# Fancomi2017/InstanceFusion

Hardware: AMD Instinct MI355X
Metric: frames/s + ms/frame (ICP|fuse|instance) at 640x480, 5M surfels, 1/2/4/8 GPU (higher is better)
Workload: dtype f32; 1 GPU; 5000000-surfel map, 640x480 synthetic RGBD stream, 3-level ICP+RGB + surfel fuse + canned-mask instance votes with superpixel refinement; surfels_live=4734799, surfel_slots=4734799, map_order=random, parallelism=replicas x1, loop_frames=90

## Files before the change

include/ifx_c_api.h:

```cpp
#ifndef IFX_C_API_H_
#define IFX_C_API_H_

#include <stdint.h>

#ifdef __cplusplus
extern "C" {
#endif

#define IFX_NUM_INSTANCES 96
#define IFX_VOTE_FLOATS 48

enum {
    IFX_OK = 0,
    IFX_E_INVALID = -1,
    IFX_E_HIP = -2,
    IFX_E_CAPACITY = -3,
    IFX_E_STATE = -4
};

typedef struct ifx_config {
    int32_t width, height;
    float fx, fy, cx, cy;
    int32_t time_delta;
    float confidence;
    float depth_cut;
    float max_depth_processed;
    float icp_weight;
    int32_t pyramid;
    int32_t fast_odom;
    int32_t so3;
    int32_t max_surfels;
    int32_t device;
    int32_t n_ranks, rank;
} ifx_config;

typedef struct ifx ifx_t;

int ifx_create(const ifx_config* cfg, ifx_t** out);
void ifx_destroy(ifx_t* h);
const char* ifx_last_error(ifx_t* h);
const char* ifx_global_error(void);

int ifx_process_frame(ifx_t* h, const uint8_t* rgb, const uint16_t* depth, int64_t timestamp,
                      const float* in_pose16, float weight_mult, float* out_pose16);
int ifx_process_frame_ex(ifx_t* h, const uint8_t* rgb, const uint16_t* depth, int64_t timestamp, const int32_t* inst_table,
                         const float* in_pose16, float weight_mult, int bootstrap, float* out_pose16);
int ifx_enqueue_frame_device(ifx_t* h, const uint8_t* d_rgb, const uint16_t* d_depth,
                             int64_t timestamp, const float* in_pose16, float weight_mult);
int ifx_prefetch_frame_device(ifx_t* h, const uint8_t* d_rgb_next, const uint16_t* d_depth_next);
int ifx_hint_next_frame_device(ifx_t* h, const uint8_t* d_rgb_next, const uint16_t* d_depth_next);
int ifx_hint_next_frame(ifx_t* h, const uint8_t* rgb_next, const uint16_t* depth_next);
int ifx_set_shard(ifx_t* h, int rank, int nranks);
int ifx_sharded_frame_phase(ifx_t* h, int phase, const uint8_t* d_rgb, const uint16_t* d_depth);
int ifx_key_images(ifx_t* h, void** key_index, void** key_splat, void** key_ids, void** key_both, int64_t* n_pixels);
int ifx_stream_handles(ifx_t* h, void** main_stream, void** side_stream);
int ifx_owner_frame_phase(ifx_t* h, int phase, const uint8_t* d_rgb, const uint16_t* d_depth);
int ifx_camera_count(ifx_t* h, int n_cameras);
int ifx_camera_select(ifx_t* h, int cam);
int ifx_owner_set_frame_pose(ifx_t* h, const float* pose16);
int ifx_owner_set_tracking_rank(ifx_t* h, int rank);
int ifx_owner_track_ahead(ifx_t* h, int cam, int tracking_rank, const uint8_t* d_rgb, const uint16_t* d_depth);
int ifx_comm_unique_id(uint8_t* out128);
int ifx_owner_init_comm(ifx_t* h, const uint8_t* unique_id128);
int ifx_owner_set_comm(ifx_t* h, void* nccl_comm);
int ifx_owner_process_frame_device(ifx_t* h, const uint8_t* d_rgb, const uint16_t* d_depth, int64_t timestamp);
int ifx_owner_process_frame(ifx_t* h, const uint8_t* rgb, const uint16_t* depth, int64_t timestamp, float* out_pose16);
int ifx_owner_predict(ifx_t* h);
int ifx_owner_process_segmentation(ifx_t* h, const uint8_t* rgb, const uint16_t* depth, const uint8_t* masks, const int32_t* class_ids, int nm, int frame, int flags);
int ifx_owner_knn_vote_colour(ifx_t* h);
int ifx_owner_exchange_stats(ifx_t* h, int64_t* out2, int reset);
int ifx_owner_comm_ranks(ifx_t* h);
int ifx_owner_exchange(ifx_t* h, int phase, void** ptrs, int64_t* bytes, int32_t* ops, int max_n);
int ifx_owner_predict_phase(ifx_t* h, int step);
int ifx_owner_of(const float* xyz, int n, int n_ranks, int32_t* out);
int ifx_owner_segmentation_begin(ifx_t* h, const uint8_t* rgb, const uint16_t* depth, const uint8_t* masks, const int32_t* class_ids, int nm, int frame, int flags);
int ifx_owner_segmentation_resume(ifx_t* h);
int ifx_owner_ids_begin(ifx_t* h);
int ifx_owner_ids_resume(ifx_t* h);
int ifx_owner_knn_export(ifx_t* h, void** d_points, void** d_labels, int* n);
int ifx_owner_knn_vote(ifx_t* h, const void* d_all_points, const void* d_all_labels, int n_all, int own_offset);
int ifx_map_seq(ifx_t* h, uint32_t* out, int max_n);
int ifx_map_bounding_boxes(ifx_t* h, int bbox_type, float ratio, float* boxes96x6, float* ground_normal3, float* gc_matrix16, float* inst_matrix96x16,
                           int32_t* ground_votes648);
int ifx_instance_point_cloud(ifx_t* h, int bbox_type, int32_t* counts96, int inst, float* out10, int max_records);
int ifx_view_list_stats(ifx_t* h, int32_t* out4);
int ifx_sync(ifx_t* h);
int ifx_get_pose(ifx_t* h, float* out_pose16);
int ifx_tick(ifx_t* h);
int ifx_trajectory(ifx_t* h, float* out_poses16, int max_frames);
int ifx_tracker_diag(ifx_t* h, float* diag8);
int ifx_tracker_fallbacks(ifx_t* h);
int ifx_tracker_range_exceeded(ifx_t* h);

int ifx_set_loop_closure(ifx_t* h, int enable, int count_thresh, float err_thresh, float cov_thresh);
int ifx_loop_closure_diag(ifx_t* h, float* out24);
typedef int (*ifx_loop_closure_cb)(ifx_t* h, const float* lc24, void* user);
int ifx_set_loop_closure_callback(ifx_t* h, ifx_loop_closure_cb cb, void* user);
int ifx_sample_graph_model(ifx_t* h, float* out_xyzt, int max_n);
int ifx_loop_closure_constraints(ifx_t* h, float* src3, float* dst3, int32_t* times, int max_n);
int ifx_set_deformation(ifx_t* h, const float* graph16, int n_nodes, int is_fern);
int ifx_adopt_estimated_pose(ifx_t* h);

typedef int (*ifx_fern_cb)(ifx_t* h, void* user);
int ifx_set_fern_callback(ifx_t* h, ifx_fern_cb cb, void* user);
int ifx_adopt_pose(ifx_t* h, const float* pose16);
int ifx_fern_frame(ifx_t* h, uint8_t* img_rgb, float* verts4, float* norms4, uint8_t* inst_rgb);
int ifx_fern_frame_async(ifx_t* h);
int ifx_fern_frame_fetch(ifx_t* h, uint8_t* img_rgb, float* verts4, float* norms4, uint8_t* inst_rgb);
int ifx_track_maps(ifx_t* h, const float* model_v4, const float* model_n4, const uint8_t* model_rgba, const float* cur_v4, const float* cur_n4,
                   const uint8_t* cur_rgba, float* pose16, float* diag8);

typedef struct ifx_soa_view {
    int32_t count;
    int32_t capacity;
    float* d_pos_conf;
    float* d_norm_rad;
    float* d_color;
    float* d_times;
    float* d_img_corr;
    float* d_votes;
} ifx_soa_view;
int ifx_map_view(ifx_t* h, ifx_soa_view* out);
int ifx_hot_records_stale(ifx_t* h);
int ifx_map_count(ifx_t* h);
int ifx_map_slots(ifx_t* h);
int ifx_map_download(ifx_t* h, int max_n, float* pc, float* nr, float* col, float* tm, float* ic,
                     float* votes);
int ifx_map_upload(ifx_t* h, int n, const float* pc, const float* nr, const float* col,
                   const float* tm, const float* ic, const float* votes);
int ifx_set_pose(ifx_t* h, const float* pose16, int tick);
int ifx_compact(ifx_t* h);
int ifx_set_option(ifx_t* h, const char* name, int value);

const int32_t* ifx_ids_after(ifx_t* h);
int ifx_image_download(ifx_t* h, const char* name, void* out, int64_t max_bytes);

int ifx_predict_indices(ifx_t* h, const float* pose16, int time);
int ifx_combined_predict(ifx_t* h, const float* pose16, int time, int max_time);
int ifx_fuse(ifx_t* h, const float* pose16, int time, float weighting);
int ifx_clean(ifx_t* h, const float* pose16, int time);
int ifx_render_ids(ifx_t* h, const float* pose16, int mode);
int ifx_set_frame(ifx_t* h, const uint8_t* rgb, const uint16_t* depth);

int ifx_icp_step(ifx_t* h, const float* Rcurr9, const float* tcurr3, const float* d_vmap_curr,
                 const float* d_nmap_curr, const float* Rprev_inv9, const float* tprev3, float fx,
                 float fy, float cx, float cy, const float* d_vmap_g_prev, const float* d_nmap_g_prev,
                 float dist_thres, float angle_thres, int w, int hgt, float* out29_host);
int ifx_rgb_residual(ifx_t* h, float min_scale, const int16_t* d_didx, const int16_t* d_didy,
                     const float* d_last_depth, const float* d_next_depth, const uint8_t* d_last_img,
                     const uint8_t* d_next_img, void* d_corres8, float max_depth_delta,
                     const float* kt3, const float* krkinv9, int w, int hgt, int* count_host,
                     int* sigma_host);
int ifx_rgb_step(ifx_t* h, const void* d_corres8, float sigma, const float* d_cloud3, float fx,
                 float fy, const int16_t* d_didx, const int16_t* d_didy, float sobel_scale, int w,
                 int hgt, float* out29_host);
int ifx_so3_step(ifx_t* h, const uint8_t* d_last_img, const uint8_t* d_next_img,
                 const float* image_basis9, const float* kinv9, const float* krlr9, int w, int hgt,
                 float* out11_host);
typedef struct ifx_pyramids {
    uint16_t* depth[3];
    float* vmap_curr[3];
    float* nmap_curr[3];
    uint8_t* next_img[3];
    int16_t* didx[3];
    int16_t* didy[3];
    float* vmap_g_prev[3];
    float* nmap_g_prev[3];
    float* last_depth[3];
// ... 41 lines not shown
```

instancefusion_amd/__init__.py:

```python
from __future__ import annotations

import ctypes as C
import os

import numpy as np

_HERE = os.path.dirname(os.path.abspath(__file__))
LIB_PATH = os.environ.get("IFX_LIB") or os.path.join(_HERE, "libifx.so")
HEADER_PATH = os.path.join(os.path.dirname(_HERE), "include", "ifx_c_api.h")

NUM_INSTANCES = 96
VOTE_FLOATS = 48


class IfxError(RuntimeError):
    pass


class IfxConfig(C.Structure):
    _fields_ = [
        ("width", C.c_int32), ("height", C.c_int32),
        ("fx", C.c_float), ("fy", C.c_float), ("cx", C.c_float), ("cy", C.c_float),
        ("time_delta", C.c_int32), ("confidence", C.c_float), ("depth_cut", C.c_float),
        ("max_depth_processed", C.c_float), ("icp_weight", C.c_float),
        ("pyramid", C.c_int32), ("fast_odom", C.c_int32), ("so3", C.c_int32),
        ("max_surfels", C.c_int32), ("device", C.c_int32), ("n_ranks", C.c_int32), ("rank", C.c_int32),
    ]


class Pyramids(C.Structure):
    _fields_ = [(n, C.c_void_p * 3) for n in ("depth", "vmap_curr", "nmap_curr", "next_img", "didx", "didy", "vmap_g_prev", "nmap_g_prev", "last_depth", "last_img", "cloud")]


class SoaView(C.Structure):
    _fields_ = [("count", C.c_int32), ("capacity", C.c_int32), ("d_pos_conf", C.c_void_p), ("d_norm_rad", C.c_void_p),
                ("d_color", C.c_void_p), ("d_times", C.c_void_p), ("d_img_corr", C.c_void_p), ("d_votes", C.c_void_p)]


def default_config(w=640, h=480, fx=528.0, fy=528.0, cx=320.0, cy=240.0, max_surfels=1 << 20, **kw):
    d = dict(width=w, height=h, fx=fx, fy=fy, cx=cx, cy=cy, time_delta=200, confidence=10.0, depth_cut=12.0,
             max_depth_processed=20.0, icp_weight=10.0, pyramid=1, fast_odom=0, so3=1, max_surfels=max_surfels,
             device=0, n_ranks=1, rank=0)
    d.update(kw)
    return d


_lib = None

_P = C.c_void_p
_SIGS = {
    "ifx_create": (C.c_int, [C.POINTER(IfxConfig), C.POINTER(_P)]),
    "ifx_destroy": (None, [_P]),
    "ifx_last_error": (C.c_char_p, [_P]),
    "ifx_global_error": (C.c_char_p, []),
    "ifx_process_frame": (C.c_int, [_P, _P, _P, C.c_int64, _P, C.c_float, _P]),
    "ifx_process_frame_ex": (C.c_int, [_P, _P, _P, C.c_int64, _P, _P, C.c_float, C.c_int, _P]),
    "ifx_enqueue_frame_device": (C.c_int, [_P, _P, _P, C.c_int64, _P, C.c_float]),
    "ifx_set_shard": (C.c_int, [_P, C.c_int, C.c_int]),
    "ifx_sharded_frame_phase": (C.c_int, [_P, C.c_int, _P, _P]),
    "ifx_key_images": (C.c_int, [_P, _P, _P, _P, _P, _P]),
    "ifx_stream_handles": (C.c_int, [_P, _P, _P]),
    "ifx_owner_frame_phase": (C.c_int, [_P, C.c_int, _P, _P]),
    "ifx_owner_exchange": (C.c_int, [_P, C.c_int, _P, _P, _P, C.c_int]),
    "ifx_owner_of": (C.c_int, [_P, C.c_int, C.c_int, _P]),
    "ifx_owner_segmentation_begin": (C.c_int, [_P, _P, _P, _P, _P, C.c_int, C.c_int, C.c_int]),
    "ifx_owner_segmentation_resume": (C.c_int, [_P]),
    "ifx_owner_ids_begin": (C.c_int, [_P]),
    "ifx_owner_ids_resume": (C.c_int, [_P]),
    "ifx_owner_knn_export": (C.c_int, [_P, _P, _P, _P]),
    "ifx_owner_knn_vote": (C.c_int, [_P, _P, _P, C.c_int, C.c_int]),
    "ifx_owner_predict_phase": (C.c_int, [_P, C.c_int]),
    "ifx_camera_count": (C.c_int, [_P, C.c_int]),
    "ifx_camera_select": (C.c_int, [_P, C.c_int]),
    "ifx_owner_set_frame_pose": (C.c_int, [_P, _P]),
    "ifx_owner_set_tracking_rank": (C.c_int, [_P, C.c_int]),
    "ifx_owner_track_ahead": (C.c_int, [_P, C.c_int, C.c_int, _P, _P]),
    "ifx_comm_unique_id": (C.c_int, [_P]),
    "ifx_owner_init_comm": (C.c_int, [_P, _P]),
    "ifx_owner_set_comm": (C.c_int, [_P, _P]),
    "ifx_owner_process_frame_device": (C.c_int, [_P, _P, _P, C.c_int64]),
    "ifx_owner_process_frame": (C.c_int, [_P, _P, _P, C.c_int64, _P]),
    "ifx_owner_predict": (C.c_int, [_P]),
    "ifx_owner_process_segmentation": (C.c_int, [_P, _P, _P, _P, _P, C.c_int, C.c_int, C.c_int]),
    "ifx_owner_knn_vote_colour": (C.c_int, [_P]),
    "ifx_owner_exchange_stats": (C.c_int, [_P, _P, C.c_int]),
    "ifx_owner_comm_ranks": (C.c_int, [_P]),
    "ifx_map_seq": (C.c_int, [_P, _P, C.c_int]),
    "ifx_prefetch_frame_device": (C.c_int, [_P, _P, _P]),
    "ifx_hint_next_frame_device": (C.c_int, [_P, _P, _P]),
    "ifx_hint_next_frame": (C.c_int, [_P, _P, _P]),
    "ifx_lookahead_stats": (C.c_int, [_P, _P, C.c_int]),
    "ifx_view_list_stats": (C.c_int, [_P, _P]),
    "ifx_map_bounding_boxes": (C.c_int, [_P, C.c_int, C.c_float, _P, _P, _P, _P, _P]),
    "ifx_instance_point_cloud": (C.c_int, [_P, C.c_int, _P, C.c_int, _P, C.c_int]),
    "ifx_sync": (C.c_int, [_P]),
    "ifx_get_pose": (C.c_int, [_P, _P]),
    "ifx_tick": (C.c_int, [_P]),
    "ifx_trajectory": (C.c_int, [_P, _P, C.c_int]),
    "ifx_tracker_diag": (C.c_int, [_P, _P]),
    "ifx_tracker_fallbacks": (C.c_int, [_P]),
    "ifx_build_pyramids": (C.c_int, [_P, _P, _P, _P, _P, _P, _P, C.POINTER(Pyramids)]),
    "ifx_tracker_range_exceeded": (C.c_int, [_P]),
    "ifx_hot_records_stale": (C.c_int, [_P]),
    "ifx_set_loop_closure": (C.c_int, [_P, C.c_int, C.c_int, C.c_float, C.c_float]),
    "ifx_loop_closure_diag": (C.c_int, [_P, _P]),
    "ifx_set_loop_closure_callback": (C.c_int, [_P, _P, _P]),
    "ifx_sample_graph_model": (C.c_int, [_P, _P, C.c_int]),
    "ifx_loop_closure_constraints": (C.c_int, [_P, _P, _P, _P, C.c_int]),
    "ifx_set_deformation": (C.c_int, [_P, _P, C.c_int, C.c_int]),
    "ifx_adopt_estimated_pose": (C.c_int, [_P]),
    "ifx_set_fern_callback": (C.c_int, [_P, _P, _P]),
    "ifx_adopt_pose": (C.c_int, [_P, _P]),
    "ifx_fern_frame": (C.c_int, [_P, _P, _P, _P, _P]),
    "ifx_fern_frame_async": (C.c_int, [_P]),
    "ifx_fern_frame_fetch": (C.c_int, [_P, _P, _P, _P, _P]),
    "ifx_track_maps": (C.c_int, [_P, _P, _P, _P, _P, _P, _P, _P, _P]),
    "ifx_map_view": (C.c_int, [_P, C.POINTER(SoaView)]),
    "ifx_map_count": (C.c_int, [_P]),
    "ifx_map_slots": (C.c_int, [_P]),
    "ifx_map_download": (C.c_int, [_P, C.c_int] + [_P] * 6),
    "ifx_map_upload": (C.c_int, [_P, C.c_int] + [_P] * 6),
    "ifx_set_pose": (C.c_int, [_P, _P, C.c_int]),
    "ifx_compact": (C.c_int, [_P]),
    "ifx_set_option": (C.c_int, [_P, C.c_char_p, C.c_int]),
    "ifx_ids_after": (_P, [_P]),
    "ifx_image_download": (C.c_int, [_P, C.c_char_p, _P, C.c_int64]),
    "ifx_predict_indices": (C.c_int, [_P, _P, C.c_int]),
    "ifx_combined_predict": (C.c_int, [_P, _P, C.c_int, C.c_int]),
    "ifx_fuse": (C.c_int, [_P, _P, C.c_int, C.c_float]),
    "ifx_clean": (C.c_int, [_P, _P, C.c_int]),
    "ifx_render_ids": (C.c_int, [_P, _P, C.c_int]),
    "ifx_set_frame": (C.c_int, [_P, _P, _P]),
    "ifx_icp_step": (C.c_int, [_P, _P, _P, _P, _P, _P, _P, C.c_float, C.c_float, C.c_float, C.c_float, _P, _P, C.c_float, C.c_float, C.c_int, C.c_int, _P]),
    "ifx_rgb_residual": (C.c_int, [_P, C.c_float, _P, _P, _P, _P, _P, _P, _P, C.c_float, _P, _P, C.c_int, C.c_int, _P, _P]),
    "ifx_rgb_step": (C.c_int, [_P, _P, C.c_float, _P, C.c_float, C.c_float, _P, _P, C.c_float, C.c_int, C.c_int, _P]),
    "ifx_so3_step": (C.c_int, [_P, _P, _P, _P, _P, _P, C.c_int, C.c_int, _P]),
    "ifx_track_pair": (C.c_int, [_P] * 9),
    "ifx_tracker_buffer_download": (C.c_int, [_P, C.c_char_p, C.c_int, _P, C.c_int64]),
    "ifx_should_segment": (C.c_int, [_P, C.c_int]),
    "ifx_process_segmentation": (C.c_int, [_P, _P, _P, _P, _P, C.c_int, C.c_int, C.c_int]),
    "ifx_process_segmentation_device": (C.c_int, [_P, _P, C.c_int, C.c_float, _P, C.c_int, C.c_int, C.c_int, _P]),
    "ifx_labels": (C.c_int, [_P, _P, C.c_int]),
    "ifx_render_project_map": (C.c_int, [_P, _P, _P]),
    "ifx_set_instance_gt": (C.c_int, [_P, _P]),
    "ifx_precision_recall": (C.c_int, [_P, _P, _P, _P]),
    "ifx_instance_table": (C.c_int, [_P, _P]),
    "ifx_loop_closure_instance_table": (C.c_int, [_P, _P]),
    "ifx_mask_clean_overlap": (C.c_int, [_P, _P, C.c_int]),
    "ifx_mask_geometric_filter": (C.c_int, [_P, _P, _P, _P, C.c_int, _P]),
    "ifx_knn_vote_colour": (C.c_int, [_P, _P, C.c_int]),
    "ifx_slic_segment": (C.c_int, [_P, _P, _P]),
    "ifx_merge_superpixels": (C.c_int, [_P, _P, _P, _P, _P]),
    "ifx_mask_superpixel_filter": (C.c_int, [_P, _P, _P, C.c_int]),
    "ifx_stage_ms": (C.c_int, [_P, _P, C.c_int]),
    "ifx_superpixel_ahead_stats": (C.c_int, [_P, _P, _P, _P, C.c_int]),
    "ifx_kernel_ms": (C.c_int, [_P, C.c_char_p, _P, _P]),
}


def lib():
    global _lib
    if _lib is None:
        if not os.path.exists(LIB_PATH):
            raise IfxError(f"{LIB_PATH} is missing: build it with `make -C instancefusion_amd/csrc` "
                           "(there is no CPU fallback)")
        L = C.CDLL(LIB_PATH)
        for name, (res, args) in _SIGS.items():
            f = getattr(L, name)
            f.restype = res
            f.argtypes = args
        _lib = L
    return _lib


def exported_symbols():
# ... 45 lines not shown
        if r != 0:
            raise IfxError(f"ifx_create failed ({r}): {self.L.ifx_global_error().decode()}")
        self.handle = hp
        if id_rule is not None:
            self.set_option("id_rule", id_rule)

    def close(self):
        if getattr(self, "handle", None):
            self.L.ifx_destroy(self.handle)
            self.handle = None

    def __del__(self):
        try:
            self.close()
        except Exception:
            pass

    def _chk(self, r, what):
        if r < 0:
            raise IfxError(f"{what} failed ({r}): {self.L.ifx_last_error(self.handle).decode()}")
        return r

    def set_option(self, name, value):
        self._chk(self.L.ifx_set_option(self.handle, name.encode(), int(value)), "ifx_set_option")

    def set_instance_gt(self, gt):
        self._chk(self.L.ifx_set_instance_gt(self.handle, None if gt is None else _ptr(np.ascontiguousarray(gt, np.uint8))), "ifx_set_instance_gt")

    def processFrame(self, rgb, depth, timestamp=0, smallInstanceTable=None, instanceGT=None, inPose=None, weightMultiplier=1.0, bootstrap=False):
        rgb = np.ascontiguousarray(rgb, np.uint8)
        depth = np.ascontiguousarray(depth, np.uint16)
        assert rgb.size == self.w * self.h * 3 and depth.size == self.w * self.h
        if instanceGT is not None:
            self.set_instance_gt(instanceGT)
        out = np.zeros(16, np.float32)
        ip = None if inPose is None else np.ascontiguousarray(inPose, np.float32).reshape(16)
        tab = None if smallInstanceTable is None else np.ascontiguousarray(smallInstanceTable, np.int32)
        self._chk(self.L.ifx_process_frame_ex(self.handle, _ptr(rgb), _ptr(depth), int(timestamp), _ptr(tab), _ptr(ip), float(weightMultiplier), int(bool(bootstrap)), _ptr(out)),
                  "ifx_process_frame_ex")
        return out.reshape(4, 4)

    process_frame = processFrame

    def hint_next_frame(self, rgb, depth):
        rgb = np.ascontiguousarray(rgb, np.uint8)
        depth = np.ascontiguousarray(depth, np.uint16)
        assert rgb.size == self.w * self.h * 3 and depth.size == self.w * self.h
        self._chk(self.L.ifx_hint_next_frame(self.handle, _ptr(rgb), _ptr(depth)), "ifx_hint_next_frame")

    def enqueue_frame_device(self, d_rgb_ptr: int, d_depth_ptr: int, timestamp=0):
        self._chk(self.L.ifx_enqueue_frame_device(self.handle, C.c_void_p(d_rgb_ptr), C.c_void_p(d_depth_ptr), int(timestamp), None, 1.0),
                  "ifx_enqueue_frame_device")

    def prefetch_frame_device(self, d_rgb_ptr: int, d_depth_ptr: int):
        self._chk(self.L.ifx_prefetch_frame_device(self.handle, C.c_void_p(d_rgb_ptr), C.c_void_p(d_depth_ptr)), "ifx_prefetch_frame_device")

    def hint_next_frame_device(self, d_rgb_ptr: int, d_depth_ptr: int):
        self._chk(self.L.ifx_hint_next_frame_device(self.handle, C.c_void_p(d_rgb_ptr), C.c_void_p(d_depth_ptr)), "ifx_hint_next_frame_device")

    def camera_count(self, k):
        self._chk(self.L.ifx_camera_count(self.handle, int(k)), "ifx_camera_count")

    def camera_select(self, c):
        self._chk(self.L.ifx_camera_select(self.handle, int(c)), "ifx_camera_select")

    def owner_set_frame_pose(self, pose):
        p = None if pose is None else np.ascontiguousarray(pose, np.float32).reshape(16)
        self._chk(self.L.ifx_owner_set_frame_pose(self.handle, _ptr(p)), "ifx_owner_set_frame_pose")

    def owner_track_ahead(self, cam, tracking_rank, d_rgb_ptr=0, d_depth_ptr=0):
        return self._chk(self.L.ifx_owner_track_ahead(self.handle, int(cam), int(tracking_rank), C.c_void_p(d_rgb_ptr), C.c_void_p(d_depth_ptr)), "ifx_owner_track_ahead")

    def owner_frame_phase(self, phase, d_rgb_ptr=0, d_depth_ptr=0):
        return self._chk(self.L.ifx_owner_frame_phase(self.handle, int(phase), C.c_void_p(d_rgb_ptr), C.c_void_p(d_depth_ptr)), "ifx_owner_frame_phase")

    def owner_set_tracking_rank(self, r):
        self._chk(self.L.ifx_owner_set_tracking_rank(self.handle, int(r)), "ifx_owner_set_tracking_rank")

    def view_list_stats(self):
        out = np.zeros(4, np.int32)
        self._chk(self.L.ifx_view_list_stats(self.handle, _ptr(out)), "ifx_view_list_stats")
        return dict(window=int(out[0]), outside=int(out[1]), scans=int(out[2]), age=int(out[3]))

    def sync(self):
        self._chk(self.L.ifx_sync(self.handle), "ifx_sync")

    def getCurrPose(self):
        out = np.zeros(16, np.float32)
        self._chk(self.L.ifx_get_pose(self.handle, _ptr(out)), "ifx_get_pose")
        return out.reshape(4, 4)

    @property
    def tick(self):
        return self.L.ifx_tick(self.handle)

    def trajectory(self, max_frames=1 << 16):
        out = np.zeros((max_frames, 16), np.float32)
        n = self._chk(self.L.ifx_trajectory(self.handle, _ptr(out), max_frames), "ifx_trajectory")
        return out[:n].reshape(n, 4, 4).copy()

    def tracker_diag(self):
        out = np.zeros(8, np.float32)
        self._chk(self.L.ifx_tracker_diag(self.handle, _ptr(out)), "ifx_tracker_diag")
        return out

    def tracker_fallbacks(self):
        return self._chk(self.L.ifx_tracker_fallbacks(self.handle), "ifx_tracker_fallbacks")

    def tracker_range_exceeded(self):
        return self._chk(self.L.ifx_tracker_range_exceeded(self.handle), "ifx_tracker_range_exceeded")

    def set_loop_closure(self, enable=True, count_thresh=35000, err_thresh=5e-5, cov_thresh=1e-5):
        self._chk(self.L.ifx_set_loop_closure(self.handle, int(enable), int(count_thresh), err_thresh, cov_thresh), "ifx_set_loop_closure")

    def loop_closure_diag(self):
        out = np.zeros(24, np.float32)
        self._chk(self.L.ifx_loop_closure_diag(self.handle, _ptr(out)), "ifx_loop_closure_diag")
        return dict(ran=bool(out[0]), inactive_pixels=int(out[1]), icp_error=float(out[2]), icp_count=float(out[3]), cov_ok=bool(out[4]),
                    accepted=bool(out[5]), est_pose=out[6:22].reshape(4, 4).copy(), cov_max=float(out[22]), candidates=int(out[23]))

    def set_loop_closure_callback(self, fn):
        if fn is None:
            self._lc_cb = None
            self._chk(self.L.ifx_set_loop_closure_callback(self.handle, None, None), "ifx_set_loop_closure_callback")
            return

        def tramp(_h, lc, _user):
            try:
                fn(self, np.ctypeslib.as_array(lc, shape=(24,)).copy())
                return 0
            except Exception:
                import traceback

                traceback.print_exc()
                return -1

        self._lc_cb = C.CFUNCTYPE(C.c_int, C.c_void_p, C.POINTER(C.c_float), C.c_void_p)(tramp)
        self._chk(self.L.ifx_set_loop_closure_callback(self.handle, C.cast(self._lc_cb, C.c_void_p), None), "ifx_set_loop_closure_callback")

    def sample_graph_model(self, max_n=4096):
        out = np.zeros((max_n, 4), np.float32)
        n = self._chk(self.L.ifx_sample_graph_model(self.handle, _ptr(out), max_n), "ifx_sample_graph_model")
        return out[:n].copy()

    def loop_closure_constraints(self, max_n=4096):
        src, dst, tm = np.zeros((max_n, 3), np.float32), np.zeros((max_n, 3), np.float32), np.zeros(max_n, np.int32)
        n = self._chk(self.L.ifx_loop_closure_constraints(self.handle, _ptr(src), _ptr(dst), _ptr(tm), max_n), "ifx_loop_closure_constraints")
        return src[:n].copy(), dst[:n].copy(), tm[:n].copy()

    def set_deformation(self, graph16, is_fern=False):
        g = np.ascontiguousarray(graph16, np.float32).reshape(-1, 16)
        self._chk(self.L.ifx_set_deformation(self.handle, _ptr(g), g.shape[0], int(is_fern)), "ifx_set_deformation")

    def adopt_estimated_pose(self):
        self._chk(self.L.ifx_adopt_estimated_pose(self.handle), "ifx_adopt_estimated_pose")

    def set_fern_callback(self, fn):
        if fn is None:
            self._fern_cb = None
            self._chk(self.L.ifx_set_fern_callback(self.handle, None, None), "ifx_set_fern_callback")
            return

        def tramp(_h, _user):
            try:
                return 1 if fn(self) else 0
            except Exception:
# ... 308 lines not shown
```

instancefusion_amd/csrc/ifx_api.hip:

```cpp
#include <climits>
#include "ifx_ctx.h"
#include <string.h>
#include <stdio.h>
#include <algorithm>

int ifx_tracker_external_pose(ifx* h, const float* d_pose16, float weight_mult);
int ifx_tracker_set_weight(ifx* h, float weight_mult);
int ifx_compact_enqueue(ifx* h, int refresh_ids);

void hs_invalidate_view(ifx* h);
static std::string g_err;
extern "C" const char* ifx_global_error(void) { return g_err.c_str(); }
extern "C" const char* ifx_last_error(ifx_t* h) { return h ? h->err.c_str() : g_err.c_str(); }

hipEvent_t ifx_event_get(ifx* h)
{
    if (!h->event_pool.empty()) { hipEvent_t e = h->event_pool.back(); h->event_pool.pop_back(); return e; }
    hipEvent_t e;
    hipEventCreate(&e);
    return e;
}
void ifx_ktime_begin(ifx* h, const char* name, hipEvent_t* a)
{
    (void)name;
// ... 207 lines not shown
    if (h->ev_cam_side) hipEventDestroy(h->ev_cam_side);
    if (h->ev_slic_ahead) hipEventDestroy(h->ev_slic_ahead);
    if (h->ev_cam_parked) hipEventDestroy(h->ev_cam_parked);
    if (h->ev_lc_ready) hipEventDestroy(h->ev_lc_ready);
    if (h->ev_lc_done) hipEventDestroy(h->ev_lc_done);
    void* ptrs[] = {h->d_state, h->d_traj, h->d_scratch, h->pc, h->nr, h->col, h->tm, h->ic, h->votes, h->pc2, h->nr2, h->col2, h->tm2, h->ic2, h->votes2, h->upd_owner, h->assoc_vis, h->list_a, h->list_b, h->list_c, h->list_v, h->list_vi, h->d_list_ctr, h->tile_n, h->tile_box, h->tile_pairs, h->tile_recs, h->labels, h->seq, h->seq2,
                    h->labels2, h->scan_flags, h->scan_out, h->scan_block, h->slot[0].rgb, h->slot[0].depth_raw, h->slot[0].depth_filt, h->slot[0].dm, h->slot[0].dmf, h->slot[1].rgb, h->slot[1].depth_raw,
                    h->slot[1].depth_filt, h->slot[1].dm, h->slot[1].dmf, h->key_index, h->key_both,
                    h->index_id, h->index_vc, h->index_ct, h->index_tap, h->pred_vertex, h->fill_vertex,
                    h->fill_normal, h->fill_image, h->ids_after, h->ids_tmp, h->assoc_key, h->assoc_target, h->meas_pc, h->meas_nr, h->meas_col};
    for (void* p : ptrs) if (p) hipFree(p);
    for (size_t q = 2; q < h->slot.size(); q++) { FrameSlot& f2 = h->slot[q]; void* p2[] = {f2.rgb, f2.depth_raw, f2.depth_filt, f2.dm, f2.dmf}; for (void* p : p2) if (p) hipFree(p); }
    if (h->h_result) hipHostFree(h->h_result);
    if (h->h_pose_early) hipHostFree(h->h_pose_early);
    if (h->ev_pose_early) hipEventDestroy(h->ev_pose_early);
    for (int q_ = 0; q_ < 2; q_++) { if (h->hint_stage_rgb[q_]) hipHostFree(h->hint_stage_rgb[q_]); if (h->hint_stage_depth[q_]) hipHostFree(h->hint_stage_depth[q_]); }
    if (h->rgb_stage) hipHostFree(h->rgb_stage);
    if (h->depth_stage) hipHostFree(h->depth_stage);
    ifx_free_tracker(h);
    ifx_free_instance(h);
    ifx_slic_free(h);
    ifx_knn_free_all(h);
    for (int q = 0; q < 2; q++) { if (h->slot[q].ready) hipEventDestroy(h->slot[q].ready); if (h->slot[q].released) hipEventDestroy(h->slot[q].released); }
    if (h->stream_c) hipStreamDestroy(h->stream_c);
    if (h->stream_b) hipStreamDestroy(h->stream_b);
    if (h->stream) hipStreamDestroy(h->stream);
    delete h;
}

extern "C" int ifx_set_loop_closure(ifx_t* h, int enable, int count_thresh, float err_thresh, float cov_thresh)
{
    if (!h) return IFX_E_INVALID;
    if (h->hint_rgb || h->slot[h->tick & 1].for_tick == h->tick) { h->err = "loop-closure detection cannot change while a frame is announced ahead"; return IFX_E_STATE; }
    ifx_drop_tracked(h);
    if (h->stream_c) { HIPCHK(h, hipStreamSynchronize(h->stream_c)); h->lc_pending = 0; }
    if (enable) {
        int r = ifx_tracker_alloc_m2m(h);
        if (r) return r;
        if (!h->stream_c && hipStreamCreate(&h->stream_c) != hipSuccess) { h->err = "stream creation failed"; return IFX_E_HIP; }
        if (!h->ev_lc_ready) {
            if (hipEventCreateWithFlags(&h->ev_lc_ready, hipEventDisableTiming) != hipSuccess ||
                hipEventCreateWithFlags(&h->ev_lc_done, hipEventDisableTiming) != hipSuccess) { h->err = "event creation failed"; return IFX_E_HIP; }
        }
    }
    h->lc_enable = enable ? 1 : 0; h->lc_count_thresh = count_thresh; h->lc_err_thresh = err_thresh; h->lc_cov_thresh = cov_thresh;
    return IFX_OK;
}
extern "C" int ifx_set_loop_closure_callback(ifx_t* h, ifx_loop_closure_cb cb, void* user)
{
    if (!h) return IFX_E_INVALID;
    h->lc_cb = cb; h->lc_user = user;
    return IFX_OK;
}
extern "C" int ifx_set_fern_callback(ifx_t* h, ifx_fern_cb cb, void* user)
{
    if (!h) return IFX_E_INVALID;
    if (cb && !h->lc_enable) { h->err = "the fern callback runs inside the loop-closure block: enable it first (ifx_set_loop_closure)"; return IFX_E_STATE; }
    h->fern_cb = cb; h->fern_user = user;
    return IFX_OK;
}
extern "C" int ifx_loop_closure_diag(ifx_t* h, float* out24)
{
    if (!h || !out24) return IFX_E_INVALID;
    if (!h->h_lc) { memset(out24, 0, 24 * 4); return IFX_OK; }
    if (h->ev_result) HIPCHK(h, hipEventSynchronize(h->ev_result));
    if (h->lc_event_valid) HIPCHK(h, hipEventSynchronize(h->ev_lc_done));
    memcpy(out24, h->h_lc, 24 * 4);
    return IFX_OK;
}

extern "C" int ifx_set_option(ifx_t* h, const char* name, int value)
{
    if (!h || !name) return IFX_E_INVALID;
    std::string s(name);
    if (s == "compact_every_frame") h->opt_compact_every_frame = value;
    else if (s == "kernel_timing") { hipStreamSynchronize(h->stream); ktime_flush(h); h->opt_kernel_timing = value; }
    else if (s == "reference_passes") { h->opt_reference_passes = value; ifx_vlist_reap(h); hs_invalidate_view(h); }
    else if (s == "two_streams") h->opt_two_streams = value;
    else if (s == "stage_timing") h->opt_stage_timing = value;
    else if (s == "track_ahead") h->opt_track_ahead = value;
    else if (s == "slic_ahead") h->opt_slic_ahead = value;
    else if (s == "fold_result") h->opt_fold_result = value;
    else if (s == "clean_raster") h->opt_clean_raster = value;
    else if (s == "hot_records") { h->opt_hot = value; h->hot_valid = 0; }
    else if (s == "hot_verify") h->opt_hot_verify = value;
    else if (s == "own_first_live") h->opt_own_first_live = value;
    else if (s == "own_track_rows") {
        if (!h->own) { h->err = "own_track_rows: the handle was not created for a sharded map"; return IFX_E_STATE; }
        h->opt_own_track_rows = value;
    }
    else if (s == "own_track_rows_emulate") h->opt_own_track_rows_emulate = value;
    else if (s == "own_key_rs") {
        if (!h->own) { h->err = "own_key_rs: the handle was not created for a sharded map"; return IFX_E_STATE; }
        if (h->own_g * 8 > IFX_KEY_SLACK) { h->err = "own_key_rs: more ranks than the key image's slack allows"; return IFX_E_INVALID; }
        h->opt_own_key_rs = value;
    }
    else if (s == "own_lazy_ids") {
        if (!h->own) { h->err = "own_lazy_ids: the handle was not created for a sharded map"; return IFX_E_STATE; }
        if (value && ifx_own_lattice(h) + 1 > 16 * 1024) { h->err = "own_lazy_ids: the image's id lattice is larger than the pack kernel's one workgroup holds (16 383 entries)"; return IFX_E_INVALID; }
        h->opt_own_lazy_ids = value;
    }
    else if (s == "id_rule") {
        if (value != 0 && value != 1) { h->err = "id_rule must be 0 (ray-disc) or 1 (the reference's screen-space quads)"; return IFX_E_INVALID; }
        if (h->own || h->shard_n > 1) { h->err = "id_rule: the id renders of a sharded map keep the ray-disc rule"; return IFX_E_STATE; }
        if (h->hint_rgb || h->slot[h->tick & 1].for_tick == h->tick || h->ids_pending || h->clean_raster_pending) { h->err = "id_rule cannot change while a frame is in flight or announced ahead"; return IFX_E_STATE; }
        if (value != h->opt_id_rule) {
            h->opt_id_rule = value;
            h->ids_full_valid = 0; h->ids_sparse_frame = 1; h->ids_view_ok = 0;
            h->seg_counts_valid = 0;
            const int r = ifx_ids_ensure(h);
            if (r) return r;
        }
    }
    else if (s == "cam_swap") h->opt_cam_swap = value;
    else if (s == "cam_side") h->opt_cam_side = value;
    else if (s == "host_entry_async") h->opt_host_entry_async = value;
    else if (s == "gn_prologue_blocks") h->opt_gn_prologue_blocks = value;
    else if (s == "compact_divisor") h->opt_compact_divisor = value;
    else if (s == "icp_blocks") h->opt_icp_blocks = std::max(0, std::min(2048, value));
    else if (s == "view_blocks") h->opt_view_blocks = std::max(0, std::min(65536, value));
    else if (s == "clean_blocks") h->opt_clean_blocks = std::max(0, std::min(65536, value));
    else if (s == "index_blocks") h->opt_index_blocks = std::max(0, std::min(8192, value));
    else if (s == "res_blocks") h->opt_res_blocks = std::max(0, std::min(4096, value));
    else if (s == "rgb_blocks") h->opt_rgb_blocks = std::max(0, std::min(1024, value));
    else if (s == "raster_tiles") h->opt_raster_tiles = value;
    else if (s == "view_list") { h->opt_vlist = value; ifx_vlist_reap(h); hs_invalidate_view(h); }
    else if (s == "seg_aside") h->opt_seg_aside = value;
    else if (s == "pace") h->opt_pace = value;
    else if (s == "lazy_ids") { ifx_ids_ensure(h); h->opt_lazy_ids = value; }
    else if (s == "seg_device") h->opt_seg_device = value;
    else if (s == "ff_rounds") h->opt_ff_rounds = value;
    else if (s == "gn_persist_blocks") { if (value < 1) return IFX_E_INVALID; ifx_drop_tracked(h); h->opt_gn_persist_blocks = value; }
    else if (s == "gn_persist") {
        if (value < 0 || value > 7) { h->err = "gn_persist is a mask of pyramid levels (0..7)"; return IFX_E_INVALID; }
        ifx_drop_tracked(h);
        h->opt_gn_persist = value;
    }
    else if (s == "gn_spin_limit" || s == "gn_fault") {
        if (value < 0) return IFX_E_INVALID;
        ifx_drop_tracked(h);
        HIPCHK(h, hipStreamSynchronize(h->stream));
        HIPCHK(h, hipMemcpy((char*)h->d_state + (s == "gn_fault" ? offsetof(DevState, gn_fault) : offsetof(DevState, gn_spin_limit)), &value, sizeof(int), hipMemcpyHostToDevice));
    }
    else if (s == "gn_prologue") { ifx_drop_tracked(h); h->opt_gn_prologue = value ? 1 : 0; }
    else if (s == "raster_lds") h->opt_raster_lds = value;
    else if (s == "raster_earlyz") h->opt_raster_earlyz = value;
    else if (s == "pyramid" || s == "fast_odom" || s == "so3" || s == "icp_weight_x1000") {
        if (h->hint_rgb || h->slot[h->tick & 1].for_tick == h->tick) { h->err = "tracker options cannot change while a frame is announced ahead"; return IFX_E_STATE; }
        ifx_drop_tracked(h);
        if (s == "pyramid") h->cfg.pyramid = value ? 1 : 0;
        else if (s == "fast_odom") h->cfg.fast_odom = value ? 1 : 0;
        else if (s == "so3") h->cfg.so3 = value ? 1 : 0;
        else { if (value < 0 || value > 100000) { h->err = "icp_weight_x1000 must be in [0, 100000]"; return IFX_E_INVALID; } h->cfg.icp_weight = value / 1000.f; }
    }
    else { h->err = "unknown option " + s; return IFX_E_INVALID; }
    return IFX_OK;
}

__global__ void k_frame_result(DevState* __restrict__ st, FrameResult* __restrict__ out, float* __restrict__ traj_slot)
{
    if (threadIdx.x < 64) frame_result_wave(st, out, traj_slot, 0, (int)threadIdx.x);
}

static int enqueue_frame_side(ifx* h, int s, int tick, const uint8_t* rgb, const uint16_t* depth, int src_kind)
{
    FrameSlot& f = h->slot[s];
// ... 652 lines not shown
        }
        break;
    default: break;
    }
    return n;
}
extern "C" int ifx_owner_ids_begin(ifx_t* h)
{
    if (!h) return IFX_E_INVALID;
    if (!h->own) { h->err = "ifx_owner_ids_begin: the handle was not created for a sharded map"; return IFX_E_STATE; }
    if (h->oseg_state) { h->err = "ifx_owner_ids_begin: a segmentation call is in flight"; return IFX_E_STATE; }
    return ifx_owner_ids_begin_impl(h);
}
extern "C" int ifx_owner_ids_resume(ifx_t* h)
{
    if (!h) return IFX_E_INVALID;
    return ifx_owner_ids_resume_impl(h);
}
extern "C" int ifx_owner_of(const float* xyz, int n, int n_ranks, int32_t* out)
{
    if (!xyz || !out || n < 0) return IFX_E_INVALID;
    for (int i = 0; i < n; i++) out[i] = ifx_owner_of_point(xyz[i * 3], xyz[i * 3 + 1], xyz[i * 3 + 2], n_ranks);
    return IFX_OK;
}
extern "C" int ifx_map_seq(ifx_t* h, uint32_t* out, int max_n)
{
    if (!h || !out) return IFX_E_INVALID;
    int r = ifx_compact(h);
    if (r) return r;
    DevState hs;
    HIPCHK(h, hipMemcpy(&hs, h->d_state, sizeof(hs), hipMemcpyDeviceToHost));
    const int n = std::min(hs.count, max_n);
    HIPCHK(h, hipMemcpy(out, h->seq, (size_t)n * 4, hipMemcpyDeviceToHost));
    return n;
}

extern "C" int ifx_enqueue_frame_device(ifx_t* h, const uint8_t* d_rgb, const uint16_t* d_depth, int64_t timestamp, const float* in_pose16, float weight_mult)
{
    (void)timestamp;
    if (!h || !d_rgb || !d_depth) return IFX_E_INVALID;
    ifx_housekeeping(h);
    return enqueue_frame(h, d_rgb, d_depth, 0, in_pose16, weight_mult);
}

extern "C" int ifx_prefetch_frame_device(ifx_t* h, const uint8_t* d_rgb_next, const uint16_t* d_depth_next)
{
    if (!h || !d_rgb_next || !d_depth_next) return IFX_E_INVALID;
    if (h->tick == 1 || !h->opt_two_streams) return IFX_OK;
    return enqueue_frame_side(h, h->tick & 1, h->tick, d_rgb_next, d_depth_next, 0);
}

extern "C" int ifx_hint_next_frame_device(ifx_t* h, const uint8_t* d_rgb_next, const uint16_t* d_depth_next)
{
    if (!h || !d_rgb_next || !d_depth_next) return IFX_E_INVALID;
    h->hint_rgb = d_rgb_next; h->hint_depth = d_depth_next; h->hint_kind = 0;
    return IFX_OK;
}

extern "C" int ifx_hint_next_frame(ifx_t* h, const uint8_t* rgb_next, const uint16_t* depth_next)
{
    if (!h || !rgb_next || !depth_next) return IFX_E_INVALID;
    if (h->own || !h->cams.empty()) { h->err = "ifx_hint_next_frame: single-stream, unsharded handles (use ifx_hint_next_frame_device)"; return IFX_E_STATE; }
    if (!h->opt_two_streams || !h->stream_b) return IFX_OK;
    const int p = (h->tick + 1) & 1;
    if (!h->hint_stage_rgb[p] || !h->hint_stage_depth[p]) {
        if (h->hint_stage_rgb[p]) { (void)hipHostFree(h->hint_stage_rgb[p]); h->hint_stage_rgb[p] = nullptr; }
        if (h->hint_stage_depth[p]) { (void)hipHostFree(h->hint_stage_depth[p]); h->hint_stage_depth[p] = nullptr; }
        uint8_t* sr = nullptr; uint16_t* sd = nullptr;
        if (hipHostMalloc((void**)&sr, (size_t)h->P * 3, hipHostMallocDefault) != hipSuccess || hipHostMalloc((void**)&sd, (size_t)h->P * 2, hipHostMallocDefault) != hipSuccess) {
            (void)hipGetLastError();
            if (sr) (void)hipHostFree(sr);
            h->err = "ifx_hint_next_frame: no pinned memory for the staging pair";
            return IFX_E_HIP;
        }
        h->hint_stage_rgb[p] = sr; h->hint_stage_depth[p] = sd;
    }
    memcpy(h->hint_stage_depth[p], depth_next, (size_t)h->P * 2);
    memcpy(h->hint_stage_rgb[p], rgb_next, (size_t)h->P * 3);
    h->hinted_src_rgb[p] = rgb_next; h->hinted_src_depth[p] = depth_next; h->hinted_tick[p] = h->tick + 1;
    h->hint_rgb = h->hint_stage_rgb[p]; h->hint_depth = h->hint_stage_depth[p]; h->hint_kind = 1;
    return IFX_OK;
}

extern "C" int ifx_view_list_stats(ifx_t* h, int32_t* out4)
{
    if (!h || !out4) return IFX_E_INVALID;
    DevState hs;
    HIPCHK(h, hipStreamSynchronize(h->stream));
    HIPCHK(h, hipMemcpy(&hs, h->d_state, sizeof(hs), hipMemcpyDeviceToHost));
    out4[0] = (int32_t)hs.vl_n[0]; out4[1] = (int32_t)hs.vl_n[1]; out4[2] = hs.vl_scans; out4[3] = hs.vl_age;
    return IFX_OK;
}

extern "C" int ifx_sync(ifx_t* h)
{
    if (!h) return IFX_E_INVALID;
    HIPCHK(h, hipStreamSynchronize(h->stream));
    HIPCHK(h, hipStreamSynchronize(h->stream_b));
    if (h->stream_c) HIPCHK(h, hipStreamSynchronize(h->stream_c));
    ktime_flush(h);
    stage_flush(h);
    if (h->h_result->overflow) { h->err = "surfel store capacity exceeded"; return IFX_E_CAPACITY; }
    return IFX_OK;
}
extern "C" int ifx_tracker_fallbacks(ifx_t* h)
{
    if (!h) return IFX_E_INVALID;
    int r = ifx_sync(h);
    return r ? r : h->h_result->gn_timeout;
}

extern "C" int ifx_hot_records_stale(ifx_t* h)
{
    if (!h) return IFX_E_INVALID;
    HIPCHK(h, hipStreamSynchronize(h->stream));
    int v = 0;
    HIPCHK(h, hipMemcpy(&v, &h->d_state->hot_stale, sizeof(int), hipMemcpyDeviceToHost));
    return v;
}
extern "C" int ifx_tracker_range_exceeded(ifx_t* h)
{
    if (!h) return IFX_E_INVALID;
    int r = ifx_sync(h);
    if (r) return r;
    if (h->stream_c) HIPCHK(h, hipStreamSynchronize(h->stream_c));
    if (h->stream_b) HIPCHK(h, hipStreamSynchronize(h->stream_b));
    std::vector<const DevState*> sts;
    sts.push_back(h->d_state);
    if (h->d_m2m) sts.push_back(h->d_m2m);
    if (h->d_cam_trk) sts.push_back(h->d_cam_trk);
    for (const FrameSlot& f : h->slot) if (f.so3) sts.push_back(f.so3);
    long long total = 0;
    for (const DevState* d : sts) {
        int v = 0;
        HIPCHK(h, hipMemcpy(&v, (const char*)d + offsetof(DevState, range_exceeded), sizeof(int), hipMemcpyDeviceToHost));
        total += v;
    }
    return (int)std::min<long long>(total, 0x7FFFFFFF);
}

static int frame_sync(ifx* h)
{
    if (h->tracked_ahead == h->tick && h->ev_result && !h->lc_enable && !h->opt_kernel_timing && !h->opt_stage_timing) {
        HIPCHK(h, hipEventSynchronize(h->ev_result));
        if (h->h_result->overflow) { h->err = "surfel store capacity exceeded"; return IFX_E_CAPACITY; }
        return IFX_OK;
    }
    return ifx_sync(h);
}

extern "C" int ifx_process_frame(ifx_t* h, const uint8_t* rgb, const uint16_t* depth, int64_t timestamp, const float* in_pose16, float weight_mult, float* out_pose16)
{
    return ifx_process_frame_ex(h, rgb, depth, timestamp, nullptr, in_pose16, weight_mult, 0, out_pose16);
}

extern "C" int ifx_process_frame_ex(ifx_t* h, const uint8_t* rgb, const uint16_t* depth, int64_t timestamp, const int32_t* inst_table, const float* in_pose16,
                                    float weight_mult, int bootstrap, float* out_pose16)
{
    (void)timestamp; (void)inst_table;
    if (!h || !rgb || !depth) return IFX_E_INVALID;
    const int par = h->tick & 1;
    const bool pre = h->hinted_tick[par] == h->tick && h->hinted_src_rgb[par] == (const void*)rgb && h->hinted_src_depth[par] == (const void*)depth && h->prestaged_tick == h->tick &&
                     h->slot[par].for_tick == h->tick && h->slot[par].src_rgb == (const void*)h->hint_stage_rgb[par] && !h->own;
    h->hinted_tick[par] = -1;
    if (pre) {
        h->want_early_pose = 0;
// ... 196 lines not shown
{
    if (!h) return IFX_E_INVALID;
    ifx_drop_tracked(h);
    h->seg_counts_valid = 0;
    ifx_compact_enqueue(h, 1);
    return ifx_sync(h);
}

extern "C" int ifx_map_download(ifx_t* h, int max_n, float* pc, float* nr, float* col, float* tm, float* ic, float* votes)
{
    if (!h) return IFX_E_INVALID;
    ifx_drop_tracked(h);
    h->seg_counts_valid = 0;
    int r = ifx_compact(h);
    if (r) return r;
    DevState hs;
    r = read_state(h, &hs);
    if (r) return r;
    int n = std::min(hs.count, max_n);
    if (pc) HIPCHK(h, hipMemcpy(pc, h->pc, (size_t)n * 16, hipMemcpyDeviceToHost));
    if (nr) HIPCHK(h, hipMemcpy(nr, h->nr, (size_t)n * 16, hipMemcpyDeviceToHost));
    if (col) HIPCHK(h, hipMemcpy(col, h->col, (size_t)n * 8, hipMemcpyDeviceToHost));
    if (tm) HIPCHK(h, hipMemcpy(tm, h->tm, (size_t)n * 8, hipMemcpyDeviceToHost));
    if (ic) HIPCHK(h, hipMemcpy(ic, h->ic, (size_t)n * 16, hipMemcpyDeviceToHost));
    if (votes) HIPCHK(h, hipMemcpy(votes, h->votes, (size_t)n * IFX_VF * 4, hipMemcpyDeviceToHost));
    return n;
}

extern "C" int ifx_map_upload(ifx_t* h, int n, const float* pc, const float* nr, const float* col, const float* tm, const float* ic, const float* votes)
{
    if (!h || n < 0 || !pc || !nr || !col || !tm) return IFX_E_INVALID;
    ifx_drop_tracked(h);
    for (CamCtx& c_ : h->cams) {
        if (c_.ahead_valid && c_.ev_ahead) hipStreamWaitEvent(h->stream, c_.ev_ahead, 0);
        c_.ahead_valid = 0;
    }
    h->housekeeping_due = 0;
    h->seg_counts_valid = 0;
    h->map_external = 1;
    h->hot_valid = 0;
    h->age_epoch = INT_MAX;
    const int n_all = n;
    std::vector<uint32_t> keep;
    std::vector<float> f_pc, f_nr, f_col, f_tm, f_ic, f_votes;
    keep.reserve(h->own ? (size_t)n / h->own_g + 1024 : (size_t)n);
    for (int i = 0; i < n; i++)
        if (!h->own || ifx_owner_of_point(pc[(size_t)i * 4], pc[(size_t)i * 4 + 1], pc[(size_t)i * 4 + 2], h->own_g) == h->cfg.rank) keep.push_back((uint32_t)i);
    if (h->own) {
        const size_t m = keep.size();
        auto gather = [&](const float* src, int width, std::vector<float>& dst) {
            if (!src) return (const float*)nullptr;
            dst.resize(m * width);
            for (size_t k = 0; k < m; k++) memcpy(&dst[k * width], &src[(size_t)keep[k] * width], (size_t)width * 4);
            return (const float*)dst.data();
        };
        pc = gather(pc, 4, f_pc); nr = gather(nr, 4, f_nr); col = gather(col, 2, f_col); tm = gather(tm, 2, f_tm); ic = gather(ic, 4, f_ic); votes = gather(votes, 48, f_votes);
        n = (int)m;
    }
    if (n > h->cap) { h->err = "upload exceeds capacity"; return IFX_E_CAPACITY; }
    if (h->stream_c) { HIPCHK(h, hipStreamSynchronize(h->stream_c)); h->lc_pending = 0; }
    if (h->stream_b) HIPCHK(h, hipStreamSynchronize(h->stream_b));
    HIPCHK(h, hipStreamSynchronize(h->stream));
    HIPCHK(h, hipMemcpy(h->pc, pc, (size_t)n * 16, hipMemcpyHostToDevice));
    HIPCHK(h, hipMemcpy(h->nr, nr, (size_t)n * 16, hipMemcpyHostToDevice));
    HIPCHK(h, hipMemcpy(h->col, col, (size_t)n * 8, hipMemcpyHostToDevice));
    HIPCHK(h, hipMemcpy(h->tm, tm, (size_t)n * 8, hipMemcpyHostToDevice));
    if (ic) HIPCHK(h, hipMemcpy(h->ic, ic, (size_t)n * 16, hipMemcpyHostToDevice));
    else HIPCHK(h, hipMemset(h->ic, 0, (size_t)n * 16));
    if (votes) HIPCHK(h, hipMemcpy(h->votes, votes, (size_t)n * IFX_VF * 4, hipMemcpyHostToDevice));
    else HIPCHK(h, hipMemset(h->votes, 0, (size_t)n * IFX_VF * 4));
    DevState hs;
    HIPCHK(h, hipMemcpy(&hs, h->d_state, sizeof(hs), hipMemcpyDeviceToHost));
    HIPCHK(h, hipMemcpy(h->seq, keep.data(), (size_t)n * 4, hipMemcpyHostToDevice));
    hs.count = n; hs.n_dead = 0; hs.n_new = 0; hs.overflow = 0; hs.vl_valid = 0; hs.next_seq = (unsigned int)n_all; hs.first_live = 0;
    h->view_dirty = 0;
    {
        float rmax = 0.f;
        for (int i = 0; i < n; i++) { float r = nr[(size_t)i * 4 + 3]; if (r == r && r > rmax && r < 1e30f) rmax = r; }
        unsigned int bits; memcpy(&bits, &rmax, 4);
        if (bits > hs.r_max_bits) hs.r_max_bits = bits;
    }
    HIPCHK(h, hipMemcpy(h->d_state, &hs, sizeof(hs), hipMemcpyHostToDevice));
    HIPCHK(h, hipMemset(h->upd_owner, 0xFF, (size_t)h->cap * 4));
    HIPCHK(h, hipMemset(h->labels, 0xFF, (size_t)h->cap * 4));
    h->labels_stale_all = 1;
    return IFX_OK;
}

extern "C" int ifx_set_pose(ifx_t* h, const float* pose16, int tick)
{
    if (!h || !pose16) return IFX_E_INVALID;
    ifx_drop_tracked(h);
    for (CamCtx& c_ : h->cams) {
        if (c_.ahead_valid && c_.ev_ahead) hipStreamWaitEvent(h->stream, c_.ev_ahead, 0);
        c_.ahead_valid = 0;
    }
    DevState hs;
    int r = read_state(h, &hs);
    if (r) return r;
    memcpy(hs.pose, pose16, 64);
    memcpy(hs.last_pose, pose16, 64);
    pose_inverse(hs.pose, hs.pose_inv);
    HIPCHK(h, hipMemcpy(h->d_state, &hs, sizeof(hs), hipMemcpyHostToDevice));
    if (tick != h->tick) h->age_epoch = INT_MAX;
    h->tick = tick;
    return IFX_OK;
}

extern "C" const int32_t* ifx_ids_after(ifx_t* h)
{
    if (!h) return nullptr;
    if (ifx_ids_ensure(h)) return nullptr;
    return h->ids_after;
}

extern "C" int ifx_image_download(ifx_t* h, const char* name, void* out, int64_t max_bytes)
{
    if (!h || !name || !out) return IFX_E_INVALID;
    std::string s(name);
    size_t P = (size_t)h->P, bytes = 0;
    const void* src = nullptr;
    if (h->stream_c) HIPCHK(h, hipStreamSynchronize(h->stream_c));
    if (s == "ids_after") { const int r_ = ifx_ids_ensure(h); if (r_) return r_; src = h->ids_after; bytes = P * 4; }
    else if (s == "ids_tmp") { src = h->ids_tmp; bytes = P * 4; }
    else if (s == "index") { src = h->index_id; bytes = P * 4; }
    else if (s == "index_vc") { src = h->index_vc; bytes = P * 16; }
    else if (s == "index_ct") { src = h->index_ct; bytes = P * 16; }
    else if (s == "index_nr") { src = h->index_nr; bytes = P * 16; }
    else if (s == "pred_vertex") { src = h->pred_vertex; bytes = P * 16; }
    else if (s == "pred_normal") { src = h->pred_normal; bytes = P * 16; }
    else if (s == "pred_image") { src = h->pred_image; bytes = P * 4; }
    else if (s == "pred_inst") { src = h->pred_inst; bytes = P * 4; }
    else if (s == "pred_time") { src = h->pred_time; bytes = P * 2; }
    else if (s == "old_vertex" && h->d_m2m) { src = h->old_vertex; bytes = P * 16; }
    else if (s == "old_normal" && h->d_m2m) { src = h->old_normal; bytes = P * 16; }
    else if (s == "old_image" && h->d_m2m) { src = h->old_image; bytes = P * 4; }
    else if (s == "old_time" && h->d_m2m) { src = h->old_time; bytes = P * 2; }
    else if (s == "act_vertex" && h->d_m2m) { src = h->act_vertex; bytes = P * 16; }
    else if (s == "act_normal" && h->d_m2m) { src = h->act_normal; bytes = P * 16; }
    else if (s == "act_image" && h->d_m2m) { src = h->act_image; bytes = P * 4; }
    else if (s == "fill_vertex") { src = h->fill_vertex; bytes = P * 16; }
    else if (s == "fill_normal") { src = h->fill_normal; bytes = P * 16; }
    else if (s == "fill_image") { src = h->fill_image; bytes = P * 4; }
    else if (s == "depth_filtered") { src = h->depth_filt; bytes = P * 2; }
    else if (s == "depth_metric") { src = h->dm; bytes = P * 4; }
    else if (s == "depth_metric_filtered") { src = h->dmf; bytes = P * 4; }
    else { h->err = "unknown image " + s; return IFX_E_INVALID; }
    if ((int64_t)bytes > max_bytes) { h->err = "buffer too small"; return IFX_E_INVALID; }
    HIPCHK(h, hipStreamSynchronize(h->stream));
    HIPCHK(h, hipMemcpy(out, src, bytes, hipMemcpyDeviceToHost));
    return (int)bytes;
}

#ifdef IFX_STAMPS
void ifx_debug_copy2(long long* out);
extern "C" int ifx_debug_stamps(ifx_t* h, long long* out8, int reset)
{
    DevState hs;
    int r = read_state(h, &hs);
    if (r) return r;
    memcpy(out8, hs.dbg, sizeof(hs.dbg));
    ifx_debug_copy2(out8 + 8);
    if (reset) { memset(hs.dbg, 0, sizeof(hs.dbg)); hipMemcpy((char*)h->d_state + offsetof(DevState, dbg), hs.dbg, sizeof(hs.dbg), hipMemcpyHostToDevice); }
    return IFX_OK;
}
#endif
// ... 1 lines not shown
```

instancefusion_amd/csrc/ifx_ctx.h:

```cpp
#pragma once
#include <hip/hip_runtime.h>
#include <stdint.h>
#include <string>
#include <vector>
#include <map>
#include "../../include/ifx_c_api.h"
#include "ifx_dev.h"

#ifndef IFX_LIST_SEGS
#define IFX_LIST_SEGS 8
#endif

struct DevState {
    float pose[16];
    float pose_inv[16];
    float last_pose[16];
    float weighting;
    int dense_enough;
    int count;
    int n_dead;
    int n_new;
    int overflow;
    unsigned int r_max_bits;
    float Rprev[9], tprev[3], Rprev_inv[9];
// ... 159 lines not shown
#pragma unroll
            for (int c = 0; c < 3; c++) tr += A[r * 4 + c] * B[r * 4 + c];
        ok = (dx * dx + dy * dy + dz * dz <= 0.81f * VL_TRANS * VL_TRANS) && ((tr - 1.0f) * 0.5f >= cosf(0.9f * VL_ROT)) && tr == tr;
    }
    if (ok) { st->vl_scan = 0; st->vl_age = age + 1; return; }
    st->vl_scan = 1; st->vl_age = 0; st->vl_valid = 1; st->vl_scans++;
#pragma unroll
    for (int k = 0; k < 16; k++) st->vl_pose[k] = B[k];
    st->vl_n[0] = 0; st->vl_n[1] = 0;
}
__device__ inline void vlist_decide(DevState* st)
{
    vlist_decide_core(st, st->vl_pose, st->pose, st->vl_valid, st->vl_age);
}

struct CamCtx {
    float* state = nullptr;
    uint8_t* pred = nullptr;
    float *fill_v = nullptr, *fill_n = nullptr;
    uint8_t* fill_i = nullptr;
    uint8_t* img[IFX_NUM_PYRS] = {};
    int32_t* ids = nullptr;
    int valid = 0;
    void* ahead_pose = nullptr;
    hipEvent_t ev_ahead = nullptr;
    int ahead_valid = 0;
    const void *ahead_rgb = nullptr, *ahead_depth = nullptr;
    int pred_root = -1;
};
#define IFX_CAM_STATE_BYTES 200

struct KernelTiming { double total_ms = 0; int launches = 0; };
struct PendingEvent { int name_id; hipEvent_t a, b; };

struct ifx {
    ifx_config cfg;
    int w, h, P, cap;
    hipStream_t stream = nullptr;
    hipStream_t stream_b = nullptr;
    hipStream_t stream_c = nullptr;
    hipEvent_t ev_lc_ready = nullptr, ev_lc_done = nullptr;
    int lc_pending = 0, lc_deferred = 0;
    hipStream_t cur = nullptr;
    std::vector<FrameSlot> slot = std::vector<FrameSlot>(3);
    int last_frame_slot = 0;
    int cur_slot = 0;
    std::vector<CamCtx> cams;
    int cur_cam = 0;
    DevState* d_cam_trk = nullptr;
    Pyr cam_pyr;
    double* cam_so3_acc = nullptr; unsigned int* cam_so3_ticket = nullptr;
    hipEvent_t ev_cam_ahead = nullptr, ev_cam_parked = nullptr, ev_cam_side = nullptr;
    hipStream_t cam_side_stream = nullptr;
    int cam_ahead_used = 0;
    unsigned long long *gfl_index = nullptr, *gfl_splat = nullptr;
    int32_t* own_slot_img = nullptr;
    int own_fast = 0, own_fast_raster = 0;
    int opt_own_lazy_ids = 0;
    int opt_own_key_rs = 0;
    int opt_own_track_rows = 0, opt_own_track_rows_emulate = 0;
    int track_rc = 0;
    int own_ids_lat = 0;
    int own_ids_pending = 0;
    unsigned long long* own_lat_tmp = nullptr;
    int own_need_decide = 0;
    int pred_root = -1;
    int own_track_rank = -1;
    float own_frame_pose[16]; int own_frame_pose_set = 0;
    int own = 0, own_g = 1;
    size_t pred_bytes = 0; int* pred_tail = nullptr;
    void* comm = nullptr;
    int shard_rank = 0, shard_n = 1;
    int opt_two_streams = 1;
    int opt_stage_timing = 0;
    int opt_gn_prologue_blocks = 2048;
    int opt_cam_side = 1;
    int opt_cam_swap = 1;
    void* hot = nullptr;
    int hot_valid = 0;
    int opt_hot_verify = 0;
    int opt_hot = 1;
    void* frame_hot = nullptr;
    int opt_clean_raster = 1;
    int clean_raster_pending = 0;
    float frame_weight_mult = 1.f;
    int opt_fold_result = 1;
    float* result_fold_traj = nullptr;
    int result_folded = 0;
    int opt_slic_ahead = 1;
    int opt_track_ahead = 1;
    int tracked_ahead = 0;
    int opt_own_first_live = 1;
    int opt_pace = 1;
    int opt_seg_aside = 1;
    hipEvent_t ev_result = nullptr;
    int n_side_prepared = 0, n_tracked_ahead = 0, n_host_hinted = 0;
    int hint_kind = 0;
    uint8_t* hint_stage_rgb[2] = {nullptr, nullptr}; uint16_t* hint_stage_depth[2] = {nullptr, nullptr};
    const void *hinted_src_rgb[2] = {nullptr, nullptr}, *hinted_src_depth[2] = {nullptr, nullptr};
    int hinted_tick[2] = {-1, -1};
    const uint8_t* hint_rgb = nullptr;
    const uint16_t* hint_depth = nullptr;
    std::string err;
    int tick = 1;
    int ids_pending = 0;
    int ids_view_ok = 0;
    int view_scan_tick = -1;
    int opt_id_rule = 0;
    int opt_lazy_ids = 1;
    int ids_full_valid = 1, ids_sparse_frame = 0;
    int ids_full_hint = 0;
    int opt_compact_every_frame = 0;
    int last_compact_tick = -1;
    int opt_compact_divisor = 8;
    int opt_kernel_timing = 0;
    int opt_reference_passes = 0;
    int opt_gn_persist_blocks = 128;
    int opt_gn_persist = 0;
    int gn_max_blocks[4] = {0, 0, 0, 0};
    int opt_rgb_blocks = 0;
    int opt_gn_prologue = 1;
    int oseg_state = 0, oseg_nm = 0, oseg_m = 0, oseg_flags = 0, oseg_pending = 0;
    std::vector<uint8_t> oseg_unavail;
    std::vector<int> oseg_cmp, oseg_bbox, oseg_class;
    hipEvent_t oseg_ev = nullptr;
    void* d_kexp = nullptr;
    int gn_begin_folded = 0;
    int labels_stale_all = 1;
    int opt_raster_lds = 0;
    int opt_view_blocks = 0, opt_clean_blocks = 0, opt_index_blocks = 0;
    int icp_resident_blocks = 1024;
    int opt_res_blocks = 0;
    int opt_icp_blocks = 0;
    int opt_raster_tiles = -1;
    int map_external = 0;
    int lc_enable = 0, lc_count_thresh = 35000;
    float lc_err_thresh = 5e-5f, lc_cov_thresh = 1e-5f;
    DevState* d_m2m = nullptr;
    Pyr m2m;
    float *old_vertex = nullptr, *old_normal = nullptr;
    uint8_t *old_image = nullptr, *old_inst = nullptr;
    uint16_t* old_time = nullptr;
    float *act_vertex = nullptr, *act_normal = nullptr;
    uint8_t *act_image = nullptr, *act_inst = nullptr;
    uint16_t* act_time = nullptr;
    size_t lc_half = 0;
    int own_tracked_tick = 0;
    float* h_lc = nullptr;
    int lc_event_valid = 0;
    float* d_graph = nullptr;
    int graph_nodes = 0, graph_is_fern = 0;
    uint8_t* d_inst_gt = nullptr;
    int inst_gt_on = 0;
    void* d_fern = nullptr;
    float* d_project = nullptr;
    float *d_sample = nullptr, *d_cons = nullptr;
    ifx_loop_closure_cb lc_cb = nullptr;
    void* lc_user = nullptr;
    ifx_fern_cb fern_cb = nullptr;
    void* fern_user = nullptr;
    uint8_t* h_fern = nullptr;
    hipEvent_t ev_fern = nullptr;
    int fern_pending = 0;
    int in_fern_cb = 0;
    DevState* d_state = nullptr;
    FrameResult* h_result = nullptr;
// ... 159 lines not shown
```

instancefusion_amd/csrc/ifx_map.hip:

```cpp
#include <climits>
#include "ifx_ctx.h"
#include <string.h>

#define DEAD_TIME (-1.0e9f)
#define ASSOC_NONE 0xFFFFFFFFu
#define ASSOC_NEW 0xFFFFFFFEu
#define MAP_THREADS 256
#ifndef MAP_BLOCKS
#define MAP_BLOCKS 2048
#endif
#ifndef LIST_BLOCKS
#define LIST_BLOCKS 1024
#endif

__device__ inline float get_radius(float depth, float norm_z, float inv_fx, float inv_fy)
{
    float meanFocal = ((1.0f / fabsf(inv_fx)) + (1.0f / fabsf(inv_fy))) / 2.0f;
    const float sqrt2 = 1.41421356237f;
    float radius = (depth / meanFocal) * sqrt2;
    float radius_n = radius / fabsf(norm_z);
    radius_n = fminf(2.0f * radius, radius_n);
    return radius_n;
}
__device__ inline float confidence_fn(float x, float y, float cx, float cy, float weighting)
// ... 1370 lines not shown
            const int ii = i < n ? i : n - 1;
            p4s[r] = ld_once(&pc_in[ii]);
            ts[r] = ld_once(&tm[ii]);
        }
        asm volatile("" ::"v"(p4s[0].x), "v"(p4s[1].x), "v"(p4s[2].x), "v"(p4s[3].x), "v"(p4s[4].x), "v"(p4s[5].x), "v"(p4s[6].x), "v"(p4s[7].x), "v"(ts[0].x), "v"(ts[1].x), "v"(ts[2].x),
                     "v"(ts[3].x), "v"(ts[4].x), "v"(ts[5].x), "v"(ts[6].x), "v"(ts[7].x));
#pragma unroll
        for (int r = 0; r < CF_ROUNDS; r++) {
            const int i = chunk * CF_SLOTS + r * MAP_THREADS + threadIdx.x;
            bool in = false, in_i = false;
            if (i < n) {
                const float4 p4 = p4s[r];
                const float2 t = ts[r];
                const float wv = t.y;
                const bool overdue = age_rule_gone(wv, p4.w, time_prev, c) && wv > DEAD_TIME;
                if (overdue) {
                    float4 q4 = p4;
                    q4.w = -1.0f;
                    pc_rw[i] = q4;
                    tm[i] = make_float2(t.x, DEAD_TIME);
                    if (hot) { hot[i].pc = q4; hot[i].tm = make_float2(t.x, DEAD_TIME); }
                    dead++;
                } else if (wv > DEAD_TIME) {
                    in = near_frustum(xf_point(T, v3m(p4.x, p4.y, p4.z)), reach, P, c.maxDepth);
                    if (in && wv > 0.f && (float)time - wv > (float)c.timeDelta) {
                        in = false;
                        in_i = !(p4.w < c.conf);
                    }
                }
            }
            pos[r] = bcount2_reserve(L2, in, in_i);
            keep |= in ? (1u << r) : 0u;
            keep_i |= in_i ? (1u << r) : 0u;
        }
        __syncthreads();
        const int seg = chunk % LIST_SEGS;
        if (threadIdx.x < 2) { L2.base[threadIdx.x] = L2.n[threadIdx.x] ? atomicAdd(list_ctr(c, 1 + threadIdx.x, seg), L2.n[threadIdx.x]) : 0u; L2.n[threadIdx.x] = 0; }
        __syncthreads();
        const unsigned int ba = seg * c.seg_cap + L2.base[0], bi = seg * c.seg_cap + L2.base[1];
#pragma unroll
        for (int r = 0; r < CF_ROUNDS; r++) {
            const unsigned int i = (unsigned int)(chunk * CF_SLOTS + r * MAP_THREADS + threadIdx.x);
            if (keep & (1u << r)) list[ba + pos[r]] = i;
            if (keep_i & (1u << r)) list_i[bi + pos[r]] = i;
        }
    }
    dead = wave_sum_i(dead);
    if ((threadIdx.x & 63) == 0 && dead) atomicAdd(&st->n_dead, dead);
}

__global__ void k_vlist_offsets(DevState* st, Cam c, const float2* __restrict__ tm)
{
    if (!st->vl_scan || threadIdx.x != 0) return;
    for (int which = 0; which < 2; which++) {
        unsigned int run = 0;
        for (int seg = 0; seg < LIST_SEGS; seg++) {
            unsigned int* ctr = list_ctr(c, 1 + which, seg);
            const unsigned int n = *ctr;
            *ctr = 0;
            st->vl_seg_n[which * LIST_SEGS + seg] = n;
            st->vl_seg_off[which * LIST_SEGS + seg] = run;
            run += n;
        }
        st->vl_n[which] = run;
    }
    {
        int f = st->first_live;
        const int n = st->count;
        while (f < n && !(tm[f].y > DEAD_TIME)) f++;
        st->first_live = f;
    }
}
__global__ __launch_bounds__(MAP_THREADS) void k_vlist_concat(const DevState* __restrict__ st, Cam c, const unsigned int* __restrict__ raw_a, const unsigned int* __restrict__ raw_i,
                                                              unsigned int* __restrict__ flat_a, unsigned int* __restrict__ flat_i)
{
    if (!st->vl_scan) return;
    const int which = blockIdx.y, seg = blockIdx.x % LIST_SEGS;
    const unsigned int n = st->vl_seg_n[which * LIST_SEGS + seg], off = st->vl_seg_off[which * LIST_SEGS + seg];
    const unsigned int* __restrict__ raw = (which ? raw_i : raw_a) + (size_t)seg * c.seg_cap;
    unsigned int* __restrict__ flat = (which ? flat_i : flat_a) + off;
    for (unsigned int t = (blockIdx.x / LIST_SEGS) * blockDim.x + threadIdx.x; t < n; t += blockDim.x * (gridDim.x / LIST_SEGS)) flat[t] = raw[t];
}

__global__ __launch_bounds__(MAP_THREADS) void k_index_list(const DevState* __restrict__ st, const float4* __restrict__ pc, const float2* __restrict__ tm, Cam c, int time,
                                                            const unsigned int* __restrict__ list, unsigned long long* __restrict__ keys, const Hot* __restrict__ hot = nullptr)
{
    const int fl = FIRST_LIVE(c);
    float T[12];
#pragma unroll
    for (int k = 0; k < 12; k++) T[k] = st->pose_inv[k];
    const unsigned int n = min(st->vl_n[0], c.seg_cap * LIST_SEGS);
#ifndef INDEX_U
#define INDEX_U 1
#endif
    constexpr int U = INDEX_U;
    const unsigned int stride = blockDim.x * gridDim.x;
    for (unsigned int t = blockIdx.x * blockDim.x + threadIdx.x; t < n; t += U * stride) {
        unsigned int i[U];
        bool in[U];
#pragma unroll
        for (int u = 0; u < U; u++) { const unsigned int tt = t + u * stride; in[u] = tt < n; i[u] = list[in[u] ? tt : t]; }
        float lastT[U];
        float4 p4[U];
#pragma unroll
        for (int u = 0; u < U; u++) { lastT[u] = hot ? hot[i[u]].tm.y : ld_once(&tm[i[u]]).y; p4[u] = hot ? hot[i[u]].pc : ld_once(&pc[i[u]]); }
#pragma unroll
        for (int u = 0; u < U; u++) asm volatile("" ::"v"(lastT[u]), "v"(p4[u].x), "v"(p4[u].y), "v"(p4[u].z));
#pragma unroll
        for (int u = 0; u < U; u++) {
            if (!in[u] || (float)time - lastT[u] > (float)c.timeDelta) continue;
            const v3 p = xf_point(T, v3m(p4[u].x, p4[u].y, p4[u].z));
            if (p.z > c.maxDepth || p.z < 0) continue;
            const float uu = ((c.fx * p.x) / p.z) + c.cx, v = ((c.fy * p.y) / p.z) + c.cy;
            if (!(uu >= 0 && uu < (float)c.w && v >= 0 && v < (float)c.h)) continue;
            const int px_ = point_pixel(uu), py_ = point_pixel(v);
            if (px_ < 0 || py_ < 0) continue;
            key_min(&keys[py_ * c.w + px_], make_key(p.z, key_id(c, i[u], fl)));
        }
    }
}

__global__ __launch_bounds__(MAP_THREADS) void k_clean_view(DevState* st, Cam c, int time, float4* __restrict__ pc, const float4* __restrict__ nr, float2* __restrict__ tm,
                                                            const float4* __restrict__ tap, const unsigned int* __restrict__ list)
{
    float T[12];
#pragma unroll
    for (int k = 0; k < 12; k++) T[k] = st->pose_inv[k];
    __shared__ unsigned int s_cand[2 * MAP_THREADS];
    __shared__ unsigned int s_n;
    const unsigned int n = min(st->vl_n[0], c.seg_cap * LIST_SEGS);
    const unsigned int* __restrict__ seg_list = list;
    const unsigned int stride = blockDim.x * gridDim.x;
    int dead = 0;
    if (threadIdx.x == 0) s_n = 0;
    __syncthreads();
    for (unsigned int t0 = blockIdx.x * blockDim.x; t0 < n; t0 += stride) {
        const unsigned int t = t0 + threadIdx.x;
        bool cand = false;
        unsigned int i = 0;
        if (t < n) {
            i = seg_list[t];
            const float2 tt = ld_once(&tm[i]);
            const float4 p4 = ld_once(&pc[i]);
            asm volatile("" ::"v"(tt.y), "v"(p4.x), "v"(p4.y), "v"(p4.z), "v"(p4.w));
            const float wv = tt.y;
            if (wv > DEAD_TIME && !(wv > 0.f && (float)time - wv > (float)c.timeDelta)) {
                if (!((float)time - wv > (float)c.timeDelta)) {
                    const v3 p = xf_point(T, v3m(p4.x, p4.y, p4.z));
                    if (p.z > 0.f) {
                        const float u = ((c.fx * p.x) / p.z) + c.cx, v = ((c.fy * p.y) / p.z) + c.cy;
                        cand = ((float)time - wv < (float)c.timeDelta && u > 0 && v > 0 && u < (float)c.w && v < (float)c.h);
                    }
                }
                if (!cand) {
                    int test = 1;
                    if (wv == -1 || (((float)time - wv) > 20 && p4.w < c.conf)) test = 0;
                    if (wv > 0 && (float)time - wv > (float)c.timeDelta) test = 1;
                    if (!test) {
                        float4 q4 = p4;
                        q4.w = -1.0f;
                        pc[i] = q4;
                        tm[i] = make_float2(tt.x, DEAD_TIME);
                        dead++;
                    }
                }
            }
        }
        {
            const unsigned long long m = __ballot(cand);
            unsigned int base = 0;
            const int lane = threadIdx.x & 63;
            if (m) {
                const int leader = __ffsll((long long)m) - 1;
                if (lane == leader) base = atomicAdd(&s_n, (unsigned int)__popcll(m));
                base = __shfl(base, leader, 64);
            }
            if (cand) s_cand[base + __popcll(m & ((1ull << lane) - 1ull))] = i;
        }
        __syncthreads();
        const bool last_round = t0 + stride >= n;
        unsigned int have = s_n;
        unsigned int done = 0;
        while (have - done >= blockDim.x || (last_round && have > done)) {
            const unsigned int k = done + threadIdx.x;
            if (k < have) {
                const unsigned int j = s_cand[k];
                const float2 tt = tm[j];
                const float4 p4 = pc[j];
                float lastT = tt.y;
                if (!clean_test(T, c, time, p4, nr[j], tt.x, lastT, tap)) {
                    float4 q4 = p4;
                    q4.w = -1.0f;
                    pc[j] = q4;
                    tm[j] = make_float2(tt.x, DEAD_TIME);
                    dead++;
                }
            }
            done += blockDim.x;
            if (done > have) done = have;
        }
        __syncthreads();
        if (done > 0 && done < have) {
            const unsigned int rest = have - done;
            unsigned int v = 0;
            if (threadIdx.x < rest) v = s_cand[done + threadIdx.x];
            __syncthreads();
            if (threadIdx.x < rest) s_cand[threadIdx.x] = v;
        }
        if (threadIdx.x == 0) s_n = have - done;
        __syncthreads();
    }
    dead = wave_sum_i(dead);
    if ((threadIdx.x & 63) == 0 && dead) atomicAdd(&st->n_dead, dead);
}

struct alignas(16) RvRec { float qx, qy, qz, nx, ny, nz, r2; unsigned int id; int x0, y0, bw, excl; int s01, s23, i01, i23; };
#define RV_SLOTS 512
struct Hot;
struct CleanArgs { float4* pc_rw; float2* tm_rw; const float4* tap; int nf_blocks; const uint32_t* assoc; const float4* mpc; const float4* mnr; int* flags; int* block_counts; Hot* hot; };
__device__ __forceinline__ void new_flags_body(DevState* st, const float* __restrict__ pose_inv_ex, const Cam& c, int time, const uint32_t* __restrict__ assoc, const float4* __restrict__ mpc,
                                               const float4* __restrict__ mnr, const float4* __restrict__ tap, int* __restrict__ flags, int* __restrict__ block_counts, int bid);
#ifndef WALK_MIN_WAVES
#define WALK_MIN_WAVES 1
#endif
template <bool LDSMIN, bool CLEAN>
__global__ __launch_bounds__(MAP_THREADS, CLEAN ? WALK_MIN_WAVES : 1) void k_raster_view(DevState* st, const float4* __restrict__ pc, const float4* __restrict__ nr, const float2* __restrict__ tm, Cam c,
                                                             int time, int maxTime, unsigned int want, const unsigned int* __restrict__ list_a, const unsigned int* __restrict__ list_i,
                                                             unsigned long long* __restrict__ key_splat, unsigned long long* __restrict__ key_ids,
                                                             unsigned long long* __restrict__ key_both, int earlyz, int ids_step, CleanArgs ca, const DevState* __restrict__ stc)
{
    const int fl = FIRST_LIVE(c);
    if (CLEAN && (int)blockIdx.x < ca.nf_blocks) { new_flags_body(st, stc->pose_inv, c, time, ca.assoc, ca.mpc, ca.mnr, ca.tap, ca.flags, ca.block_counts, (int)blockIdx.x); return; }
    const unsigned int rblk = CLEAN ? blockIdx.x - (unsigned int)ca.nf_blocks : blockIdx.x, rgrid = CLEAN ? gridDim.x - (unsigned int)ca.nf_blocks : gridDim.x;
    __shared__ RvRec recs[MAP_THREADS / 64][64];
    __shared__ unsigned int s_tag[LDSMIN ? MAP_THREADS / 64 : 1][LDSMIN ? RV_SLOTS : 1];
    __shared__ unsigned long long s_key[LDSMIN ? MAP_THREADS / 64 : 1][LDSMIN ? RV_SLOTS : 1];
    float T[12];
#pragma unroll
    for (int k = 0; k < 12; k++) T[k] = stc->pose_inv[k];
    const int lane = threadIdx.x & 63, wid = threadIdx.x >> 6;
    if (LDSMIN) {
#pragma unroll
        for (int q = 0; q < RV_SLOTS / 64; q++) { s_tag[wid][q * 64 + lane] = 0u; s_key[wid][q * 64 + lane] = ~0ull; }
    }
    const bool dual = (want & LIST_DUAL) != 0;
    const unsigned int na = min(stc->vl_n[0], c.seg_cap * LIST_SEGS), n = na + (((want & LIST_IDS) || dual) ? min(stc->vl_n[1], c.seg_cap * LIST_SEGS) : 0u);
    const unsigned int* __restrict__ seg_a = list_a;
    const unsigned int* __restrict__ seg_i = list_i;
    const float reach = __uint_as_float(stc->r_max_bits) * 1.41421356f * 1.001f;
    const unsigned int stride = blockDim.x * rgrid;
    int dead = 0;
#ifndef WALK_PIPE
#define WALK_PIPE 1
#endif
    const unsigned int tfirst = rblk * blockDim.x + wid * 64 + lane;
    auto entry_of = [&](unsigned int t_) -> unsigned int { return t_ < n ? (t_ < na ? seg_a[t_] : seg_i[t_ - na]) : 0u; };
    unsigned int i_cur = 0, i_nxt = 0;
    float4 p4_cur = make_float4(0.f, 0.f, 0.f, 0.f);
    float2 tt_cur = make_float2(0.f, 0.f);
    const Hot* const hot = CLEAN ? ca.hot : (const Hot*)nullptr;
    if (WALK_PIPE) {
        i_cur = entry_of(tfirst);
        i_nxt = entry_of(tfirst + stride);
        if (tfirst < n) { p4_cur = hot ? hot[i_cur].pc : ld_once(&pc[i_cur]); if (tfirst < na || dual) tt_cur = hot ? hot[i_cur].tm : ld_once(&tm[i_cur]); }
    }
    for (unsigned int t0 = rblk * blockDim.x + wid * 64; t0 < n; t0 += stride) {
        const unsigned int t = t0 + lane;
        int area = 0;
        RvRec R;
        R.bw = 1;
        unsigned int i_pre = 0;
        float4 p4_pre = make_float4(0.f, 0.f, 0.f, 0.f);
        float2 tt_pre = make_float2(0.f, 0.f);
        if (WALK_PIPE) {
            i_pre = i_cur; p4_pre = p4_cur; tt_pre = tt_cur;
            const unsigned int tn = t + stride;
            i_cur = i_nxt;
            if (tn < n) {
                p4_cur = hot ? hot[i_nxt].pc : ld_once(&pc[i_nxt]);
                tt_cur = (tn < na || dual) ? (hot ? hot[i_nxt].tm : ld_once(&tm[i_nxt])) : make_float2(0.f, 0.f);
            }
            i_nxt = entry_of(tn + stride);
        }
        if (t < n) {
            const unsigned int i = WALK_PIPE ? i_pre : (t < na ? seg_a[t] : seg_i[t - na]);
            float4 p4 = WALK_PIPE ? p4_pre : (hot ? hot[i].pc : ld_once(&pc[i]));
            const float2 tt = WALK_PIPE ? tt_pre : ((t < na || dual) ? (hot ? hot[i].tm : ld_once(&tm[i])) : make_float2(0.f, 0.f));
            const float lastT = tt.y;
            asm volatile("" ::"v"(lastT), "v"(p4.x), "v"(p4.y), "v"(p4.z), "v"(p4.w));
            float4 n4c = make_float4(0.f, 0.f, 0.f, 0.f);
            bool have_n = false;
            if (CLEAN && t < na) {
                const float wv = tt.y;
                if (wv > DEAD_TIME && !(wv > 0.f && (float)time - wv > (float)c.timeDelta)) {
                    bool cand = false;
                    if (!((float)time - wv > (float)c.timeDelta)) {
                        const v3 p = xf_point(T, v3m(p4.x, p4.y, p4.z));
                        if (p.z > 0.f) {
                            const float u = ((c.fx * p.x) / p.z) + c.cx, v = ((c.fy * p.y) / p.z) + c.cy;
                            cand = ((float)time - wv < (float)c.timeDelta && u > 0 && v > 0 && u < (float)c.w && v < (float)c.h);
                        }
                    }
                    int test = 1;
                    if (cand) {
                        n4c = hot ? hot[i].nr : ld_once(&nr[i]);
                        have_n = true;
                        float lt2 = tt.y;
                        test = clean_test(T, c, time, p4, n4c, tt.x, lt2, ca.tap);
                    } else {
                        if (wv == -1 || (((float)time - wv) > 20 && p4.w < c.conf)) test = 0;
                        if (wv > 0 && (float)time - wv > (float)c.timeDelta) test = 1;
                    }
                    if (!test) {
                        p4.w = -1.0f;
                        ca.pc_rw[i] = p4;
                        ca.tm_rw[i] = make_float2(tt.x, DEAD_TIME);
                        if (ca.hot) { ca.hot[i].pc = p4; ca.hot[i].tm = make_float2(tt.x, DEAD_TIME); }
                        dead++;
                    }
                }
            }
            unsigned int flags = 0;
            if (!(p4.w < c.conf)) {
                const v3 q = xf_point(T, v3m(p4.x, p4.y, p4.z));
                if (q.z > 0.f && may_touch_image(reach, q, c)) {
                    if (dual) {
                        if (!(q.z > c.maxDepth)) {
                            const bool act = !((float)time - lastT > (float)c.timeDelta || lastT > (float)maxTime);
                            const bool old = !(0.f - lastT > (float)c.timeDelta || lastT > (float)(time - c.timeDelta));
                            if (act || old) {
                                const float u = ((c.fx * q.x) / q.z) + c.cx, v = ((c.fy * q.y) / q.z) + c.cy;
                                if (u >= 0 && u <= (float)c.w && v >= 0 && v <= (float)c.h) flags |= (act ? LIST_SPLAT : 0u) | (old ? LIST_IDS : 0u);
                            }
                        }
                    } else {
                    if ((want & LIST_IDS) && (p4.w > c.conf) && (q.z / c.maxDepth > 0.01f)) flags |= LIST_IDS;
                    if ((want & LIST_SPLAT) && !(q.z > c.maxDepth) && !((float)time - lastT > (float)c.timeDelta || lastT > (float)maxTime)) {
                        const float u = ((c.fx * q.x) / q.z) + c.cx, v = ((c.fy * q.y) / q.z) + c.cy;
                        if (u >= 0 && u <= (float)c.w && v >= 0 && v <= (float)c.h) flags |= LIST_SPLAT;
                    }
                    }
                }
            }
            if (flags) {
                SurfGeo G;
                surfel_geo(T, p4, (CLEAN && have_n) ? n4c : (hot ? hot[i].nr : ld_once(&nr[i])), dual ? (i | LIST_SPLAT) : (i | flags), c, G);
                int sx0 = G.sx0, sx1 = G.sx1, sy0 = G.sy0, sy1 = G.sy1, ix0, ix1, iy0, iy1;
                bool do_i = dual ? (G.do_s && (flags & LIST_IDS)) : surfel_id_box(G, i | flags, c, ix0, ix1, iy0, iy1);
                const bool do_s = dual ? (G.do_s && (flags & LIST_SPLAT)) : G.do_s;
                if (dual) { ix0 = sx0; ix1 = sx1; iy0 = sy0; iy1 = sy1; }
                int lattice = 0;
                if (do_i && ids_step > 1) {
                    const int lx0 = ((ix0 + ids_step - 1) / ids_step) * ids_step, lx1 = (ix1 / ids_step) * ids_step;
                    const int ly0 = ((iy0 + ids_step - 1) / ids_step) * ids_step, ly1 = (iy1 / ids_step) * ids_step;
                    if (lx0 > lx1 || ly0 > ly1) do_i = false;
                    else { ix0 = lx0; ix1 = lx1; iy0 = ly0; iy1 = ly1; lattice = !do_s; }
                }
                if (do_s || do_i) {
                    if (!do_s) { sx0 = 1; sx1 = 0; sy0 = 1; sy1 = 0; }
                    if (!do_i) { ix0 = 1; ix1 = 0; iy0 = 1; iy1 = 0; }
                    const int x0 = do_s && do_i ? min(sx0, ix0) : (do_s ? sx0 : ix0), x1 = do_s && do_i ? max(sx1, ix1) : (do_s ? sx1 : ix1);
                    const int y0 = do_s && do_i ? min(sy0, iy0) : (do_s ? sy0 : iy0), y1 = do_s && do_i ? max(sy1, iy1) : (do_s ? sy1 : iy1);
                    if (x1 >= x0 && y1 >= y0) {
                        const int nx_ = lattice ? (x1 - x0) / ids_step + 1 : x1 - x0 + 1, ny_ = lattice ? (y1 - y0) / ids_step + 1 : y1 - y0 + 1;
                        area = nx_ * ny_;
                        R.qx = G.q.x; R.qy = G.q.y; R.qz = G.q.z; R.nx = G.nn.x; R.ny = G.nn.y; R.nz = G.nn.z; R.r2 = G.r * G.r; R.id = CLEAN ? i : key_id(c, i, fl);
                        R.x0 = x0; R.y0 = y0; R.bw = nx_ | (lattice << 16);
                        R.s01 = (sx0 & 0xFFFF) | (sx1 << 16); R.s23 = (sy0 & 0xFFFF) | (sy1 << 16);
                        R.i01 = (ix0 & 0xFFFF) | (ix1 << 16); R.i23 = (iy0 & 0xFFFF) | (iy1 << 16);
                    }
                }
            }
        }
        int incl = area;
#pragma unroll
        for (int o = 1; o < 64; o <<= 1) { const int u = __shfl_up(incl, o, 64); if (lane >= o) incl += u; }
        const int excl = incl - area, total = __shfl(incl, 63, 64);
        if (total == 0) continue;
        R.excl = excl;
        if (area) recs[wid][lane] = R;
        int jlo = 0;
        for (int g0 = 0; g0 < total; g0 += 64) {
            while (jlo < 63 && __builtin_amdgcn_readlane(incl, __builtin_amdgcn_readfirstlane(jlo)) <= g0) jlo++;
            const int g = g0 + lane;
            int mine = jlo;
            for (int j = jlo + 1; j < 64; j++) {
                const int ej = __builtin_amdgcn_readlane(excl, __builtin_amdgcn_readfirstlane(j));
                if (ej >= g0 + 64) break;
                if (g >= ej) mine = j;
            }
            if (g >= total) continue;
            const RvRec* rp = &recs[wid][mine];
            const float4 a = *reinterpret_cast<const float4*>(&rp->qx), b = *reinterpret_cast<const float4*>(&rp->ny);
            const int4 bx = *reinterpret_cast<const int4*>(&rp->x0), rg = *reinterpret_cast<const int4*>(&rp->s01);
            const int k = g - bx.w;
            const int bwv = bx.z & 0xFFFF, stp = (bx.z >> 16) ? ids_step : 1;
            const int row = (int)(((float)k + 0.5f) * __builtin_amdgcn_rcpf((float)bwv)), col = k - row * bwv;
            const int px = bx.x + col * stp, py = bx.y + row * stp;
            Disc d;
            d.q = v3m(a.x, a.y, a.z); d.n = v3m(a.w, b.x, b.y); d.r2 = b.z;
            const unsigned int id = __float_as_uint(b.w);
            float z;
            if (!disc_hit(d, (float)px + 0.5f, (float)py + 0.5f, c, z)) continue;
            const int sx0 = (short)(rg.x & 0xFFFF), sx1 = rg.x >> 16, sy0 = (short)(rg.y & 0xFFFF), sy1 = rg.y >> 16;
            const int ix0 = (short)(rg.z & 0xFFFF), ix1 = rg.z >> 16, iy0 = (short)(rg.w & 0xFFFF), iy1 = rg.w >> 16;
            const bool in_s = px >= sx0 && px <= sx1 && py >= sy0 && py <= sy1 && (z >= -c.maxDepth && z <= c.maxDepth);
            const bool in_i = px >= ix0 && px <= ix1 && py >= iy0 && py <= iy1 && (dual ? (z >= -c.maxDepth && z <= c.maxDepth) : (z > 0 && z <= c.maxDepth)) &&
                              (ids_step <= 1 || (px % ids_step == 0 && py % ids_step == 0));
            if (!in_s && !in_i) continue;
            if (dual && in_s && in_i) {
                key_min(key_splat + (py * c.w + px), make_key(z, id));
                key_min(key_ids + (py * c.w + px), make_key(z, id));
                continue;
            }
            const int tsel = in_s && in_i ? 0 : (in_s ? 1 : 2);
            unsigned long long* addr = (tsel == 0 ? key_both : (tsel == 1 ? key_splat : key_ids)) + (py * c.w + px);
            const unsigned long long key = make_key(z, id);
            if (LDSMIN) {
                const unsigned int tag = ((unsigned int)(py * c.w + px) << 2 | (unsigned int)tsel) + 1u;
                const int slot = ((py & 15) << 5) | ((px & 15) << 1) | (tsel != 0);
                const unsigned int old = atomicCAS(&s_tag[wid][slot], 0u, tag);
                if (old == 0u || old == tag) { atomicMin(&s_key[wid][slot], key); continue; }
            }
            if (earlyz && !(key < __hip_atomic_load(addr, __ATOMIC_RELAXED, __HIP_MEMORY_SCOPE_AGENT))) continue;
            key_min(addr, key);
        }
        if (LDSMIN) {
#pragma unroll
            for (int q = 0; q < RV_SLOTS / 64; q++) {
                const int sl = q * 64 + lane;
                const unsigned int tag = s_tag[wid][sl];
                if (tag) {
                    const unsigned long long key = s_key[wid][sl];
                    const unsigned int pt = tag - 1u, tsel = pt & 3u, pix = pt >> 2;
                    key_min((tsel == 0 ? key_both : (tsel == 1 ? key_splat : key_ids)) + pix, key);
                    s_tag[wid][sl] = 0u; s_key[wid][sl] = ~0ull;
                }
            }
        }
    }
    if (CLEAN) {
        dead = wave_sum_i(dead);
        if (lane == 0 && dead) atomicAdd(&st->n_dead, dead);
    }
}

static void launch_raster_view(ifx* h, const char* name, const Cam& c, unsigned int want, int ids_step, bool lds, const CleanArgs* clean)
{
    const CleanArgs ca = clean ? *clean : CleanArgs{nullptr, nullptr, nullptr, 0, nullptr, nullptr, nullptr, nullptr, nullptr, nullptr};
    const dim3 grid(ca.nf_blocks + (h->opt_view_blocks > 0 ? h->opt_view_blocks : 4 * LIST_BLOCKS));
    auto go = [&](auto kernel) {
        LAUNCH(h, name, grid, dim3(MAP_THREADS), kernel, h->d_state, (const float4*)h->pc, (const float4*)h->nr, (const float2*)h->tm, c, h->tick, h->tick, want, h->list_v, h->list_vi,
               h->key_splat, h->key_ids, h->key_both, h->opt_raster_earlyz, ids_step, ca, (const DevState*)h->d_state);
    };
    if (clean) go(k_raster_view<false, true>);
    else if (lds) go(k_raster_view<true, false>);
    else go(k_raster_view<false, false>);
}

static void raster_pass(ifx* h, const float* d_pose_inv, int time, int maxTime, unsigned int want, int32_t* ids_out, bool frame_sums = false, int part = 0, int old_target = 0,
                        bool fold_finish = false, int resolve_ids_step = 1, bool raw_ids = false)
{
    unsigned int want_r = want;
    Cam c = make_cam(h);
    if (part == 0) { c.srank = 0; c.sn = 1; }
    const bool quad = h->opt_id_rule && !h->own && (want & LIST_IDS);
    if (quad) want_r &= ~LIST_IDS;
    if (part != 2 && want_r) {
        const int tw = cdiv(h->w, TILE), th = cdiv(h->h, TILE);
        const bool want_tiles = h->opt_raster_tiles < 0 ? (h->P >= 1000000) : (h->opt_raster_tiles != 0);
        if (want_tiles && !h->tile_recs && hipMalloc(&h->tile_recs, (size_t)h->list_seg_cap * LIST_SEGS * 32) != hipSuccess) h->tile_recs = nullptr;
        const bool tiled = want_tiles && tw * th <= TILE_MAX && tw <= 255 && th <= 255 && h->tile_pairs && h->tile_recs;
        LAUNCH(h, "cull_raster", dim3(MAP_BLOCKS), dim3(MAP_THREADS), k_cull_raster, h->d_state, d_pose_inv, (const float4*)h->pc, (const float2*)h->tm, c, time, maxTime, want_r,
               h->list_a, tiled ? h->tile_n : (unsigned int*)nullptr, tw * th);
        if (tiled) {
            TileArgs ta;
            ta.tile_n = h->tile_n; ta.tile_off = h->tile_n + TILE_MAX; ta.tile_fill = h->tile_n + 2 * TILE_MAX; ta.blk_off = h->tile_n + 3 * TILE_MAX; ta.overflow = (int*)(h->tile_n + 4 * TILE_MAX + 8);
            ta.tile_box = h->tile_box; ta.pairs = h->tile_pairs; ta.recs = (TileRec*)h->tile_recs; ta.pair_cap = h->tile_pair_cap; ta.tw = tw; ta.th = th;
            LAUNCH(h, "tile_count", dim3(LIST_BLOCKS), dim3(MAP_THREADS), k_tile_count, (const DevState*)h->d_state, d_pose_inv, (const float4*)h->pc, (const float4*)h->nr, c, h->list_a, ta);
            LAUNCH(h, "tile_scan", dim3(1), dim3(256), k_tile_scan, ta);
            LAUNCH(h, "tile_fill", dim3(LIST_BLOCKS), dim3(MAP_THREADS), k_tile_fill, c, h->list_a, ta);
            LAUNCH(h, "tile_raster", dim3(tw * th + h->tile_pair_cap / TILE_CHUNK), dim3(TILE_THREADS), k_tile_raster, (const DevState*)h->d_state, d_pose_inv, (const float4*)h->pc, (const float4*)h->nr, c, ta, h->key_splat,
                   h->key_ids, h->key_both);
            LAUNCH(h, "raster_list", dim3(LIST_BLOCKS), dim3(MAP_THREADS), k_raster_list, h->d_state, d_pose_inv, (const float4*)h->pc, (const float4*)h->nr, c, h->list_a, h->key_splat,
                   h->key_ids, h->key_both, 0, (const int*)ta.overflow);
        } else
            LAUNCH(h, "raster_list", dim3(LIST_BLOCKS), dim3(MAP_THREADS), k_raster_list, h->d_state, d_pose_inv, (const float4*)h->pc, (const float4*)h->nr, c, h->list_a, h->key_splat,
                   h->key_ids, h->key_both, 0, (const int*)nullptr);
    }
    if (part == 1) return;
    if (quad)
        LAUNCH(h, "raster_quad", dim3(MAP_BLOCKS), dim3(MAP_THREADS), k_raster_quad<1>, (const DevState*)h->d_state, d_pose_inv, (const float4*)h->pc, (const float4*)h->nr,
               (const float4*)h->votes, c, h->key_ids, resolve_ids_step);
    if ((want & LIST_SPLAT) && old_target) {
        const bool old = old_target == 1;
        LAUNCH(h, old ? "splat_resolve_old" : "splat_resolve_act", dim3(cdiv(h->w, 32), cdiv(h->h, 8)), dim3(32, 8), k_splat_resolve, h->d_state, d_pose_inv, h->key_splat,
               (const float4*)h->pc, (const float4*)h->nr, (const float2*)h->col, (const float2*)h->tm, c, h->rgb, h->depth_filt, (float4*)(old ? h->old_vertex : h->act_vertex),
               (float4*)(old ? h->old_normal : h->act_normal), (uchar4*)(old ? h->old_image : h->act_image), (uchar4*)(old ? h->old_inst : h->act_inst),
               old ? h->old_time : h->act_time, (float4*)nullptr, (float4*)nullptr, (uchar4*)nullptr, h->key_ids, h->key_both, (int32_t*)nullptr, (int*)nullptr, FinishFold());
        LAUNCH(h, "raster_finish", dim3(1), dim3(256), k_raster_finish, h->d_state, (const uchar4*)h->pred_image, h->w, h->h, 0, h->ids_after, (const float4*)h->votes, h->cap, 10, h->d_list_ctr, ifx_idmap(h));
        return;
    }
    if (want & LIST_SPLAT) {
        FinishFold ff = FinishFold();
        if (fold_finish && frame_sums && !h->own && h->w >= 20 && h->h >= 20) {
            ff.acc = &h->d_state->fold_acc[0][0]; ff.total = &h->d_state->fold_total;
            ff.votes = (const float4*)h->votes; ff.cap = h->cap; ff.ds = 10; ff.rw = h->w / 20; ff.rh = h->h / 20;
        }
        FrameOut fo = FrameOut{nullptr, nullptr, 0};
        if (ff.acc && h->result_fold_traj && h->opt_fold_result) {
            fo.out = h->h_result; fo.traj = h->result_fold_traj; fo.fold_total = ff.rw * ff.rh;
            ff.total = nullptr;
            h->result_folded = 1;
        }
        if (raw_ids) c.raw_slots = 2;
        LAUNCH(h, "splat_resolve", dim3(cdiv(h->w, 32), cdiv(h->h, 8)), dim3(32, 8), k_splat_resolve, h->d_state, d_pose_inv, h->key_splat, (const float4*)h->pc,
               (const float4*)h->nr, (const float2*)h->col, (const float2*)h->tm, c, h->rgb, h->depth_filt, (float4*)h->pred_vertex, (float4*)h->pred_normal,
               (uchar4*)h->pred_image, (uchar4*)h->pred_inst, h->pred_time, (float4*)h->fill_vertex, (float4*)h->fill_normal, (uchar4*)h->fill_image, h->key_ids,
               h->key_both, (want & LIST_IDS) ? ids_out : (int32_t*)nullptr, (int*)nullptr, ff, (float*)nullptr, resolve_ids_step, (const int32_t*)nullptr, fo,
               raw_ids ? (const Hot*)h->frame_hot : (const Hot*)nullptr);
        if (ff.acc) return;
    } else if (want & LIST_IDS) LAUNCH(h, "ids_resolve", dim3(cdiv(h->P, 256)), dim3(256), k_ids_resolve, h->key_ids, h->P, ids_out);
    const int seg = frame_sums && (want & LIST_IDS);
    const int ds = 10, nseg = seg ? cdiv(cdiv(h->w, ds) * cdiv(h->h, ds), 256) : 0;
    LAUNCH(h, "raster_finish", dim3(1 + nseg), dim3(256), k_raster_finish, h->d_state, (const uchar4*)h->pred_image, h->w, h->h, (want & LIST_SPLAT) ? 1 : 0, h->ids_after,
           (const float4*)h->votes, h->cap, ds, h->d_list_ctr, ifx_idmap(h));
}
static void splat_pass(ifx* h, const float* d_pose_inv, int time, int maxTime) { raster_pass(h, d_pose_inv, time, maxTime, LIST_SPLAT, nullptr); }

static void ids_pass(ifx* h, const float* d_pose_inv, int mode, int32_t* out)
{
    if (h->opt_id_rule && !h->own) {
// ... 93 lines not shown
        const uint8_t c0 = cc[0], c1 = cc[1], c2 = cc[2];
        float4 vcs[9], nrs[9];
#pragma unroll
        for (int q = 0; q < 9; q++) {
            const int a = q / 3, b = q - 3 * a;
            const int kk = ys[b] * c.w + xs[a];
            vcs[q] = index_vc[kk];
            nrs[q] = index_nr[kk];
        }
        asm volatile("" ::"v"(d_c), "v"(d_l), "v"(d_u), "v"(d_r), "v"(d_d), "v"(f_c), "v"(f_l), "v"(f_u), "v"(f_r), "v"(f_d), "v"(cur[0]), "v"(cur[1]), "v"(cur[2]), "v"(cur[3]), "v"(cur[4]),
                     "v"(cur[5]), "v"(cur[6]), "v"(cur[7]), "v"(cur[8]));
        asm volatile("" ::"v"(vcs[0].x), "v"(vcs[1].x), "v"(vcs[2].x), "v"(vcs[3].x), "v"(vcs[4].x), "v"(vcs[5].x), "v"(vcs[6].x), "v"(vcs[7].x), "v"(vcs[8].x), "v"(nrs[0].x),
                     "v"(nrs[1].x), "v"(nrs[2].x), "v"(nrs[3].x), "v"(nrs[4].x), "v"(nrs[5].x), "v"(nrs[6].x), "v"(nrs[7].x), "v"(nrs[8].x));
        v3 vl = v3m((x - c.cx) * d_c * ifx_, (y - c.cy) * d_c * ify_, d_c);
        bool nb = !(d_l == 0 || d_u == 0 || d_r == 0 || d_d == 0);
        if (nb && vl.z > 0 && vl.z <= c.maxDepth) {
            v3 vg = xf_point(pose, vl);
            v3 vf = v3m((x - c.cx) * f_c * ifx_, (y - c.cy) * f_c * ify_, f_c);
            v3 nl;
            {
                const v3 xf = v3m((x + 1 - c.cx) * f_r * ifx_, (y - c.cy) * f_r * ify_, f_r), xb = v3m((x - 1 - c.cx) * f_l * ifx_, (y - c.cy) * f_l * ify_, f_l);
                const v3 yf = v3m((x - c.cx) * f_d * ifx_, (y + 1 - c.cy) * f_d * ify_, f_d), yb = v3m((x - c.cx) * f_u * ifx_, (y - 1 - c.cy) * f_u * ify_, f_u);
                const v3 del_x = ((xb + vf) * 0.5f) - ((xf + vf) * 0.5f), del_y = ((yb + vf) * 0.5f) - ((yf + vf) * 0.5f);
                nl = normalized(cross(del_x, del_y));
            }
            v3 ng = xf_dir(pose, nl);
            mpc[k] = make_float4(vg.x, vg.y, vg.z, confidence_fn(x, y, c.cx, c.cy, weighting));
            mcol[k] = encode_color(c0 / 255.0f, c1 / 255.0f, c2 / 255.0f);
            mnr[k] = make_float4(ng.x, ng.y, ng.z, get_radius(vf.z, nl.z, ifx_, ify_));
            float xl = (x - c.cx) * ifx_, yl = (y - c.cy) * ify_;
            float lambda = sqrtf(xl * xl + yl * yl + 1);
            v3 ray = v3m(xl, yl, 1);
            float rayLen = norm(ray);
            float bestDist = 1000;
            uint32_t best = 0;
            int counter = 0, best_q = 0;
#pragma unroll
            for (int q = 0; q < 9; q++) {
                if (!((vis_x >> (q / 3)) & (vis_y >> (q % 3)) & 1u)) continue;
                if (cur[q] > 0u && (!akey || (__float_as_uint(vcs[q].x) | __float_as_uint(vcs[q].y) | __float_as_uint(vcs[q].z) | __float_as_uint(vcs[q].w)) != 0u)) {
                    const float4 vc = vcs[q];
                    if (fabsf((vc.z * lambda) - (vl.z * lambda)) < 0.05f) {
                        float dist = norm(cross(ray, v3m(vc.x, vc.y, vc.z))) / rayLen;
                        const float4 nrm = nrs[q];
                        v3 nn = v3m(nrm.x, nrm.y, nrm.z);
                        float cang = dot(nn, nl) / (norm(nn) * norm(nl));
                        if (dist < bestDist && (fabsf(nrm.z) < 0.75f || cang > 0.87758256189f)) { counter++; bestDist = dist; best = cur[q]; best_q = q; }
                    }
                }
            }
            if (akey) {
                if (counter > 0) akey[by * ((c.w + 1) / 2) + bx] = ((unsigned long long)__float_as_uint(bestDist) << 32) | (unsigned int)best_q;
                res = ASSOC_NEW;
            } else if (counter > 0) {
                res = best;
                const int lb = local_slot(c, st->count, best, fl);
                if (lb >= 0) atomicMin(&upd_owner[lb], (uint32_t)(i * c.h + j));
            } else res = ASSOC_NEW;
        }
    }
    assoc[k] = res;
}

__global__ void k_assoc_decode(const DevState* __restrict__ st, const unsigned long long* __restrict__ akey, const uint32_t* __restrict__ index_id, Cam c, int time,
                               uint32_t* __restrict__ assoc, uint32_t* __restrict__ upd_owner, const int32_t* __restrict__ own_slot = nullptr, int32_t* __restrict__ assoc_slot = nullptr)
{
    const int fl = FIRST_LIVE(c);
    const int bx = blockIdx.x * blockDim.x + threadIdx.x, by = blockIdx.y * blockDim.y + threadIdx.y;
    const int par = time % 2, i = 2 * bx + par, j = 2 * by + par;
    if (i >= c.w || j >= c.h) return;
    const unsigned long long key = akey[by * ((c.w + 1) / 2) + bx];
    if (key == IFX_KEY_EMPTY) return;
    const int q = (int)(key & 0xFu), a = q / 3, b = q - 3 * a;
    const float x = (float)i + 0.5f, y = (float)j + 0.5f;
    const int xs[3] = {clampi((int)floorf(x - 1.0f), 0, c.w - 1), clampi((int)floorf(x - 0.5f), 0, c.w - 1), clampi((int)floorf(x + 0.5f), 0, c.w - 1)};
    const int ys[3] = {clampi((int)floorf(y - 1.0f), 0, c.h - 1), clampi((int)floorf(y - 0.5f), 0, c.h - 1), clampi((int)floorf(y + 0.5f), 0, c.h - 1)};
    const uint32_t best = index_id[ys[b] * c.w + xs[a]];
    assoc[j * c.w + i] = best;
    const int lb = own_slot ? own_slot_of(c, own_slot[ys[b] * c.w + xs[a]], best) : local_slot(c, st->count, best, fl);
    if (assoc_slot) assoc_slot[j * c.w + i] = lb;
    if (lb >= 0) atomicMin(&upd_owner[lb], (uint32_t)(i * c.h + j));
}

__global__ void k_fuse_update(DevState* __restrict__ st, const uint32_t* __restrict__ assoc, const float4* __restrict__ mpc, const float4* __restrict__ mnr,
                              const float* __restrict__ mcol, Cam c, int time, uint32_t* __restrict__ upd_owner, float4* __restrict__ pc, float4* __restrict__ nr,
                              float2* __restrict__ col, float2* __restrict__ tm, const int32_t* __restrict__ assoc_slot = nullptr, Hot* __restrict__ hot = nullptr)
{
    const int fl = FIRST_LIVE(c);
    const int par = time % 2, i = 2 * (blockIdx.x * blockDim.x + threadIdx.x) + par, j = 2 * (blockIdx.y * blockDim.y + threadIdx.y) + par;
    if (i >= c.w || j >= c.h) return;
    int k = j * c.w + i;
    const uint32_t gid = assoc[k];
    if (gid >= ASSOC_NEW) return;
    const int li = assoc_slot ? assoc_slot[k] : local_slot(c, st->count, gid, fl);
    if (li < 0 || li >= st->count) return;
    const uint32_t id = (uint32_t)li;
    if (upd_owner[id] != (uint32_t)(i * c.h + j)) return;
    upd_owner[id] = 0xFFFFFFFFu;
    float4 p = hot ? hot[id].pc : pc[id], n = hot ? hot[id].nr : nr[id], mp = mpc[k], mn = mnr[k];
    const float2 cl0 = col[id], t0_ = hot ? hot[id].tm : tm[id];
    const float mc = mcol[k];
    float c_k = p.w, a = mp.w;
    if (mn.w < (1.0f + 0.5f) * n.w) {
        p.x = ((c_k * p.x) + (a * mp.x)) / (c_k + a);
        p.y = ((c_k * p.y) + (a * mp.y)) / (c_k + a);
        p.z = ((c_k * p.z) + (a * mp.z)) / (c_k + a);
        p.w = c_k + a;
        float2 cl = cl0;
        float oc[3], nc[3];
        decode_color(cl.x, oc);
        decode_color(mc, nc);
        cl.x = encode_color(((c_k * oc[0]) + (a * nc[0])) / (c_k + a), ((c_k * oc[1]) + (a * nc[1])) / (c_k + a), ((c_k * oc[2]) + (a * nc[2])) / (c_k + a));
        col[id] = cl;
        float t0 = ((c_k * n.x) + (a * mn.x)) / (c_k + a), t1 = ((c_k * n.y) + (a * mn.y)) / (c_k + a), t2 = ((c_k * n.z) + (a * mn.z)) / (c_k + a);
        float t3 = ((c_k * n.w) + (a * mn.w)) / (c_k + a);
        v3 nn = normalized(v3m(t0, t1, t2));
        nr[id] = make_float4(nn.x, nn.y, nn.z, t3);
        if (hot) hot[id].nr = make_float4(nn.x, nn.y, nn.z, t3);
        if (t3 > 0.f && t3 < 1e30f && __float_as_uint(t3) > st->r_max_bits) atomicMax(&st->r_max_bits, __float_as_uint(t3));
        pc[id] = p;
    } else {
        p.w = c_k + a;
        pc[id] = p;
    }
    float2 t = t0_;
    t.y = (float)time;
    tm[id] = t;
    if (hot) { hot[id].pc = p; hot[id].tm = t; }
}

__device__ inline int clean_test(const float* T, const Cam& c, int time, float4 p4, float4 n4, float initT, float& lastT, const float4* __restrict__ tap)
{
    int test = 1;
    v3 lp = xf_point(T, v3m(p4.x, p4.y, p4.z));
    float x = ((c.fx * lp.x) / lp.z) + c.cx, y = ((c.fy * lp.y) / lp.z) + c.cy;
    int count = 0, zCount = 0;
    float wv = lastT;
    if ((float)time - wv < (float)c.timeDelta && lp.z > 0 && x > 0 && y > 0 && x < (float)c.w && y < (float)c.h) {
        v3 ln = normalized(xf_dir(T, v3m(n4.x, n4.y, n4.z)));
        const bool flat = fabsf(ln.z) > 0.85f;
        int tx[IFX_MAX_TAPS], ty[IFX_MAX_TAPS];
        window_taps(x / (float)c.w, (float)c.w, c.w, tx);
        window_taps(y / (float)c.h, (float)c.h, c.h, ty);
        int mx[4], my[4];
#pragma unroll
        for (int q = 0; q < 4; q++) {
            mx[q] = 0; my[q] = 0;
#pragma unroll
            for (int a = 0; a < IFX_MAX_TAPS; a++) { mx[q] += (tx[a] == tx[0] + q) ? 1 : 0; my[q] += (ty[a] == ty[0] + q) ? 1 : 0; }
        }
        if (mx[3] | my[3]) {
            for (int a = 0; a < 4; a++)
                for (int b = 0; b < 4; b++) {
                    const int wgt = mx[a] * my[b];
                    if (!wgt) continue;
                    const float4 e = tap[min(ty[0] + b, c.h - 1) * c.w + min(tx[0] + a, c.w - 1)];
                    if (e.z == 0.f) continue;
                    const float ez = fabsf(e.z);
                    const bool stable = e.w > 0.f, now = e.z < 0.f;
                    const float dx = e.x - lp.x, dy = e.y - lp.y;
                    if (fabsf(e.w) < initT && stable && ez > lp.z && ez - lp.z < 0.01f && sqrtf(dx * dx + dy * dy) < n4.w * 1.4f) count += wgt;
                    if (now && stable && ez > lp.z && ez - lp.z > 0.01f && flat) zCount += wgt;
                }
            mx[0] = mx[1] = mx[2] = 0;
        }
        float4 t[9];
#pragma unroll
        for (int a = 0; a < 3; a++)
#pragma unroll
            for (int b = 0; b < 3; b++) t[a * 3 + b] = tap[min(ty[0] + b, c.h - 1) * c.w + min(tx[0] + a, c.w - 1)];
#pragma unroll
        for (int k = 0; k < 9; k++) {
            const int wgt = mx[k / 3] * my[k % 3];
            const float4 e = t[k];
            if (wgt == 0 || e.z == 0.f) continue;
            const float ez = fabsf(e.z);
            const bool stable = e.w > 0.f, now = e.z < 0.f;
            const float dx = e.x - lp.x, dy = e.y - lp.y;
            if (fabsf(e.w) < initT && stable && ez > lp.z && ez - lp.z < 0.01f && sqrtf(dx * dx + dy * dy) < n4.w * 1.4f) count += wgt;
            if (now && stable && ez > lp.z && ez - lp.z > 0.01f && flat) zCount += wgt;
        }
    }
    if (count > 8 || zCount > 4) test = 0;
    if (wv == -2) wv = (float)time;
    if (wv == -1 || (((float)time - wv) > 20 && p4.w < c.conf)) test = 0;
    if (wv > 0 && (float)time - wv > (float)c.timeDelta) test = 1;
    lastT = wv;
    return test;
}



__device__ __forceinline__ void new_flags_body(DevState* st, const float* __restrict__ pose_inv_ex, const Cam& c, int time, const uint32_t* __restrict__ assoc, const float4* __restrict__ mpc,
                                               const float4* __restrict__ mnr, const float4* __restrict__ tap, int* __restrict__ flags, int* __restrict__ block_counts, int bid)
{
    __shared__ int lds[4][2];
    const int P = c.w * c.h, ord0 = bid * NEW_PER_BLOCK + threadIdx.x * 4;
    const float* Ti = pose_inv_ex ? pose_inv_ex : st->pose_inv;
    float T[12];
#pragma unroll
    for (int k = 0; k < 12; k++) T[k] = Ti[k];
    int keep[4], cnt = 0, own = 0;
#pragma unroll
    for (int u = 0; u < 4; u++) {
        const int ord = ord0 + u;
        keep[u] = 0;
        if (ord < P) {
            const int i = ord / c.h, j = ord - i * c.h, k = j * c.w + i;
            if (assoc[k] == ASSOC_NEW) {
                float lastT = -2.f;
                const float4 m4 = mpc[k];
// ... 71 lines not shown
        const int ord = ord0 + u, i = ord / c.h, j = ord - i * c.h, k = j * c.w + i;
        const int n = count0 + rankO++;
        const unsigned int vp = vpos++;
        if (n >= cap) { over = true; continue; }
        if (to_view && vp < c.seg_cap * LIST_SEGS) list_v[vp] = (unsigned int)n;
        const float4 m4 = mpc[k], n4 = mnr[k];
        pc[n] = m4;
        nr[n] = n4;
        { const float rad = n4.w; if (rad > 0.f && rad < 1e30f && __float_as_uint(rad) > rmax0) atomicMax(&st->r_max_bits, __float_as_uint(rad)); }
        col[n] = make_float2(mcol[k], 0.f);
        tm[n] = make_float2((float)time, (float)time);
        if (hot) { Hot r; r.pc = m4; r.nr = n4; r.tm = make_float2((float)time, (float)time); r.pad0 = make_float2(0.f, 0.f); r.pad1 = make_float4(0.f, 0.f, 0.f, 0.f); hot[n] = r; }
        ic[n] = make_float4((float)i + 0.5f, (float)j + 0.5f, (float)tick, inst_gt ? (float)inst_gt[j * c.w + i] : -2.f);
        for (int q = 0; q < 12; q++) VOTE4(votes, n, q) = make_float4(0.f, 0.f, 0.f, 0.f);
        labels[n] = -1;
        seq[n] = sq;
    }
    if (over) { st->overflow = 1; st->vl_valid = 0; }
    if (bid != nblocks - 1) return;
    if (tid == 0) {
        const int tg = s_base[0] + s_wave[0][0] + s_wave[1][0] + s_wave[2][0] + s_wave[3][0], to = s_base[1] + blk_total;
        int nc = count0 + to;
        bool ovf = false;
        if (nc > cap) { nc = cap; ovf = true; }
        if (seq0 + (unsigned int)tg < seq0 || seq0 + (unsigned int)tg > 0xFFF00000u) ovf = true;
        st->n_new = nc - count0;
        st->count = nc;
        {
            int f = st->first_live;
            while (f < count0) {
                const float wv = tm[f].y;
                if (wv > DEAD_TIME && !age_rule_gone(wv, pc[f].w, time, c)) break;
                f++;
            }
            st->first_live = f;
        }
        st->next_seq = seq0 + (unsigned int)tg;
        if (ovf) st->overflow = 1;
        if (to_view) {
            const unsigned int vn = vln0 + (unsigned int)(nc - count0);
            if (vn > c.seg_cap * LIST_SEGS) st->vl_valid = 0; else st->vl_n[0] = vn;
        }
    }
}
__global__ void __launch_bounds__(256) k_append_scan(DevState* st, Cam c, int time, int tick, const int* __restrict__ flags, const int* __restrict__ block_counts, int nblocks,
                                                     const float4* __restrict__ mpc, const float4* __restrict__ mnr, const float* __restrict__ mcol, int cap, float4* __restrict__ pc,
                                                     float4* __restrict__ nr, float2* __restrict__ col, float2* __restrict__ tm, float4* __restrict__ ic, float4* __restrict__ votes,
                                                     const uint8_t* __restrict__ inst_gt, unsigned int* __restrict__ list_v, int32_t* __restrict__ labels, uint32_t* __restrict__ seq,
                                                     Hot* __restrict__ hot = nullptr)
{
    append_scan_body(st, c, time, tick, flags, block_counts, nblocks, mpc, mnr, mcol, cap, pc, nr, col, tm, ic, votes, inst_gt, list_v, labels, seq, (int)threadIdx.x, (int)blockIdx.x, hot);
}

__global__ void k_alive_flags(const DevState* __restrict__ st, const float2* __restrict__ tm, int* __restrict__ flags, int cap)
{
    int i = blockIdx.x * blockDim.x + threadIdx.x;
    if (i >= cap) return;
    flags[i] = (i < st->count && tm[i].y > DEAD_TIME) ? 1 : 0;
}
__global__ void k_compact_scatter(const int* __restrict__ flags, const int* __restrict__ rank, int cap, const float4* __restrict__ pc, const float4* __restrict__ nr,
                                  const float2* __restrict__ col, const float2* __restrict__ tm, const float4* __restrict__ ic, const float4* __restrict__ votes,
                                  const int32_t* __restrict__ labels, float4* __restrict__ pc2, float4* __restrict__ nr2, float2* __restrict__ col2,
                                  float2* __restrict__ tm2, float4* __restrict__ ic2, float4* __restrict__ votes2, int32_t* __restrict__ labels2,
                                  const uint32_t* __restrict__ seq, uint32_t* __restrict__ seq2)
{
    int i = blockIdx.x * blockDim.x + threadIdx.x;
    if (i >= cap || !flags[i]) return;
    int d = rank[i];
    pc2[d] = pc[i]; nr2[d] = nr[i]; col2[d] = col[i]; tm2[d] = tm[i]; ic2[d] = ic[i];
    if (labels2) labels2[d] = labels[i];
    seq2[d] = seq[i];
    for (int q = 0; q < 12; q++) VOTE4(votes2, d, q) = VOTE4(votes, i, q);
}
__global__ void k_compact_count(DevState* st, const int* total)
{
    if (threadIdx.x == 0) { st->count = *total; st->n_dead = 0; st->vl_valid = 0; st->first_live = 0; }
}

static void ids_pass(ifx* h, const float* d_pose_inv, int mode, int32_t* out);
int ifx_compact_enqueue(ifx* h, int refresh_ids)
{
    h->ids_view_ok = 0;
    h->hot_valid = 0;
    ifx_vlist_reap(h);
    int n = h->cap;
    LAUNCH(h, "alive_flags", dim3(cdiv(n, 256)), dim3(256), k_alive_flags, h->d_state, (const float2*)h->tm, h->scan_flags, n);
    ifx_scan_exclusive(h, h->scan_flags, n, h->scan_out, &h->d_state->seg_counts[1]);
    LAUNCH(h, "compact_scatter", dim3(cdiv(n, 256)), dim3(256), k_compact_scatter, h->scan_flags, h->scan_out, n, (const float4*)h->pc, (const float4*)h->nr,
           (const float2*)h->col, (const float2*)h->tm, (const float4*)h->ic, (const float4*)h->votes, (const int32_t*)h->labels, (float4*)h->pc2, (float4*)h->nr2,
           (float2*)h->col2, (float2*)h->tm2, (float4*)h->ic2, (float4*)h->votes2, h->labels2, (const uint32_t*)h->seq, h->seq2);
    LAUNCH(h, "compact_count", dim3(1), dim3(64), k_compact_count, h->d_state, &h->d_state->seg_counts[1]);
    std::swap(h->pc, h->pc2); std::swap(h->nr, h->nr2); std::swap(h->col, h->col2); std::swap(h->tm, h->tm2); std::swap(h->ic, h->ic2); std::swap(h->votes, h->votes2); std::swap(h->labels, h->labels2); std::swap(h->seq, h->seq2);
    if (refresh_ids && !h->own) { ids_pass(h, nullptr, 0, h->ids_after); h->ids_full_valid = 1; }
    return IFX_OK;
}

static void fuse_pass(ifx* h, const float* d_pose, float weighting, int time, int part = 0, const int32_t* own_slot = nullptr, Hot* hot = nullptr)
{
    if (!hot) h->hot_valid = 0;
    Cam c = make_cam(h);
    dim3 b(32, 8), g(cdiv(cdiv(h->w, 2), 32), cdiv(cdiv(h->h, 2), 8));
    if (part != 2)
        LAUNCH(h, "associate", g, b, k_associate, h->d_state, d_pose, weighting, h->dm, h->dmf, h->rgb, h->index_id, (const float4*)h->index_vc, (const float4*)h->index_nr, c, time,
               h->assoc_target, (float4*)h->meas_pc, (float4*)h->meas_nr, h->meas_col, h->upd_owner, (const uint8_t*)h->assoc_vis, part == 1 ? h->assoc_key : (unsigned long long*)nullptr);
    if (part == 1) return;
    const bool slots = part == 2 && own_slot && h->own_slot_img;
    if (part == 2) LAUNCH(h, "assoc_decode", g, b, k_assoc_decode, h->d_state, (const unsigned long long*)h->assoc_key, h->index_id, c, time, h->assoc_target, h->upd_owner,
                          slots ? own_slot : (const int32_t*)nullptr, slots ? h->own_slot_img + 3 * (size_t)h->P : (int32_t*)nullptr);
    LAUNCH(h, "fuse_update", g, b, k_fuse_update, h->d_state, h->assoc_target, (const float4*)h->meas_pc, (const float4*)h->meas_nr, h->meas_col, c, time, h->upd_owner,
           (float4*)h->pc, (float4*)h->nr, (float2*)h->col, (float2*)h->tm, slots ? (const int32_t*)(h->own_slot_img + 3 * (size_t)h->P) : (const int32_t*)nullptr, hot);
}

__global__ __launch_bounds__(256) void k_deform(const DevState* __restrict__ st, const float* __restrict__ pose_inv_ex, const float* __restrict__ graph, int nodes, int is_fern,
                                                 int time, Cam c, const float4* __restrict__ depth_v4, float4* __restrict__ pc, float4* __restrict__ nr, float2* __restrict__ tm)
{
    extern __shared__ float g[];
    for (int k = threadIdx.x; k < nodes * 16; k += blockDim.x) g[k] = graph[k];
    __syncthreads();
    if (blockIdx.x == 0 && threadIdx.x == 0) const_cast<DevState*>(st)->vl_valid = 0;
    const float* T = pose_inv_ex ? pose_inv_ex : st->pose_inv;
    const int n = st->count;
    for (int i = blockIdx.x * blockDim.x + threadIdx.x; i < n; i += blockDim.x * gridDim.x) {
        float2 t2 = tm[i];
        if (!(t2.y > DEAD_TIME) || t2.x == (float)time) continue;
        float4 p4 = pc[i], n4 = nr[i];
        const int K = 4, LOOK = 20;
        int nearNodes[LOOK];
        float nearDists[LOOK];
#pragma unroll
        for (int q = 0; q < LOOK; q++) { nearNodes[q] = -1; nearDists[q] = 16777216.0f; }
        const int poseTime = (int)t2.x;
        int foundIndex = 0, imin = 0, imax = nodes - 1, imid = (imin + imax) / 2;
        while (imax >= imin) {
            imid = (imin + imax) / 2;
            const int nodeTime = (int)g[imid * 16 + 15];
            if (nodeTime < poseTime) imin = imid + 1;
            else if (nodeTime > poseTime) imax = imid - 1;
            else break;
        }
        imin = min(imin, nodes - 1);
        const int cmax = imax < 0 ? 0 : imax;
        const int nodeMin = (int)g[imin * 16 + 15], nodeMid = (int)g[imid * 16 + 15], nodeMax = (int)g[cmax * 16 + 15];
        if (abs(nodeMin - poseTime) <= abs(nodeMid - poseTime) && abs(nodeMin - poseTime) <= abs(nodeMax - poseTime)) foundIndex = imin;
        else if (abs(nodeMid - poseTime) <= abs(nodeMin - poseTime) && abs(nodeMid - poseTime) <= abs(nodeMax - poseTime)) foundIndex = imid;
        else foundIndex = cmax;
        if (foundIndex == nodes) foundIndex = nodes - 1;
        int nearNodeIndex = 0, distanceBack = 0;
        const v3 p = v3m(p4.x, p4.y, p4.z);
        for (int j = foundIndex; j >= 0; j--) {
            const v3 d = p - v3m(g[j * 16], g[j * 16 + 1], g[j * 16 + 2]);
            nearNodes[nearNodeIndex] = j;
            nearDists[nearNodeIndex] = sqrtf(dot(d, d));
            nearNodeIndex++;
            if (++distanceBack == LOOK / 2) break;
        }
        for (int j = foundIndex + 1; j < nodes; j++) {
            const v3 d = p - v3m(g[j * 16], g[j * 16 + 1], g[j * 16 + 2]);
            nearNodes[nearNodeIndex] = j;
            nearDists[nearNodeIndex] = sqrtf(dot(d, d));
            nearNodeIndex++;
            if (++distanceBack == LOOK) break;
        }
        for (int a = 0; a < LOOK - 1; ++a)
            for (int b = a + 1; b < LOOK; ++b)
                if (nearDists[b] < nearDists[a]) {
                    const float t = nearDists[a]; nearDists[a] = nearDists[b]; nearDists[b] = t;
                    const int u = nearNodes[a]; nearNodes[a] = nearNodes[b]; nearNodes[b] = u;
                }
        const float dMax = nearDists[K];
        float wgt[K], weightSum = 0;
        for (int j = 0; j < K; j++) {
            const float* nd = &g[nearNodes[j] * 16];
            const v3 d = p - v3m(nd[0], nd[1], nd[2]);
            const float u = 1.0f - (sqrtf(dot(d, d)) / dMax);
            wgt[j] = u * u;
            weightSum += wgt[j];
        }
        for (int j = 0; j < K; j++) wgt[j] /= weightSum;
        v3 newPos = v3m(0, 0, 0), newNorm = v3m(0, 0, 0);
        for (int q = 0; q < K; q++) {
            const float* nd = &g[nearNodes[q] * 16];
            const v3 gp = v3m(nd[0], nd[1], nd[2]);
            const float R[9] = {nd[3], nd[6], nd[9], nd[4], nd[7], nd[10], nd[5], nd[8], nd[11]};
            const v3 tr = v3m(nd[12], nd[13], nd[14]);
            const v3 qd = p - gp;
            const v3 rq = v3m(R[0] * qd.x + R[1] * qd.y + R[2] * qd.z, R[3] * qd.x + R[4] * qd.y + R[5] * qd.z, R[6] * qd.x + R[7] * qd.y + R[8] * qd.z);
            newPos = newPos + ((rq + gp) + tr) * wgt[q];
            const float c00 = R[4] * R[8] - R[5] * R[7], c01 = R[5] * R[6] - R[3] * R[8], c02 = R[3] * R[7] - R[4] * R[6];
// ... 53 lines not shown
    if (threadIdx.x != 0) return;
    for (int k = 0; k < 16; k++) st->pose[k] = st->lc[6 + k];
    pose_inverse(st->pose, st->pose_inv);
    st->vl_valid = 0;
}

static void launch_new_flags_count(ifx* h, const float* d_pose_inv, const Cam& c, int time)
{
    LAUNCH(h, "new_flags_count", dim3(cdiv(h->P, NEW_PER_BLOCK)), dim3(256), k_new_flags_count, h->d_state, d_pose_inv, c, time, h->assoc_target, (const float4*)h->meas_pc,
           (const float4*)h->meas_nr, (const float4*)h->index_tap, h->scan_flags, h->scan_block);
}
static void launch_append_scan(ifx* h, const Cam& c, int time, unsigned int* list, Hot* hot = nullptr)
{
    const int nb_new = cdiv(h->P, NEW_PER_BLOCK);
    LAUNCH(h, "append_scan", dim3(nb_new), dim3(256), k_append_scan, h->d_state, c, time, time, h->scan_flags, h->scan_block, nb_new, (const float4*)h->meas_pc,
           (const float4*)h->meas_nr, h->meas_col, h->cap, (float4*)h->pc, (float4*)h->nr, (float2*)h->col, (float2*)h->tm, (float4*)h->ic, (float4*)h->votes,
           h->inst_gt_on ? (const uint8_t*)h->d_inst_gt : (const uint8_t*)nullptr, list, h->labels, h->seq, hot);
}

static inline void age_epoch_begin(ifx* h, int time) { if (h->age_epoch == INT_MAX) h->age_epoch = time; }
static void clean_pass(ifx* h, const float* d_pose_inv, int time, int part = 0)
{
    age_epoch_begin(h, time);
    h->hot_valid = 0;
    h->last_clean_time = time;
    Cam c = make_cam(h);
    if (part == 0) { c.srank = 0; c.sn = 1; }
    const bool deform = h->graph_nodes > 0 && part != 1;
    if (deform && !h->graph_is_fern) raster_pass(h, d_pose_inv, 0, time - h->cfg.time_delta, LIST_SPLAT, nullptr, false, 0, 1);
    if (part != 2) LAUNCH(h, "cull_clean", dim3(MAP_BLOCKS), dim3(MAP_THREADS), k_cull_clean, h->d_state, d_pose_inv, (const float4*)h->pc, (const float2*)h->tm, c, time, h->key_index,
           h->list_b, h->list_c);
    if (part == 1) return;
    LAUNCH(h, "index_resolve_taps", dim3(cdiv(h->P, 256)), dim3(256), k_index_resolve, h->d_state, d_pose_inv, h->key_index, (const float4*)h->pc, (const float4*)h->nr,
           (const float2*)h->col, (const float2*)h->tm, h->P, (uint32_t*)nullptr, (float4*)nullptr, (float4*)nullptr, (float4*)nullptr, time, h->cfg.confidence,
           (float4*)h->index_tap, c);
    LAUNCH(h, "clean_list", dim3(LIST_BLOCKS), dim3(MAP_THREADS), k_clean_list, h->d_state, d_pose_inv, c, time, (float4*)h->pc, (const float4*)h->nr, (float2*)h->tm,
           (const float4*)h->index_tap, h->list_b, h->list_c);
    if (deform) {
        LAUNCH_SMEM(h, "deform", dim3(MAP_BLOCKS), dim3(256), (size_t)h->graph_nodes * 64, k_deform, h->d_state, d_pose_inv, h->d_graph, h->graph_nodes, h->graph_is_fern, time, c,
                    (const float4*)h->old_vertex, (float4*)h->pc, (float4*)h->nr, (float2*)h->tm);
        h->graph_nodes = 0;
    }
    launch_new_flags_count(h, d_pose_inv, c, time);
    launch_append_scan(h, c, time, h->own ? (unsigned int*)nullptr : h->list_v);
}

__global__ void k_vlist_invalidate(DevState* st) { if (threadIdx.x == 0) st->vl_valid = 0; }
void hs_invalidate_view(ifx* h) { h->ids_view_ok = 0; LAUNCH(h, "vlist_invalidate", dim3(1), dim3(64), k_vlist_invalidate, h->d_state); }
static bool use_view_list(ifx* h) { return h->opt_vlist && h->shard_n <= 1 && !h->own && !h->opt_reference_passes && h->graph_nodes == 0 && !h->view_block && h->tick > 1; }
static bool use_view_list_own(ifx* h) { return h->opt_vlist && h->own && !h->opt_reference_passes && h->graph_nodes == 0 && !h->view_block; }
static void view_scan(ifx* h, int time)
{
    Cam c = make_cam(h);
    c.srank = 0; c.sn = 1;
    LAUNCH(h, "cull_frame", dim3(MAP_BLOCKS), dim3(MAP_THREADS), k_cull_frame, h->d_state, (const float4*)h->pc, (float4*)h->pc, (float2*)h->tm, c, make_planes(c), time, h->list_b, h->list_c,
           h->hot_valid ? (Hot*)h->hot : (Hot*)nullptr,
           std::max(0, std::min(time, h->last_clean_time)));
    LAUNCH(h, "vlist_offsets", dim3(1), dim3(64), k_vlist_offsets, h->d_state, c, (const float2*)h->tm);
    LAUNCH(h, "vlist_concat", dim3(256, 2), dim3(MAP_THREADS), k_vlist_concat, (const DevState*)h->d_state, c, h->list_b, h->list_c, h->list_v, h->list_vi);
}
int ifx_vlist_reap(ifx* h)
{
    if (!h->view_dirty) return IFX_OK;
    h->view_dirty = 0;
    h->ids_view_ok = 0;
    LAUNCH(h, "vlist_decide", dim3(1), dim3(64), k_vlist_decide, h->d_state, h->d_list_ctr, 1);
    view_scan(h, h->last_clean_time);
    return IFX_OK;
}
static void index_list_pass(ifx* h, int time, bool taps)
{
    Cam c = make_cam(h);
    c.srank = 0; c.sn = 1;
    LAUNCH(h, "index_list", dim3(h->opt_index_blocks > 0 ? h->opt_index_blocks : LIST_BLOCKS), dim3(MAP_THREADS), k_index_list, (const DevState*)h->d_state, (const float4*)h->pc, (const float2*)h->tm, c, time, h->list_v, h->key_index, (const Hot*)h->frame_hot);
    if (!taps)
        LAUNCH(h, "index_resolve", dim3(cdiv(h->P, 256)), dim3(256), k_index_resolve, h->d_state, (const float*)nullptr, h->key_index, (const float4*)h->pc, (const float4*)h->nr,
               (const float2*)h->col, (const float2*)h->tm, h->P, h->index_id, (float4*)h->index_vc, (float4*)nullptr, (float4*)h->index_nr, time, h->cfg.confidence, (float4*)nullptr, c,
               (const int32_t*)nullptr, (const Hot*)h->frame_hot);
    else
        LAUNCH(h, "index_resolve_taps", dim3(cdiv(h->P, 256)), dim3(256), k_index_resolve, h->d_state, (const float*)nullptr, h->key_index, (const float4*)h->pc, (const float4*)h->nr,
               (const float2*)h->col, (const float2*)h->tm, h->P, (uint32_t*)nullptr, (float4*)nullptr, (float4*)nullptr, (float4*)nullptr, time, h->cfg.confidence, (float4*)h->index_tap, c,
               (const int32_t*)nullptr, (const Hot*)h->frame_hot);
}

static void view_clean_append(ifx* h, const Cam& c, int time)
{
    h->hot_valid = 0;
    LAUNCH(h, "clean_view", dim3(h->opt_clean_blocks > 0 ? h->opt_clean_blocks : 2 * LIST_BLOCKS), dim3(MAP_THREADS), k_clean_view, h->d_state, c, time, (float4*)h->pc, (const float4*)h->nr, (float2*)h->tm,
           (const float4*)h->index_tap, h->list_v);
    launch_new_flags_count(h, nullptr, c, time);
    launch_append_scan(h, c, time, h->own ? (unsigned int*)nullptr : h->list_v);
}

int ifx_map_frame(ifx* h)
{
    h->clean_raster_pending = 0;
    h->view_frame = 0;
    h->ids_view_ok = 0;
    age_epoch_begin(h, h->tick);
    if (use_view_list(h)) {
        Cam c = make_cam(h);
        c.srank = 0; c.sn = 1;
        const int time = h->tick;
        const bool fused = h->opt_clean_raster && !h->opt_compact_every_frame && h->last_compact_tick != h->tick && h->opt_raster_tiles <= 0 && !h->opt_raster_lds &&
                           h->cfg.confidence > fmaxf(1.f, h->frame_weight_mult);
        Hot* hot = nullptr;
        if (fused && h->opt_hot) {
            if (!h->hot && hipMalloc(&h->hot, (size_t)h->cap * sizeof(Hot)) != hipSuccess) { h->hot = nullptr; (void)hipGetLastError(); }
            if (h->hot && !h->hot_valid) {
                LAUNCH(h, "hot_rebuild", dim3(MAP_BLOCKS), dim3(MAP_THREADS), k_hot_rebuild, (const DevState*)h->d_state, (const float4*)h->pc, (const float4*)h->nr, (const float2*)h->tm, (Hot*)h->hot);
                h->hot_valid = 1;
            } else if (h->hot && h->opt_hot_verify)
                LAUNCH(h, "hot_verify", dim3(MAP_BLOCKS), dim3(MAP_THREADS), k_hot_verify, h->d_state, (const float4*)h->pc, (const float4*)h->nr, (const float2*)h->tm, (Hot*)h->hot);
            hot = (Hot*)h->hot;
        }
        if (!hot) h->hot_valid = 0;
        h->frame_hot = hot;
        if (h->view_scan_tick != time) view_scan(h, time);
        index_list_pass(h, time, false);
        fuse_pass(h, nullptr, 0.f, time, 0, nullptr, hot);
        index_list_pass(h, time, true);
        h->clean_raster_pending = fused ? 1 : 0;
        if (!fused) view_clean_append(h, c, time);
        h->view_frame = 1; h->view_dirty = 1; h->last_clean_time = time;
        if (h->opt_compact_every_frame) ifx_compact_enqueue(h, 0);
        h->ids_pending = 1;
        return IFX_OK;
    }
    h->frame_hot = nullptr;
    if (h->opt_vlist && !h->own && h->shard_n <= 1) hs_invalidate_view(h);
    index_pass(h, nullptr, h->tick, true);
    fuse_pass(h, nullptr, 0.f, h->tick);
    if (h->opt_reference_passes) {
        index_pass(h, nullptr, h->tick);
        ids_pass(h, nullptr, 1, h->ids_tmp);
        ids_pass(h, nullptr, 0, h->ids_tmp);
    }
    clean_pass(h, nullptr, h->tick);
    h->view_block = 0;
    if (h->opt_compact_every_frame) ifx_compact_enqueue(h, 0);
    h->ids_pending = 1;
    return IFX_OK;
}

int ifx_map_predict_loop_closure(ifx* h)
{
    Cam c = make_cam(h);
    c.srank = 0; c.sn = 1;
    const bool by_view = use_view_list(h);
    if (by_view) {
        view_scan(h, h->tick);
        h->view_scan_tick = h->tick;
        launch_raster_view(h, "raster_view_lc", c, LIST_SPLAT | LIST_DUAL, 1, false, nullptr);
    } else {
    LAUNCH(h, "cull_raster", dim3(MAP_BLOCKS), dim3(MAP_THREADS), k_cull_raster, h->d_state, (const float*)nullptr, (const float4*)h->pc, (const float2*)h->tm, c, h->tick, h->tick,
           LIST_SPLAT | LIST_DUAL, h->list_a, (unsigned int*)nullptr, 0);
    LAUNCH(h, "raster_list", dim3(LIST_BLOCKS), dim3(MAP_THREADS), k_raster_list, h->d_state, (const float*)nullptr, (const float4*)h->pc, (const float4*)h->nr, c, h->list_a, h->key_splat,
           h->key_ids, h->key_both, 1, (const int*)nullptr);
    }
    {
        ResolveTarget ta, to;
        ta.keys = h->key_splat; ta.pv = (float4*)h->act_vertex; ta.pn = (float4*)h->act_normal; ta.pimg = (uchar4*)h->act_image; ta.pinst = (uchar4*)h->act_inst; ta.ptime = h->act_time;
        to.keys = h->key_ids; to.pv = (float4*)h->old_vertex; to.pn = (float4*)h->old_normal; to.pimg = (uchar4*)h->old_image; to.pinst = (uchar4*)h->old_inst; to.ptime = h->old_time;
        LAUNCH(h, "splat_resolve_lc", dim3(cdiv(h->w, 32), cdiv(h->h, 8), 2), dim3(32, 8), k_splat_resolve_pair, (const DevState*)h->d_state, (const float4*)h->pc, (const float4*)h->nr,
               (const float2*)h->col, (const float2*)h->tm, c, (const uint8_t*)h->rgb, (const uint16_t*)h->depth_filt, ta, to);
    }
    if (!by_view)
        LAUNCH(h, "raster_finish", dim3(1), dim3(256), k_raster_finish, h->d_state, (const uchar4*)h->pred_image, h->w, h->h, 0, h->ids_after, (const float4*)h->votes, h->cap, 10, h->d_list_ctr, ifx_idmap(h));
    return IFX_OK;
}

int ifx_map_predict(ifx* h)
{
    const unsigned int want = LIST_SPLAT | (h->ids_pending ? LIST_IDS : 0u);
    const unsigned int want_walk = (h->opt_id_rule && !h->own) ? (want & ~LIST_IDS) : want;
    const bool tiles = h->opt_raster_tiles > 0;
    if (h->view_frame && !(h->opt_compact_every_frame || h->last_compact_tick == h->tick) && !tiles) {
        Cam c = make_cam(h);
        c.srank = 0; c.sn = 1;
        const int ids_step = (h->opt_lazy_ids && !h->ids_full_hint && (want & LIST_IDS)) ? 10 : 1;
        h->ids_full_hint = 0;
        h->ids_full_valid = ids_step == 1;
        h->ids_sparse_frame = ids_step > 1;
        h->ids_view_ok = ids_step > 1;
        if (h->clean_raster_pending) {
            h->clean_raster_pending = 0;
            const int nb_new = cdiv(h->P, NEW_PER_BLOCK);
            CleanArgs ca;
            ca.pc_rw = (float4*)h->pc; ca.tm_rw = (float2*)h->tm; ca.tap = (const float4*)h->index_tap; ca.nf_blocks = nb_new; ca.assoc = h->assoc_target; ca.mpc = (const float4*)h->meas_pc;
            ca.mnr = (const float4*)h->meas_nr; ca.flags = h->scan_flags; ca.block_counts = h->scan_block; ca.hot = (Hot*)h->frame_hot;
            launch_raster_view(h, "clean_raster_view", c, want_walk, ids_step, false, &ca);
            launch_append_scan(h, c, h->tick, h->list_v, (Hot*)h->frame_hot);
            raster_pass(h, nullptr, h->tick, h->tick, want, h->ids_after, true, 2, 0, true, ids_step, true);
        } else {
            launch_raster_view(h, "raster_view", c, want_walk, ids_step, h->opt_raster_lds != 0, nullptr);
            raster_pass(h, nullptr, h->tick, h->tick, want, h->ids_after, true, 2, 0, true, ids_step);
        }
    } else {
        if (h->clean_raster_pending) {
            h->clean_raster_pending = 0;
            Cam cc = make_cam(h);
            cc.srank = 0; cc.sn = 1;
            view_clean_append(h, cc, h->tick);
        }
        raster_pass(h, nullptr, h->tick, h->tick, want, h->ids_after, true);
        if (want & LIST_IDS) { h->ids_full_valid = 1; h->ids_sparse_frame = 0; }
        h->ids_view_ok = 0;
    }
    h->view_frame = 0;
    h->ids_pending = 0;
    return IFX_OK;
}

int ifx_map_sharded_phase(ifx* h, int phase, bool first_frame)
{
    h->hot_valid = 0;
    if (first_frame) {
        if (phase == 0) return ifx_map_init_first(h);
        if (phase == 2) raster_pass(h, nullptr, h->tick, h->tick, LIST_SPLAT, h->ids_after, true, 1);
        if (phase == 3) raster_pass(h, nullptr, h->tick, h->tick, LIST_SPLAT, h->ids_after, true, 2);
        return IFX_OK;
    }
    switch (phase) {
    case 0: index_pass(h, nullptr, h->tick, true, 1); break;
    case 1: index_pass(h, nullptr, h->tick, true, 2); fuse_pass(h, nullptr, 0.f, h->tick); clean_pass(h, nullptr, h->tick, 1); break;
    case 2: clean_pass(h, nullptr, h->tick, 2); raster_pass(h, nullptr, h->tick, h->tick, LIST_SPLAT | LIST_IDS, h->ids_after, true, 1); break;
    case 3: raster_pass(h, nullptr, h->tick, h->tick, LIST_SPLAT | LIST_IDS, h->ids_after, true, 2); break;
    default: return IFX_E_INVALID;
    }
    return IFX_OK;
}

__global__ void k_owner_flags(const DevState* __restrict__ st, const float4* __restrict__ pc, int n_ranks, int rank, int* __restrict__ flags, int cap)
{
    const int i = blockIdx.x * blockDim.x + threadIdx.x;
    if (i >= cap) return;
    int f = 0;
    if (i < st->count) { const float4 p = pc[i]; f = ifx_owner_of_point(p.x, p.y, p.z, n_ranks) == rank; }
    flags[i] = f;
}
__global__ void k_owner_count(DevState* st, const int* total)
{
    if (threadIdx.x == 0) { st->next_seq = (unsigned int)st->count; st->count = *total; st->n_dead = 0; }
}
__global__ void k_fill_in(Cam c, const uint8_t* __restrict__ rgb, const uint16_t* __restrict__ depth_filt, float4* __restrict__ pv, const float4* __restrict__ pn,
                          const uchar4* __restrict__ pimg, float4* __restrict__ fv, float4* __restrict__ fn, uchar4* __restrict__ fimg, const float* __restrict__ pconf)
{
    const int x = blockIdx.x * blockDim.x + threadIdx.x, y = blockIdx.y * blockDim.y + threadIdx.y;
    if (x >= c.w || y >= c.h) return;
    const int k = y * c.w + x;
    float4 vo = pv[k];
    const float4 no = pn[k];
    if (pconf) { vo.w = pconf[k]; pv[k] = vo; }
    const uchar4 io = pimg[k];
    float ifx_ = 1.0f / c.fx, ify_ = 1.0f / c.fy;
    if ((int)io.x + (int)io.y + (int)io.z == 0) fimg[k] = make_uchar4(rgb[k * 3], rgb[k * 3 + 1], rgb[k * 3 + 2], 255);
    else fimg[k] = io;
    float zc = (float)depth_filt[k] / 1000.0f;
    if (vo.z == 0) fv[k] = make_float4(((float)x - c.cx) * zc * ifx_, ((float)y - c.cy) * zc * ify_, zc, 1.f);
    else fv[k] = vo;
    if (no.z == 0) {
        v3 vp = v3m(((float)x - c.cx) * zc * ifx_, ((float)y - c.cy) * zc * ify_, zc);
        int xr = clampi(x + 1, 0, c.w - 1), yd = clampi(y + 1, 0, c.h - 1);
        float zx = (float)depth_filt[y * c.w + xr] / 1000.0f, zy = (float)depth_filt[yd * c.w + x] / 1000.0f;
        v3 vx = v3m(((float)(x + 1) - c.cx) * zx * ifx_, ((float)y - c.cy) * zx * ify_, zx);
        v3 vy = v3m(((float)x - c.cx) * zy * ifx_, ((float)(y + 1) - c.cy) * zy * ify_, zy);
        v3 nn = normalized(cross(vx - vp, vy - vp));
        fn[k] = make_float4(nn.x, nn.y, nn.z, 1.f);
    } else fn[k] = no;
}

static void owner_filter(ifx* h)
{
// ... 52 lines not shown
        case 4: h->own_ids_lat = 0; raster_pass(h, nullptr, time, time, LIST_SPLAT, h->ids_after, false, 1); break;
        case 5:
            LAUNCH(h, "splat_resolve", g2, b2, k_splat_resolve, h->d_state, (const float*)nullptr, h->key_splat, (const float4*)h->pc, (const float4*)h->nr, (const float2*)h->col,
                   (const float2*)h->tm, c, h->rgb, h->depth_filt, (float4*)h->pred_vertex, (float4*)h->pred_normal, (uchar4*)h->pred_image, (uchar4*)h->pred_inst, h->pred_time,
                   (float4*)nullptr, (float4*)nullptr, (uchar4*)nullptr, h->key_ids, h->key_both, (int32_t*)nullptr, (int*)nullptr, FinishFold(), h->pred_conf);
            break;
        case 6:
            LAUNCH(h, "fill_in", g2, b2, k_fill_in, c, (const uint8_t*)h->rgb, (const uint16_t*)h->depth_filt, (float4*)h->pred_vertex, (const float4*)h->pred_normal,
                   (const uchar4*)h->pred_image, (float4*)h->fill_vertex, (float4*)h->fill_normal, (uchar4*)h->fill_image, (const float*)h->pred_conf);
            LAUNCH(h, "raster_finish", dim3(1), dim3(256), k_raster_finish, h->d_state, (const uchar4*)h->pred_image, h->w, h->h, 1, h->ids_after, (const float4*)h->votes, h->cap, 10, h->d_list_ctr, ifx_idmap(h),
                   (int*)nullptr, h->pred_tail);
            break;
        default: break;
        }
        return IFX_OK;
    }
    switch (phase) {
    case 300:
        LAUNCH(h, "cull_raster", dim3(MAP_BLOCKS), dim3(MAP_THREADS), k_cull_raster, h->d_state, (const float*)nullptr, (const float4*)h->pc, (const float2*)h->tm, c, time, time,
               LIST_SPLAT | LIST_DUAL, h->list_a, (unsigned int*)nullptr, 0);
        LAUNCH(h, "raster_list", dim3(LIST_BLOCKS), dim3(MAP_THREADS), k_raster_list, h->d_state, (const float*)nullptr, (const float4*)h->pc, (const float4*)h->nr, c, h->list_a, h->key_splat,
               h->key_ids, h->key_both, 1, (const int*)nullptr);
        break;
    case 301:
        for (int old = 0; old < 2; old++)
            LAUNCH(h, old ? "splat_resolve_old" : "splat_resolve_act", g2, b2, k_splat_resolve, h->d_state, (const float*)nullptr, old ? h->key_ids : h->key_splat, (const float4*)h->pc,
                   (const float4*)h->nr, (const float2*)h->col, (const float2*)h->tm, c, h->rgb, h->depth_filt, (float4*)(old ? h->old_vertex : h->act_vertex),
                   (float4*)(old ? h->old_normal : h->act_normal), (uchar4*)(old ? h->old_image : h->act_image), (uchar4*)(old ? h->old_inst : h->act_inst),
                   old ? h->old_time : h->act_time, (float4*)nullptr, (float4*)nullptr, (uchar4*)nullptr, h->key_ids, h->key_both, (int32_t*)nullptr, (int*)nullptr, FinishFold());
        LAUNCH(h, "raster_finish", dim3(1), dim3(256), k_raster_finish, h->d_state, (const uchar4*)h->pred_image, h->w, h->h, 0, h->ids_after, (const float4*)h->votes, h->cap, 10, h->d_list_ctr, ifx_idmap(h),
               (int*)nullptr, (int*)nullptr);
        break;
    case 0:
        age_epoch_begin(h, time);
        c.age_epoch = h->age_epoch;
        h->view_frame = 0;
        h->ids_view_ok = 0;
        if (h->own_need_decide) {
            LAUNCH(h, "vlist_decide", dim3(1), dim3(64), k_vlist_decide, h->d_state, h->d_list_ctr, 0);
            h->own_need_decide = 0;
        }
        h->own_fast = 0; h->own_fast_raster = 0;
        if (use_view_list_own(h)) {
            if (h->view_scan_tick != time) view_scan(h, time);
            h->view_frame = 1;
            if (!h->own_slot_img && hipMalloc(&h->own_slot_img, (size_t)h->P * 4 * sizeof(int32_t)) != hipSuccess) h->own_slot_img = nullptr;
            h->own_fast = h->own_slot_img != nullptr;
            Cam cl = c;
            if (h->own_fast) { cl.own_n = 0; cl.raw_slots = 1; }
            LAUNCH(h, "index_list", dim3(h->opt_index_blocks > 0 ? h->opt_index_blocks : LIST_BLOCKS), dim3(MAP_THREADS), k_index_list, (const DevState*)h->d_state, (const float4*)h->pc, (const float2*)h->tm, cl, time, h->list_v, h->key_index);
            if (h->own_fast) LAUNCH(h, "own_translate", dim3(cdiv(h->P, 256)), dim3(256), k_own_translate, h->key_index, h->P, (const uint32_t*)h->seq, h->own_slot_img, OWN_GFL(h, h->gfl_index));
            else OWN_FIRST_LIVE(h, h->gfl_index);
        } else {
            if (h->opt_vlist) hs_invalidate_view(h);
            index_pass(h, nullptr, time, true, 1);
            OWN_FIRST_LIVE(h, h->gfl_index);
        }
        break;
    case 1: index_pass(h, nullptr, time, true, 2, h->own_fast ? h->own_slot_img : nullptr); fuse_pass(h, nullptr, 0.f, time, 1); break;
    case 2:
        fuse_pass(h, nullptr, 0.f, time, 2, h->own_fast ? h->own_slot_img : nullptr);
        if (h->view_frame) {
            Cam cl = c;
            if (h->own_fast) { cl.own_n = 0; cl.raw_slots = 1; }
            LAUNCH(h, "index_list", dim3(h->opt_index_blocks > 0 ? h->opt_index_blocks : LIST_BLOCKS), dim3(MAP_THREADS), k_index_list, (const DevState*)h->d_state, (const float4*)h->pc, (const float2*)h->tm, cl, time, h->list_v, h->key_index);
            if (h->own_fast) LAUNCH(h, "own_translate", dim3(cdiv(h->P, 256)), dim3(256), k_own_translate, h->key_index, h->P, (const uint32_t*)h->seq, h->own_slot_img);
        } else clean_pass(h, nullptr, time, 1);
        break;
    case 3:
        LAUNCH(h, "index_resolve_taps", dim3(cdiv(h->P, 256)), dim3(256), k_index_resolve, h->d_state, (const float*)nullptr, h->key_index, (const float4*)h->pc, (const float4*)h->nr,
               (const float2*)h->col, (const float2*)h->tm, h->P, (uint32_t*)nullptr, (float4*)nullptr, (float4*)nullptr, (float4*)nullptr, time, h->cfg.confidence,
               (float4*)h->index_tap, c, (h->own_fast && h->view_frame) ? (const int32_t*)h->own_slot_img : (const int32_t*)nullptr);
        break;
    case 4: {
        const int nb_new = cdiv(h->P, NEW_PER_BLOCK);
        const bool lat = h->opt_own_lazy_ids != 0;
        bool whole_drawn = false;
        h->own_ids_lat = lat;
        const bool fused = h->opt_clean_raster && h->view_frame && h->own_fast && !h->opt_compact_every_frame && h->last_compact_tick != h->tick && h->opt_raster_tiles <= 0 &&
                           h->cfg.confidence > fmaxf(1.f, h->frame_weight_mult);
        if (fused) {
            CleanArgs ca;
            ca.pc_rw = (float4*)h->pc; ca.tm_rw = (float2*)h->tm; ca.tap = (const float4*)h->index_tap; ca.nf_blocks = nb_new; ca.assoc = h->assoc_target; ca.mpc = (const float4*)h->meas_pc;
            ca.mnr = (const float4*)h->meas_nr; ca.flags = h->scan_flags; ca.block_counts = h->scan_block; ca.hot = nullptr;
            LAUNCH(h, "clean_raster_view", dim3(nb_new + (h->opt_view_blocks > 0 ? h->opt_view_blocks : 4 * LIST_BLOCKS)), dim3(MAP_THREADS), (k_raster_view<false, true>), h->d_state, (const float4*)h->pc, (const float4*)h->nr,
                   (const float2*)h->tm, c, time, time, LIST_SPLAT | LIST_IDS, h->list_v, h->list_vi, h->key_splat, h->key_ids, h->key_both, 0, lat ? OWN_LAT_DS : 1, ca, (const DevState*)h->d_state);
            launch_append_scan(h, c, time, h->list_v);
            h->last_clean_time = time;
            h->view_dirty = 1;
            h->own_fast_raster = h->own_fast;
        } else {
        if (h->view_frame)
            LAUNCH(h, "clean_view", dim3(h->opt_clean_blocks > 0 ? h->opt_clean_blocks : 2 * LIST_BLOCKS), dim3(MAP_THREADS), k_clean_view, h->d_state, c, time, (float4*)h->pc, (const float4*)h->nr, (float2*)h->tm,
                   (const float4*)h->index_tap, h->list_v);
        else
        LAUNCH(h, "clean_list", dim3(LIST_BLOCKS), dim3(MAP_THREADS), k_clean_list, h->d_state, (const float*)nullptr, c, time, (float4*)h->pc, (const float4*)h->nr, (float2*)h->tm,
               (const float4*)h->index_tap, h->list_b, h->list_c);
        launch_new_flags_count(h, nullptr, c, time);
        launch_append_scan(h, c, time, h->view_frame ? h->list_v : (unsigned int*)nullptr);
        h->last_clean_time = time;
        if (h->view_frame) h->view_dirty = 1;
        if (h->opt_compact_every_frame) ifx_compact_enqueue(h, 0);
        if (h->view_frame && !(h->opt_compact_every_frame || h->last_compact_tick == h->tick)) {
            Cam cl = make_cam(h);
            cl.srank = 0; cl.sn = 1;
            if (h->own_fast) { cl.own_n = 0; cl.raw_slots = 1; }
            LAUNCH(h, "raster_view", dim3(h->opt_view_blocks > 0 ? h->opt_view_blocks : 4 * LIST_BLOCKS), dim3(MAP_THREADS), (k_raster_view<false, false>), h->d_state, (const float4*)h->pc, (const float4*)h->nr, (const float2*)h->tm, cl, time, time,
                   LIST_SPLAT | LIST_IDS, h->list_v, h->list_vi, h->key_splat, h->key_ids, h->key_both, 0, lat ? OWN_LAT_DS : 1, CleanArgs{nullptr, nullptr, nullptr, 0, nullptr, nullptr, nullptr, nullptr, nullptr, nullptr}, (const DevState*)h->d_state);
            h->own_fast_raster = h->own_fast;
        } else {
            raster_pass(h, nullptr, time, time, LIST_SPLAT | LIST_IDS, h->ids_after, false, 1);
            whole_drawn = true;
        }
        }
        h->view_frame = 0;
        if (h->own_fast_raster) {
            LAUNCH(h, "own_merge_translate", dim3(cdiv(h->P, 256)), dim3(256), k_own_merge_translate, h->key_splat, h->key_ids, h->key_both, h->P, (const uint32_t*)h->seq, h->own_slot_img + (size_t)h->P,
                   h->own_slot_img + 2 * (size_t)h->P, OWN_GFL(h, h->gfl_splat));
        } else {
            LAUNCH(h, "merge_both", dim3(cdiv(h->P, 256)), dim3(256), k_merge_both, h->key_splat, h->key_ids, h->key_both, h->P);
            OWN_FIRST_LIVE(h, h->gfl_splat);
        }
        if (lat) {
            if (!whole_drawn) LAUNCH(h, "own_ids_pack", dim3(1), dim3(1024), k_own_ids_pack, (const unsigned long long*)h->key_ids, h->w, h->h, (const unsigned long long*)h->gfl_splat, h->key_ids);
            else {
                const size_t L = (size_t)ifx_own_lattice(h);
                if (!h->own_lat_tmp && hipMalloc(&h->own_lat_tmp, (L + 1) * 8) != hipSuccess) { h->err = "hipMalloc (own_lat_tmp)"; return IFX_E_HIP; }
                LAUNCH(h, "own_ids_pack", dim3(1), dim3(1024), k_own_ids_pack, (const unsigned long long*)h->key_ids, h->w, h->h, (const unsigned long long*)h->gfl_splat, h->own_lat_tmp);
                HIPCHK(h, hipMemsetAsync(h->key_ids, 0xFF, (size_t)h->P * 8, h->cur));
                HIPCHK(h, hipMemcpyAsync(h->key_ids, h->own_lat_tmp, (L + 1) * 8, hipMemcpyDeviceToDevice, h->cur));
            }
        }
        break;
    }
    case 104:
        h->own_ids_lat = 0;
        raster_pass(h, nullptr, time, time, LIST_SPLAT | LIST_IDS, h->ids_after, false, 1);
        LAUNCH(h, "merge_both", dim3(cdiv(h->P, 256)), dim3(256), k_merge_both, h->key_splat, h->key_ids, h->key_both, h->P);
        OWN_FIRST_LIVE(h, h->gfl_splat);
        break;
    case 5: {
        const int lat = h->own_ids_lat;
        if (lat) LAUNCH(h, "own_ids_unpack", dim3(1), dim3(1024), k_own_ids_unpack, h->key_ids, h->w, h->h, h->gfl_splat);
        h->ids_full_valid = !lat; h->ids_sparse_frame = lat; h->ids_view_ok = 0;
        LAUNCH(h, "splat_resolve", g2, b2, k_splat_resolve, h->d_state, (const float*)nullptr, h->key_splat, (const float4*)h->pc, (const float4*)h->nr, (const float2*)h->col,
               (const float2*)h->tm, c, h->rgb, h->depth_filt, (float4*)h->pred_vertex, (float4*)h->pred_normal, (uchar4*)h->pred_image, (uchar4*)h->pred_inst, h->pred_time,
               (float4*)nullptr, (float4*)nullptr, (uchar4*)nullptr, h->key_ids, h->key_both, h->ids_after, (int*)nullptr, FinishFold(), h->pred_conf, lat ? OWN_LAT_DS : 1,
               (in_frame && h->own_fast_raster) ? (const int32_t*)(h->own_slot_img + (size_t)h->P) : (const int32_t*)nullptr);
        if (in_frame) {
            const int ds = 10, nseg = cdiv(cdiv(h->w, ds) * cdiv(h->h, ds), 256);
            LAUNCH(h, "raster_finish", dim3(1 + nseg), dim3(256), k_raster_finish, h->d_state, (const uchar4*)h->pred_image, h->w, h->h, 0, h->ids_after, (const float4*)h->votes, h->cap, ds, h->d_list_ctr, ifx_idmap(h),
                   h->pred_tail, (int*)nullptr, h->own_fast_raster ? (const int32_t*)(h->own_slot_img + 2 * (size_t)h->P) : (const int32_t*)nullptr);
        }
        break;
    }
    case 6:
        LAUNCH(h, "fill_in", g2, b2, k_fill_in, c, (const uint8_t*)h->rgb, (const uint16_t*)h->depth_filt, (float4*)h->pred_vertex, (const float4*)h->pred_normal,
               (const uchar4*)h->pred_image, (float4*)h->fill_vertex, (float4*)h->fill_normal, (uchar4*)h->fill_image, (const float*)h->pred_conf);
        LAUNCH(h, "raster_finish", dim3(1), dim3(256), k_raster_finish, h->d_state, (const uchar4*)h->pred_image, h->w, h->h, 1, h->ids_after, (const float4*)h->votes, h->cap, 10, h->d_list_ctr, ifx_idmap(h),
               (int*)nullptr, in_frame ? h->pred_tail : (int*)nullptr);
        break;
    case 7: break;
    default: return IFX_E_INVALID;
    }
    return IFX_OK;
}

static int upload_pose(ifx* h, const float* pose16, float** d_pose, float** d_inv)
{
    float buf[32];
    memcpy(buf, pose16, 64);
    pose_inverse(pose16, buf + 16);
    float* slot = h->d_scratch;
    HIPCHK(h, hipMemcpyAsync(slot, buf, 128, hipMemcpyHostToDevice, h->stream));
    HIPCHK(h, hipStreamSynchronize(h->stream));
    *d_pose = slot;
    *d_inv = slot + 16;
    return IFX_OK;
}

extern "C" int ifx_predict_indices(ifx_t* h, const float* pose16, int time)
{
    if (!h || !pose16) return IFX_E_INVALID;
    ifx_drop_tracked(h);
    float *dp, *di;
    int r = upload_pose(h, pose16, &dp, &di);
    if (r) return r;
    index_pass(h, di, time);
    HIPCHK(h, hipStreamSynchronize(h->stream));
    return IFX_OK;
}
// ... 233 lines not shown
```

Measured before the change: 1623 frames/s.

## Fuse surfel update into the post-fuse index pass via upd_owner marks

Adds a k_index_fuse kernel in which some blocks run the per-pixel surfel fuse update and splat the updated surfel straight into the index keys, while the remaining blocks index the view list and skip surfels marked as fused in upd_owner. This replaces the separate fuse-update launch plus a second full index_list pass, so the view list is read once less per frame. The upd_owner marks are left in place and cleared lazily later, either by clean_view or clean_raster_view, or by a full memset when another path needs them. The index block count is capped using an occupancy query so fuse blocks and index blocks can be resident together. This adds state-tracking risk around the marks and uses the r_max value from before the frame. It also adds a small ifx_segment_sums query API.

```diff
diff --git a/include/ifx_c_api.h b/include/ifx_c_api.h
--- a/include/ifx_c_api.h
+++ b/include/ifx_c_api.h
@@ -84,6 +84,7 @@
                            int32_t* ground_votes648);
 int ifx_instance_point_cloud(ifx_t* h, int bbox_type, int32_t* counts96, int inst, float* out10, int max_records);
 int ifx_view_list_stats(ifx_t* h, int32_t* out4);
+int ifx_segment_sums(ifx_t* h, int32_t* out2);
 int ifx_sync(ifx_t* h);
 int ifx_get_pose(ifx_t* h, float* out_pose16);
 int ifx_tick(ifx_t* h);
diff --git a/instancefusion_amd/__init__.py b/instancefusion_amd/__init__.py
--- a/instancefusion_amd/__init__.py
+++ b/instancefusion_amd/__init__.py
@@ -91,6 +91,7 @@
     "ifx_hint_next_frame": (C.c_int, [_P, _P, _P]),
     "ifx_lookahead_stats": (C.c_int, [_P, _P, C.c_int]),
     "ifx_view_list_stats": (C.c_int, [_P, _P]),
+    "ifx_segment_sums": (C.c_int, [_P, _P]),
     "ifx_map_bounding_boxes": (C.c_int, [_P, C.c_int, C.c_float, _P, _P, _P, _P, _P]),
     "ifx_instance_point_cloud": (C.c_int, [_P, C.c_int, _P, C.c_int, _P, C.c_int]),
     "ifx_sync": (C.c_int, [_P]),
@@ -302,6 +303,11 @@
         self._chk(self.L.ifx_view_list_stats(self.handle, _ptr(out)), "ifx_view_list_stats")
         return dict(window=int(out[0]), outside=int(out[1]), scans=int(out[2]), age=int(out[3]))
 
+    def segment_sums(self):
+        out = np.zeros(2, np.int32)
+        self._chk(self.L.ifx_segment_sums(self.handle, _ptr(out)), "ifx_segment_sums")
+        return int(out[0]), int(out[1])
+
     def sync(self):
         self._chk(self.L.ifx_sync(self.handle), "ifx_sync")
 
diff --git a/instancefusion_amd/csrc/ifx_api.hip b/instancefusion_amd/csrc/ifx_api.hip
--- a/instancefusion_amd/csrc/ifx_api.hip
+++ b/instancefusion_amd/csrc/ifx_api.hip
@@ -313,6 +313,7 @@
     else if (s == "slic_ahead") h->opt_slic_ahead = value;
     else if (s == "fold_result") h->opt_fold_result = value;
     else if (s == "clean_raster") h->opt_clean_raster = value;
+    else if (s == "fuse_in_index") h->opt_fuse_in_index = value ? 1 : 0;
     else if (s == "hot_records") { h->opt_hot = value; h->hot_valid = 0; }
     else if (s == "hot_verify") h->opt_hot_verify = value;
     else if (s == "own_first_live") h->opt_own_first_live = value;
@@ -1131,6 +1132,15 @@
     return IFX_OK;
 }
 
+extern "C" int ifx_segment_sums(ifx_t* h, int32_t* out2)
+{
+    if (!h || !out2) return IFX_E_INVALID;
+    if (!h->seg_counts_valid || !h->ev_result) { h->err = "ifx_segment_sums: no frame has left its sums"; return IFX_E_STATE; }
+    HIPCHK(h, hipEventSynchronize(h->ev_result));
+    out2[0] = h->h_result->seg_counts[0]; out2[1] = h->h_result->seg_counts[1];
+    return IFX_OK;
+}
+
 extern "C" int ifx_view_list_stats(ifx_t* h, int32_t* out4)
 {
     if (!h || !out4) return IFX_E_INVALID;
@@ -1493,6 +1503,7 @@
     }
     HIPCHK(h, hipMemcpy(h->d_state, &hs, sizeof(hs), hipMemcpyHostToDevice));
     HIPCHK(h, hipMemset(h->upd_owner, 0xFF, (size_t)h->cap * 4));
+    h->marks_pending = 0;
     HIPCHK(h, hipMemset(h->labels, 0xFF, (size_t)h->cap * 4));
     h->labels_stale_all = 1;
     return IFX_OK;
diff --git a/instancefusion_amd/csrc/ifx_ctx.h b/instancefusion_amd/csrc/ifx_ctx.h
--- a/instancefusion_amd/csrc/ifx_ctx.h
+++ b/instancefusion_amd/csrc/ifx_ctx.h
@@ -265,6 +265,9 @@
     int opt_hot = 1;
     void* frame_hot = nullptr;
     int opt_clean_raster = 1;
+    int opt_fuse_in_index = 1;
+    int marks_pending = 0;
+    int index_fuse_resident = -1;
     int clean_raster_pending = 0;
     float frame_weight_mult = 1.f;
     int opt_fold_result = 1;
diff --git a/instancefusion_amd/csrc/ifx_map.hip b/instancefusion_amd/csrc/ifx_map.hip
--- a/instancefusion_amd/csrc/ifx_map.hip
+++ b/instancefusion_amd/csrc/ifx_map.hip
@@ -1476,32 +1476,33 @@
     for (unsigned int t = (blockIdx.x / LIST_SEGS) * blockDim.x + threadIdx.x; t < n; t += blockDim.x * (gridDim.x / LIST_SEGS)) flat[t] = raw[t];
 }
 
-__global__ __launch_bounds__(MAP_THREADS) void k_index_list(const DevState* __restrict__ st, const float4* __restrict__ pc, const float2* __restrict__ tm, Cam c, int time,
-                                                            const unsigned int* __restrict__ list, unsigned long long* __restrict__ keys, const Hot* __restrict__ hot = nullptr)
-{
-    const int fl = FIRST_LIVE(c);
-    float T[12];
-#pragma unroll
-    for (int k = 0; k < 12; k++) T[k] = st->pose_inv[k];
-    const unsigned int n = min(st->vl_n[0], c.seg_cap * LIST_SEGS);
+template <bool MARKS>
+__device__ __forceinline__ void index_list_body(const float* T, unsigned int n, int fl, const float4* __restrict__ pc, const float2* __restrict__ tm, const Cam& c, int time, const unsigned int* __restrict__ list,
+                                                unsigned long long* __restrict__ keys, const Hot* __restrict__ hot, const uint32_t* __restrict__ marks, unsigned int bid, unsigned int nblk)
+{
 #ifndef INDEX_U
 #define INDEX_U 1
 #endif
     constexpr int U = INDEX_U;
-    const unsigned int stride = blockDim.x * gridDim.x;
-    for (unsigned int t = blockIdx.x * blockDim.x + threadIdx.x; t < n; t += U * stride) {
+    const unsigned int stride = blockDim.x * nblk;
+    for (unsigned int t = bid * blockDim.x + threadIdx.x; t < n; t += U * stride) {
         unsigned int i[U];
         bool in[U];
 #pragma unroll
         for (int u = 0; u < U; u++) { const unsigned int tt = t + u * stride; in[u] = tt < n; i[u] = list[in[u] ? tt : t]; }
         float lastT[U];
         float4 p4[U];
-#pragma unroll
-        for (int u = 0; u < U; u++) { lastT[u] = hot ? hot[i[u]].tm.y : ld_once(&tm[i[u]]).y; p4[u] = hot ? hot[i[u]].pc : ld_once(&pc[i[u]]); }
-#pragma unroll
-        for (int u = 0; u < U; u++) asm volatile("" ::"v"(lastT[u]), "v"(p4[u].x), "v"(p4[u].y), "v"(p4[u].z));
+        uint32_t mk[U];
 #pragma unroll
         for (int u = 0; u < U; u++) {
+            lastT[u] = hot ? hot[i[u]].tm.y : ld_once(&tm[i[u]]).y; p4[u] = hot ? hot[i[u]].pc : ld_once(&pc[i[u]]);
+            mk[u] = MARKS ? marks[i[u]] : 0xFFFFFFFFu;
+        }
+#pragma unroll
+        for (int u = 0; u < U; u++) asm volatile("" ::"v"(lastT[u]), "v"(p4[u].x), "v"(p4[u].y), "v"(p4[u].z), "v"(mk[u]));
+#pragma unroll
+        for (int u = 0; u < U; u++) {
+            if (MARKS && mk[u] != 0xFFFFFFFFu) continue;
             if (!in[u] || (float)time - lastT[u] > (float)c.timeDelta) continue;
             const v3 p = xf_point(T, v3m(p4[u].x, p4[u].y, p4[u].z));
             if (p.z > c.maxDepth || p.z < 0) continue;
@@ -1513,9 +1514,19 @@
         }
     }
 }
+__global__ __launch_bounds__(MAP_THREADS) void k_index_list(const DevState* __restrict__ st, const float4* __restrict__ pc, const float2* __restrict__ tm, Cam c, int time,
+                                                            const unsigned int* __restrict__ list, unsigned long long* __restrict__ keys, const Hot* __restrict__ hot = nullptr)
+{
+    const int fl = FIRST_LIVE(c);
+    float T[12];
+#pragma unroll
+    for (int k = 0; k < 12; k++) T[k] = st->pose_inv[k];
+    const unsigned int n = min(st->vl_n[0], c.seg_cap * LIST_SEGS);
+    index_list_body<false>(T, n, fl, pc, tm, c, time, list, keys, hot, nullptr, blockIdx.x, gridDim.x);
+}
 
 __global__ __launch_bounds__(MAP_THREADS) void k_clean_view(DevState* st, Cam c, int time, float4* __restrict__ pc, const float4* __restrict__ nr, float2* __restrict__ tm,
-                                                            const float4* __restrict__ tap, const unsigned int* __restrict__ list)
+                                                            const float4* __restrict__ tap, const unsigned int* __restrict__ list, uint32_t* __restrict__ upd_owner = nullptr)
 {
     float T[12];
 #pragma unroll
@@ -1538,6 +1549,7 @@
             const float4 p4 = ld_once(&pc[i]);
             asm volatile("" ::"v"(tt.y), "v"(p4.x), "v"(p4.y), "v"(p4.z), "v"(p4.w));
             const float wv = tt.y;
+            if (upd_owner && wv == (float)time) upd_owner[i] = 0xFFFFFFFFu;
             if (wv > DEAD_TIME && !(wv > 0.f && (float)time - wv > (float)c.timeDelta)) {
                 if (!((float)time - wv > (float)c.timeDelta)) {
                     const v3 p = xf_point(T, v3m(p4.x, p4.y, p4.z));
@@ -1611,7 +1623,7 @@
 struct alignas(16) RvRec { float qx, qy, qz, nx, ny, nz, r2; unsigned int id; int x0, y0, bw, excl; int s01, s23, i01, i23; };
 #define RV_SLOTS 512
 struct Hot;
-struct CleanArgs { float4* pc_rw; float2* tm_rw; const float4* tap; int nf_blocks; const uint32_t* assoc; const float4* mpc; const float4* mnr; int* flags; int* block_counts; Hot* hot; };
+struct CleanArgs { float4* pc_rw; float2* tm_rw; const float4* tap; int nf_blocks; const uint32_t* assoc; const float4* mpc; const float4* mnr; int* flags; int* block_counts; Hot* hot; uint32_t* upd_owner; };
 __device__ __forceinline__ void new_flags_body(DevState* st, const float* __restrict__ pose_inv_ex, const Cam& c, int time, const uint32_t* __restrict__ assoc, const float4* __restrict__ mpc,
                                                const float4* __restrict__ mnr, const float4* __restrict__ tap, int* __restrict__ flags, int* __restrict__ block_counts, int bid);
 #ifndef WALK_MIN_WAVES
@@ -1685,6 +1697,7 @@
             float4 n4c = make_float4(0.f, 0.f, 0.f, 0.f);
             bool have_n = false;
             if (CLEAN && t < na) {
+                if (ca.upd_owner && tt.y == (float)time) ca.upd_owner[i] = 0xFFFFFFFFu;
                 const float wv = tt.y;
                 if (wv > DEAD_TIME && !(wv > 0.f && (float)time - wv > (float)c.timeDelta)) {
                     bool cand = false;
@@ -1841,7 +1854,7 @@
 
 static void launch_raster_view(ifx* h, const char* name, const Cam& c, unsigned int want, int ids_step, bool lds, const CleanArgs* clean)
 {
-    const CleanArgs ca = clean ? *clean : CleanArgs{nullptr, nullptr, nullptr, 0, nullptr, nullptr, nullptr, nullptr, nullptr, nullptr};
+    const CleanArgs ca = clean ? *clean : CleanArgs{nullptr, nullptr, nullptr, 0, nullptr, nullptr, nullptr, nullptr, nullptr, nullptr, nullptr};
     const dim3 grid(ca.nf_blocks + (h->opt_view_blocks > 0 ? h->opt_view_blocks : 4 * LIST_BLOCKS));
     auto go = [&](auto kernel) {
         LAUNCH(h, name, grid, dim3(MAP_THREADS), kernel, h->d_state, (const float4*)h->pc, (const float4*)h->nr, (const float2*)h->tm, c, h->tick, h->tick, want, h->list_v, h->list_vi,
@@ -2101,21 +2114,22 @@
     if (lb >= 0) atomicMin(&upd_owner[lb], (uint32_t)(i * c.h + j));
 }
 
-__global__ void k_fuse_update(DevState* __restrict__ st, const uint32_t* __restrict__ assoc, const float4* __restrict__ mpc, const float4* __restrict__ mnr,
-                              const float* __restrict__ mcol, Cam c, int time, uint32_t* __restrict__ upd_owner, float4* __restrict__ pc, float4* __restrict__ nr,
-                              float2* __restrict__ col, float2* __restrict__ tm, const int32_t* __restrict__ assoc_slot = nullptr, Hot* __restrict__ hot = nullptr)
-{
-    const int fl = FIRST_LIVE(c);
-    const int par = time % 2, i = 2 * (blockIdx.x * blockDim.x + threadIdx.x) + par, j = 2 * (blockIdx.y * blockDim.y + threadIdx.y) + par;
+template <bool INDEX>
+__device__ __forceinline__ void fuse_update_body(DevState* __restrict__ st, int fl, int count, int bx, int by, const uint32_t* __restrict__ assoc, const float4* __restrict__ mpc, const float4* __restrict__ mnr,
+                                                 const float* __restrict__ mcol, const Cam& c, int time, uint32_t* __restrict__ upd_owner, float4* __restrict__ pc, float4* __restrict__ nr,
+                                                 float2* __restrict__ col, float2* __restrict__ tm, const int32_t* __restrict__ assoc_slot, Hot* __restrict__ hot, const float* T = nullptr,
+                                                 unsigned long long* __restrict__ keys = nullptr, unsigned int rmax0 = 0u)
+{
+    const int par = time % 2, i = 2 * bx + par, j = 2 * by + par;
     if (i >= c.w || j >= c.h) return;
     int k = j * c.w + i;
     const uint32_t gid = assoc[k];
     if (gid >= ASSOC_NEW) return;
-    const int li = assoc_slot ? assoc_slot[k] : local_slot(c, st->count, gid, fl);
-    if (li < 0 || li >= st->count) return;
+    const int li = assoc_slot ? assoc_slot[k] : local_slot(c, count, gid, fl);
+    if (li < 0 || li >= count) return;
     const uint32_t id = (uint32_t)li;
     if (upd_owner[id] != (uint32_t)(i * c.h + j)) return;
-    upd_owner[id] = 0xFFFFFFFFu;
+    if (!INDEX) upd_owner[id] = 0xFFFFFFFFu;
     float4 p = hot ? hot[id].pc : pc[id], n = hot ? hot[id].nr : nr[id], mp = mpc[k], mn = mnr[k];
     const float2 cl0 = col[id], t0_ = hot ? hot[id].tm : tm[id];
     const float mc = mcol[k];
@@ -2136,7 +2150,7 @@
         v3 nn = normalized(v3m(t0, t1, t2));
         nr[id] = make_float4(nn.x, nn.y, nn.z, t3);
         if (hot) hot[id].nr = make_float4(nn.x, nn.y, nn.z, t3);
-        if (t3 > 0.f && t3 < 1e30f && __float_as_uint(t3) > st->r_max_bits) atomicMax(&st->r_max_bits, __float_as_uint(t3));
+        if (t3 > 0.f && t3 < 1e30f && __float_as_uint(t3) > (INDEX ? rmax0 : st->r_max_bits)) atomicMax(&st->r_max_bits, __float_as_uint(t3));
         pc[id] = p;
     } else {
         p.w = c_k + a;
@@ -2146,6 +2160,41 @@
     t.y = (float)time;
     tm[id] = t;
     if (hot) { hot[id].pc = p; hot[id].tm = t; }
+    if (INDEX) {
+        const v3 q = xf_point(T, v3m(p.x, p.y, p.z));
+        if (q.z > c.maxDepth || q.z < 0) return;
+        const float uu = ((c.fx * q.x) / q.z) + c.cx, v = ((c.fy * q.y) / q.z) + c.cy;
+        if (!(uu >= 0 && uu < (float)c.w && v >= 0 && v < (float)c.h)) return;
+        const int px_ = point_pixel(uu), py_ = point_pixel(v);
+        if (px_ < 0 || py_ < 0) return;
+        key_min(&keys[py_ * c.w + px_], make_key(q.z, key_id(c, id, fl)));
+    }
+}
+__global__ void k_fuse_update(DevState* __restrict__ st, const uint32_t* __restrict__ assoc, const float4* __restrict__ mpc, const float4* __restrict__ mnr,
+                              const float* __restrict__ mcol, Cam c, int time, uint32_t* __restrict__ upd_owner, float4* __restrict__ pc, float4* __restrict__ nr,
+                              float2* __restrict__ col, float2* __restrict__ tm, const int32_t* __restrict__ assoc_slot = nullptr, Hot* __restrict__ hot = nullptr)
+{
+    const int fl = FIRST_LIVE(c);
+    fuse_update_body<false>(st, fl, st->count, blockIdx.x * blockDim.x + threadIdx.x, blockIdx.y * blockDim.y + threadIdx.y, assoc, mpc, mnr, mcol, c, time, upd_owner, pc, nr, col, tm, assoc_slot, hot);
+}
+
+struct FuseArgs { const uint32_t* assoc; const float4* mpc; const float4* mnr; const float* mcol; uint32_t* upd_owner; float4* pc; float4* nr; float2* col; float2* tm; Hot* hot; int nb, gx; };
+__global__ __launch_bounds__(MAP_THREADS) void k_index_fuse(DevState* st, const DevState* __restrict__ stc, const float4* __restrict__ pc, const float2* __restrict__ tm, Cam c, int time,
+                                                            const unsigned int* __restrict__ list, unsigned long long* __restrict__ keys, const Hot* __restrict__ hot, FuseArgs fa)
+{
+    const int fl = FIRST_LIVE(c);
+    float T[12];
+#pragma unroll
+    for (int k = 0; k < 12; k++) T[k] = stc->pose_inv[k];
+    const unsigned int n = min(stc->vl_n[0], c.seg_cap * LIST_SEGS);
+    if ((int)blockIdx.x < fa.nb) {
+        const int gbx = (int)blockIdx.x % fa.gx, gby = (int)blockIdx.x / fa.gx;
+        const unsigned int rmax0 = stc->r_max_bits;
+        fuse_update_body<true>(st, fl, stc->count, gbx * 32 + (int)(threadIdx.x & 31), gby * 8 + (int)(threadIdx.x >> 5), fa.assoc, fa.mpc, fa.mnr, fa.mcol, c, time, fa.upd_owner, fa.pc, fa.nr, fa.col, fa.tm,
+                               nullptr, fa.hot, T, keys, rmax0);
+        return;
+    }
+    index_list_body<true>(T, n, fl, pc, tm, c, time, list, keys, hot, fa.upd_owner, blockIdx.x - (unsigned int)fa.nb, gridDim.x - (unsigned int)fa.nb);
 }
 
 __device__ inline int clean_test(const float* T, const Cam& c, int time, float4 p4, float4 n4, float initT, float& lastT, const float4* __restrict__ tap)
@@ -2383,6 +2432,7 @@
 {
     h->ids_view_ok = 0;
     h->hot_valid = 0;
+    if (h->marks_pending) { hipMemsetAsync(h->upd_owner, 0xFF, (size_t)h->cap * 4, h->cur); h->marks_pending = 0; }
     ifx_vlist_reap(h);
     int n = h->cap;
     LAUNCH(h, "alive_flags", dim3(cdiv(n, 256)), dim3(256), k_alive_flags, h->d_state, (const float2*)h->tm, h->scan_flags, n);
@@ -2399,12 +2449,16 @@
 static void fuse_pass(ifx* h, const float* d_pose, float weighting, int time, int part = 0, const int32_t* own_slot = nullptr, Hot* hot = nullptr)
 {
     if (!hot) h->hot_valid = 0;
+    if (h->marks_pending) {
+        hipMemsetAsync(h->upd_owner, 0xFF, (size_t)h->cap * 4, h->cur);
+        h->marks_pending = 0;
+    }
     Cam c = make_cam(h);
     dim3 b(32, 8), g(cdiv(cdiv(h->w, 2), 32), cdiv(cdiv(h->h, 2), 8));
     if (part != 2)
         LAUNCH(h, "associate", g, b, k_associate, h->d_state, d_pose, weighting, h->dm, h->dmf, h->rgb, h->index_id, (const float4*)h->index_vc, (const float4*)h->index_nr, c, time,
                h->assoc_target, (float4*)h->meas_pc, (float4*)h->meas_nr, h->meas_col, h->upd_owner, (const uint8_t*)h->assoc_vis, part == 1 ? h->assoc_key : (unsigned long long*)nullptr);
-    if (part == 1) return;
+    if (part == 1 || part == 3) return;
     const bool slots = part == 2 && own_slot && h->own_slot_img;
     if (part == 2) LAUNCH(h, "assoc_decode", g, b, k_assoc_decode, h->d_state, (const unsigned long long*)h->assoc_key, h->index_id, c, time, h->assoc_target, h->upd_owner,
                           slots ? own_slot : (const int32_t*)nullptr, slots ? h->own_slot_img + 3 * (size_t)h->P : (int32_t*)nullptr);
@@ -2624,12 +2678,38 @@
                (const float2*)h->col, (const float2*)h->tm, h->P, (uint32_t*)nullptr, (float4*)nullptr, (float4*)nullptr, (float4*)nullptr, time, h->cfg.confidence, (float4*)h->index_tap, c,
                (const int32_t*)nullptr, (const Hot*)h->frame_hot);
 }
+static void index_fuse_pass(ifx* h, int time, Hot* hot)
+{
+    Cam c = make_cam(h);
+    c.srank = 0; c.sn = 1;
+    if (!hot) h->hot_valid = 0;
+    FuseArgs fa;
+    fa.assoc = h->assoc_target; fa.mpc = (const float4*)h->meas_pc; fa.mnr = (const float4*)h->meas_nr; fa.mcol = h->meas_col; fa.upd_owner = h->upd_owner;
+    fa.pc = (float4*)h->pc; fa.nr = (float4*)h->nr; fa.col = (float2*)h->col; fa.tm = (float2*)h->tm; fa.hot = hot;
+    fa.gx = cdiv(cdiv(h->w, 2), 32); fa.nb = fa.gx * cdiv(cdiv(h->h, 2), 8);
+    if (h->index_fuse_resident < 0) {
+        int cus = 0, dev = 0, occ = 0;
+        hipGetDevice(&dev);
+        hipDeviceGetAttribute(&cus, hipDeviceAttributeMultiprocessorCount, dev);
+        h->index_fuse_resident = (hipOccupancyMaxActiveBlocksPerMultiprocessor(&occ, k_index_fuse, MAP_THREADS, 0) == hipSuccess && occ > 0 && cus > 0) ? occ * cus : 0;
+        (void)hipGetLastError();
+    }
+    int nb_index = h->opt_index_blocks > 0 ? h->opt_index_blocks : LIST_BLOCKS;
+    if (h->index_fuse_resident > 0) nb_index = std::max(64, std::min(nb_index, h->index_fuse_resident - fa.nb));
+    LAUNCH(h, "index_list", dim3(fa.nb + nb_index), dim3(MAP_THREADS), k_index_fuse, h->d_state, (const DevState*)h->d_state, (const float4*)h->pc, (const float2*)h->tm, c, time, h->list_v, h->key_index,
+           (const Hot*)hot, fa);
+    h->marks_pending = 1;
+    LAUNCH(h, "index_resolve_taps", dim3(cdiv(h->P, 256)), dim3(256), k_index_resolve, h->d_state, (const float*)nullptr, h->key_index, (const float4*)h->pc, (const float4*)h->nr,
+           (const float2*)h->col, (const float2*)h->tm, h->P, (uint32_t*)nullptr, (float4*)nullptr, (float4*)nullptr, (float4*)nullptr, time, h->cfg.confidence, (float4*)h->index_tap, c,
+           (const int32_t*)nullptr, (const Hot*)hot);
+}
 
 static void view_clean_append(ifx* h, const Cam& c, int time)
 {
     h->hot_valid = 0;
     LAUNCH(h, "clean_view", dim3(h->opt_clean_blocks > 0 ? h->opt_clean_blocks : 2 * LIST_BLOCKS), dim3(MAP_THREADS), k_clean_view, h->d_state, c, time, (float4*)h->pc, (const float4*)h->nr, (float2*)h->tm,
-           (const float4*)h->index_tap, h->list_v);
+           (const float4*)h->index_tap, h->list_v, h->marks_pending ? h->upd_owner : (uint32_t*)nullptr);
+    h->marks_pending = 0;
     launch_new_flags_count(h, nullptr, c, time);
     launch_append_scan(h, c, time, h->own ? (unsigned int*)nullptr : h->list_v);
 }
@@ -2660,8 +2740,13 @@
         h->frame_hot = hot;
         if (h->view_scan_tick != time) view_scan(h, time);
         index_list_pass(h, time, false);
+        if (fused && h->opt_fuse_in_index && !h->lc_enable) {
+            fuse_pass(h, nullptr, 0.f, time, 3, nullptr, hot);
+            index_fuse_pass(h, time, hot);
+        } else {
         fuse_pass(h, nullptr, 0.f, time, 0, nullptr, hot);
         index_list_pass(h, time, true);
+        }
         h->clean_raster_pending = fused ? 1 : 0;
         if (!fused) view_clean_append(h, c, time);
         h->view_frame = 1; h->view_dirty = 1; h->last_clean_time = time;
@@ -2731,6 +2816,8 @@
             CleanArgs ca;
             ca.pc_rw = (float4*)h->pc; ca.tm_rw = (float2*)h->tm; ca.tap = (const float4*)h->index_tap; ca.nf_blocks = nb_new; ca.assoc = h->assoc_target; ca.mpc = (const float4*)h->meas_pc;
             ca.mnr = (const float4*)h->meas_nr; ca.flags = h->scan_flags; ca.block_counts = h->scan_block; ca.hot = (Hot*)h->frame_hot;
+            ca.upd_owner = h->marks_pending ? h->upd_owner : (uint32_t*)nullptr;
+            h->marks_pending = 0;
             launch_raster_view(h, "clean_raster_view", c, want_walk, ids_step, false, &ca);
             launch_append_scan(h, c, h->tick, h->list_v, (Hot*)h->frame_hot);
             raster_pass(h, nullptr, h->tick, h->tick, want, h->ids_after, true, 2, 0, true, ids_step, true);
@@ -2949,7 +3036,7 @@
         if (fused) {
             CleanArgs ca;
             ca.pc_rw = (float4*)h->pc; ca.tm_rw = (float2*)h->tm; ca.tap = (const float4*)h->index_tap; ca.nf_blocks = nb_new; ca.assoc = h->assoc_target; ca.mpc = (const float4*)h->meas_pc;
-            ca.mnr = (const float4*)h->meas_nr; ca.flags = h->scan_flags; ca.block_counts = h->scan_block; ca.hot = nullptr;
+            ca.mnr = (const float4*)h->meas_nr; ca.flags = h->scan_flags; ca.block_counts = h->scan_block; ca.hot = nullptr; ca.upd_owner = nullptr;
             LAUNCH(h, "clean_raster_view", dim3(nb_new + (h->opt_view_blocks > 0 ? h->opt_view_blocks : 4 * LIST_BLOCKS)), dim3(MAP_THREADS), (k_raster_view<false, true>), h->d_state, (const float4*)h->pc, (const float4*)h->nr,
                    (const float2*)h->tm, c, time, time, LIST_SPLAT | LIST_IDS, h->list_v, h->list_vi, h->key_splat, h->key_ids, h->key_both, 0, lat ? OWN_LAT_DS : 1, ca, (const DevState*)h->d_state);
             launch_append_scan(h, c, time, h->list_v);
@@ -2973,7 +3060,7 @@
             cl.srank = 0; cl.sn = 1;
             if (h->own_fast) { cl.own_n = 0; cl.raw_slots = 1; }
             LAUNCH(h, "raster_view", dim3(h->opt_view_blocks > 0 ? h->opt_view_blocks : 4 * LIST_BLOCKS), dim3(MAP_THREADS), (k_raster_view<false, false>), h->d_state, (const float4*)h->pc, (const float4*)h->nr, (const float2*)h->tm, cl, time, time,
-                   LIST_SPLAT | LIST_IDS, h->list_v, h->list_vi, h->key_splat, h->key_ids, h->key_both, 0, lat ? OWN_LAT_DS : 1, CleanArgs{nullptr, nullptr, nullptr, 0, nullptr, nullptr, nullptr, nullptr, nullptr, nullptr}, (const DevState*)h->d_state);
+                   LIST_SPLAT | LIST_IDS, h->list_v, h->list_vi, h->key_splat, h->key_ids, h->key_both, 0, lat ? OWN_LAT_DS : 1, CleanArgs{nullptr, nullptr, nullptr, 0, nullptr, nullptr, nullptr, nullptr, nullptr, nullptr, nullptr}, (const DevState*)h->d_state);
             h->own_fast_raster = h->own_fast;
         } else {
             raster_pass(h, nullptr, time, time, LIST_SPLAT | LIST_IDS, h->ids_after, false, 1);
```

Measured after the change: 1645 frames/s, median of 6. Within noise of the previous version (+1.3%).
